# Li-Yuetao/ActiveSplat

Measured on AMD Instinct MI355X. Metric: render+backward frames/sec at 640x480, N Gaussians, higher is better.
Workload: dtype f32; 1 GPU; BASELINE configs[2]'s render (the north star's target configuration): 2000000 Gaussians, SH degree 3, 640x480, forward (colour+radii+depth+opacity) + backward (all input gradients), frames strictly one after the other; gaussians=2000000, sh_degree=3, width=640, height=480, tile_instances_D=4842856, streams=1, parallelism=single GPU

## Files before the change

activesplat_amd/_lib.py:

```python
from __future__ import annotations

import ctypes as C
import os

_HERE = os.path.dirname(os.path.abspath(__file__))
LIB_PATH = os.path.join(_HERE, "libgsplat_hip.so")

_lib = None
_emulated = False


class GsCamera(C.Structure):
    _fields_ = [("image_width", C.c_int32), ("image_height", C.c_int32), ("sh_degree", C.c_int32),
                ("sh_coeffs", C.c_int32), ("tanfovx", C.c_float), ("tanfovy", C.c_float),
                ("scale_modifier", C.c_float), ("num_views", C.c_int32), ("bg", C.c_void_p),
                ("viewmatrix", C.c_void_p), ("projmatrix", C.c_void_p), ("campos", C.c_void_p)]


class GsGeomLayout(C.Structure):
    _fields_ = [(n, C.c_uint64) for n in ("total_bytes", "geom", "rect", "tiles_touched", "offsets", "block_sums", "clamped",
                                          "tile_total", "tile_base", "sh_jac", "depth_bits")]


class GsImageLayout(C.Structure):
    _fields_ = [(n, C.c_uint64) for n in ("total_bytes", "ranges", "final_T", "n_contrib", "split_state")]


class GsAdamTensor(C.Structure):
    _fields_ = [("n", C.c_int64), ("param", C.c_void_p), ("grad", C.c_void_p), ("exp_avg", C.c_void_p), ("exp_avg_sq", C.c_void_p),
                ("lr", C.c_double), ("beta1", C.c_double), ("beta2", C.c_double), ("eps", C.c_double), ("step", C.c_int32),
                ("reserved", C.c_int32)]


class GsRowTensor(C.Structure):
    _fields_ = [("param", C.c_void_p), ("exp_avg", C.c_void_p), ("exp_avg_sq", C.c_void_p), ("grad", C.c_void_p),
                ("lr", C.c_double), ("beta1", C.c_double), ("beta2", C.c_double), ("eps", C.c_double), ("width", C.c_int32),
                ("step", C.c_int32)]


class GsBinLayout(C.Structure):
    _fields_ = [(n, C.c_uint64) for n in ("total_bytes", "path", "pairs", "keys_unsorted", "vals_unsorted", "keys_sorted",
                                          "sort_temp", "segments", "seg_T", "pairs_alt")]


class GsDbscanLayout(C.Structure):
    _fields_ = [(n, C.c_uint64) for n in ("total_bytes", "mask_bits", "core_bits", "root_bits", "word_prefix", "parent", "root", "row_range")]


class GsEvalLayout(C.Structure):
    _fields_ = [("total_bytes", C.c_uint64), ("ms_ssim_defined", C.c_int32), ("levels", C.c_int32), ("level_width", C.c_int32 * 5),
                ("level_height", C.c_int32 * 5)]


class GsHullLayout(C.Structure):
    _fields_ = [(n, C.c_uint64) for n in ("total_bytes", "cluster_status")]


class GsMeshLayout(C.Structure):
    _fields_ = [(n, C.c_uint64) for n in ("total_bytes", "total", "records", "rects", "tile_count", "tile_offset", "list")]


SORT_AUTO, SORT_TILE_LDS, SORT_RADIX = 0, 1, 2


ABI_VERSION = 22

vp, i32, u32, i64, u64, f32, f64, cint = C.c_void_p, C.c_int32, C.c_uint32, C.c_int64, C.c_uint64, C.c_float, C.c_double, C.c_int

BINDINGS = {
    "gs_atlas_layout": (cint, [i32, i32, i32, C.POINTER(i32), C.POINTER(i32), C.POINTER(i32)]),
    "gs_geom_layout": (cint, [i32, i32, i32, C.POINTER(GsGeomLayout)]),
    "gs_image_layout": (cint, [i32, i32, C.POINTER(GsImageLayout)]),
    "gs_bin_layout": (cint, [i64, u32, i32, i32, C.POINTER(GsBinLayout)]),
    "gs_set_sort_path": (cint, [i32]),
    "gs_set_forward_segments": (cint, [i32]),
    "gs_set_half_quadrants": (cint, [i32]),
    "gs_set_backward_chain": (cint, [i32, i32]),
    "gs_set_backward_chain_tickets": (cint, [i32]),
    "gs_set_backward_chain_polls": (cint, [i32]),
    "gs_set_forward_priority": (cint, [i32, f32]),
    "gs_async_status_word": (cint, [C.POINTER(C.POINTER(u32))]),
    "gs_async_status_clear": (cint, []),
    "gs_recorded_cut": (cint, [u32, C.POINTER(u32), C.POINTER(i32)]),
    "gs_set_backward_segments": (cint, [i32]),
    "gs_backward_scratch_bytes": (u64, [i32]),
    "gs_last_error": (C.c_char_p, []),
    "gs_version": (C.c_char_p, []),
    "gs_abi_version": (i32, []),
    "gs_profile_enable": (cint, [i32]),
    "gs_profile_stage_count": (i32, []),
    "gs_profile_stage_name": (C.c_char_p, [i32]),
    "gs_profile_collect": (cint, [vp, vp, i32]),
    "gs_preprocess_forward": (cint, [C.POINTER(GsCamera), i32] + [vp] * 12 + [i32, vp]),
    "gs_render_forward": (cint, [C.POINTER(GsCamera), i32, i64, u32] + [vp] * 10),
    "gs_render_backward": (cint, [C.POINTER(GsCamera), i32, i64] + [vp] * 21 + [i32, i32, vp]),
    "gs_preprocess_forward_raw": (cint, [C.POINTER(GsCamera), i32] + [vp] * 7 + [i32] + [vp] * 7 + [i32, vp]),
    "gs_render_backward_raw": (cint, [C.POINTER(GsCamera), i32, i64] + [vp] * 7 + [i32, i32] + [vp] * 14 + [i32, i32, vp]),
    "gs_pose_grad_scratch_bytes": (u64, [i32]),
    "gs_render_backward_raw_pose": (cint, [C.POINTER(GsCamera), i32, i64] + [vp] * 7 + [i32, i32] + [vp] * 14 + [i32, i32, i32, vp, vp, vp]),
    "gs_adam_step": (cint, [i64] + [vp] * 4 + [f64] * 4 + [i32, vp]),
    "gs_adam_step_multi": (cint, [i32, C.POINTER(GsAdamTensor), vp]),
    "gs_render_backward_raw_adam": (cint, [C.POINTER(GsCamera), i32, i64] + [vp] * 7 + [i32] + [vp] * 8 + [i32, i32, C.POINTER(GsAdamTensor), vp]),
    "gs_pack_columns": (cint, [i32, C.POINTER(GsRowTensor), i64, i64, vp, vp]),
    "gs_adam_rows": (cint, [i32, C.POINTER(GsRowTensor), i64, i64, i64, vp, vp, vp]),
    "gs_unpack_columns": (cint, [i32, C.POINTER(GsRowTensor), i64, vp, vp]),
    "gs_activate_forward": (cint, [i32, i32] + [vp] * 10),
    "gs_activate_backward": (cint, [i32, i32] + [vp] * 13),
    "gs_activate_backward_accumulate": (cint, [i32, i32] + [vp] * 13),
    "gs_activate_backward_pose": (cint, [i32, i32] + [vp] * 13 + [i32, i32, vp, vp, vp]),
    "gs_mapping_loss_scratch_bytes": (u64, [i32, i32]),
    "gs_mapping_loss": (cint, [i32, i32] + [vp] * 5 + [f32, f32] + [vp] * 4 + [i64, vp]),
    "gs_depth_error_median_scratch_bytes": (u64, [i32, i32]),
    "gs_depth_error_median": (cint, [i32, i32] + [vp] * 5),
    "gs_depth_error_median_grid": (cint, [i32, i32] + [vp] * 4 + [i32, vp]),
    "gs_depth_error_median_workgroups": (i32, [i32, i32]),
    "gs_mapping_loss_outlier": (cint, [i32, i32] + [vp] * 5 + [f32, f32] + [vp] * 4 + [i64, vp, vp]),
    "gs_tracking_loss_scratch_bytes": (u64, [i32, i32]),
    "gs_tracking_loss": (cint, [i32, i32] + [vp] * 6 + [i32, f32, f32, f32] + [vp] * 5),
    "gs_tracking_loss_outlier": (cint, [i32, i32] + [vp] * 6 + [i32, f32, f32, f32] + [vp] * 6),
    "gs_preprocess_forward_raw_dev": (cint, [C.POINTER(GsCamera), i32] + [vp] * 8 + [i64, i64, i32] + [vp] * 7 + [i32, vp]),
    "gs_preprocess_forward_topdown": (cint, [C.POINTER(GsCamera), i32] + [vp] * 5 + [i32, f32, f32] + [vp] * 6),
    "gs_render_forward_topdown": (cint, [C.POINTER(GsCamera), i32, i64, u32] + [vp] * 9),
    "gs_render_backward_raw_pose_dev": (cint, [C.POINTER(GsCamera), i32, i64] + [vp] * 8 + [i64, i64, i32] + [vp] * 8 + [i32, i32, vp, vp, vp]),
    "gs_tracking_state_bytes": (u64, []),
    "gs_tracking_begin": (cint, [vp, vp, i64, i64, vp, vp]),
    "gs_tracking_step": (cint, [i32, vp, i32, i32, vp, f32, f32, vp, vp, i64, i64, f64, f64, i32, vp, vp, vp]),
    "gs_compact_scratch_bytes": (u64, [i64]),
    "gs_compact_index": (cint, [i64] + [vp] * 5),
    "gs_gather_rows": (cint, [i64, i32] + [vp] * 4),
    "gs_gather_rows_zero_tail": (cint, [i64, i64, i32] + [vp] * 4),
    "gs_densify_classify": (cint, [i32, i32] + [vp] * 5 + [f32, f32, i32, i32] + [vp] * 5),
    "gs_densify_children": (cint, [i32, i32, i32, vp, vp, u64, vp, vp, vp]),
    "gs_compact3_scratch_bytes": (u64, [i64]),
    "gs_compact_index3": (cint, [i64, vp, vp, vp, i32] + [vp] * 4),
    "gs_visibility_stats": (cint, [i32] + [vp] * 4),
    "gs_accumulate_grad2d": (cint, [i32] + [vp] * 5),
    "gs_grid_dbscan_layout": (cint, [i32] * 4 + [C.POINTER(GsDbscanLayout)]),
    "gs_grid_dbscan": (cint, [i32, i32, i32, vp, i64, i64, f32] + [i32] * 4 + [vp] * 7),
    "gs_cluster_hulls_layout": (cint, [i32] * 5 + [C.POINTER(GsHullLayout)]),
    "gs_cluster_hulls": (cint, [i32, i32, i32, vp, vp, i64, i64, vp, vp, i32, C.POINTER(u32), i32, i32, f32, f64, f64, i32] + [vp] * 8),
    "gs_high_loss_grid": (cint, [i32, i32, vp, vp, vp, f32, f32, i32, i32, vp, vp, vp]),
    "gs_grow_scratch_bytes": (u64, [i32, i32]),
    "gs_grow_gaussians": (cint, [i32, i32] + [vp] * 6 + [f32, i32] + [vp] * 8),
    "gs_keyframe_overlap": (cint, [i32, vp, i32, vp, vp, i32, i32, i32, vp, vp]),
    "gs_frame_ingest": (cint, [i32, i32, vp, vp, vp, i32, C.POINTER(i32)] + [vp] * 5),
    "gs_mesh_render_layout": (cint, [i32, i32, i32, u32, C.POINTER(GsMeshLayout)]),
    "gs_mesh_render": (cint, [i32, vp, i32, vp, vp, C.POINTER(f32), C.POINTER(f32), f32, i32, i32, vp, u32, vp, vp, vp, vp, vp]),
    "gs_depth_cloud": (cint, [i32, i32, vp, C.POINTER(f32), C.POINTER(f32), vp, vp, vp]),
    "gs_cloud_nearest_scratch_bytes": (u64, [i64, i64]),
    "gs_cloud_nearest": (cint, [i64, vp, vp, i64, vp, vp, i32, vp, vp, vp]),
    "gs_completion_row_scratch_bytes": (u64, []),
    "gs_completion_row": (cint, [i64, vp, i64, vp, vp, f64, vp, vp, vp]),
    "gs_eval_frame_layout": (cint, [i32, i32, i32, C.POINTER(GsEvalLayout)]),
    "gs_eval_frame": (cint, [i32, i32] + [vp] * 5 + [f32, i32, vp, vp, vp]),
}

SYMBOLS = tuple(BINDINGS)


def _bind(lib):
    try:
        lib.gs_abi_version.restype = i32
        have = int(lib.gs_abi_version())
# ... 92 lines not shown
```

activesplat_amd/csrc/api.hip:

```cpp
#include <stdio.h>
#include <string.h>

#include <mutex>

#include "gs_common.h"

namespace {

thread_local char g_err[512] = "";

int fail(int code, const char* fmt, const char* a = "")
{
    snprintf(g_err, sizeof(g_err), fmt, a);
    return code;
}

int launched(const char* who, const char* what, hipError_t e)
{
    if (e == hipSuccess) return GS_OK;
    snprintf(g_err, sizeof(g_err), "%s: %s%s%s", who, what, *what ? " " : "", hipGetErrorString(e));
    return GS_ELAUNCH;
}

bool adam_aligned16(const void* p, const void* g, const void* m, const void* v)
// ... 94 lines not shown
    g.geom = (float4*)(b + L.geom); g.rect = (uint2*)(b + L.rect); g.tiles = (uint32_t*)(b + L.tiles_touched);
    g.offsets = (uint32_t*)(b + L.offsets); g.block_sums = (uint32_t*)(b + L.block_sums);
    g.clamped = (uint32_t*)(b + L.clamped);
    g.tile_total = (uint32_t*)(b + L.tile_total); g.tile_base = (uint32_t*)(b + L.tile_base);
    g.sh_jac = (float2*)(b + L.sh_jac);
    g.depth_bits = (uint32_t*)(b + L.depth_bits);
    g.vis_max = nullptr; g.vis_seen = nullptr;
    return g;
}

}

extern "C" {

const char* gs_last_error(void) { return g_err; }
const char* gs_version(void) { return "activesplat_amd gsplat_hip 0.4 (gfx950)"; }
int32_t gs_abi_version(void) { return GS_ABI_VERSION; }

int gs_profile_enable(int32_t on)
{
    g_prof.on = on != 0;
    g_prof.n = 0;
    return GS_OK;
}

int32_t gs_profile_stage_count(void) { return ST_COUNT; }

const char* gs_profile_stage_name(int32_t stage) { return stage >= 0 && stage < ST_COUNT ? kStageNames[stage] : ""; }

int gs_profile_collect(float* ms_sum, int32_t* calls, int32_t n_stages)
{
    if (!ms_sum || !calls || n_stages < ST_COUNT) return fail(GS_EINVAL, "gs_profile_collect: bad argument");
    for (int i = 0; i < n_stages; i++) { ms_sum[i] = 0.f; calls[i] = 0; }
    for (int i = 0; i < g_prof.n; i++) {
        if (hipEventSynchronize(g_prof.ev[i][1]) != hipSuccess) return fail(GS_ELAUNCH, "gs_profile_collect: event sync failed");
        float ms = 0.f;
        if (hipEventElapsedTime(&ms, g_prof.ev[i][0], g_prof.ev[i][1]) != hipSuccess) return fail(GS_ELAUNCH, "gs_profile_collect: elapsed failed");
        ms_sum[g_prof.stage[i]] += ms; calls[g_prof.stage[i]]++;
    }
    g_prof.n = 0;
    return GS_OK;
}

int gs_set_sort_path(int32_t path)
{
    if (path < GS_SORT_AUTO || path > GS_SORT_RADIX) return fail(GS_EINVAL, "gs_set_sort_path: bad path");
    g_sort_path = path;
    return GS_OK;
}

int gs_set_half_quadrants(int32_t max_tiles)
{
    gs::g_half_quadrant_tiles = max_tiles < 0 ? 0 : max_tiles;
    return GS_OK;
}

int gs_set_backward_chain(int32_t pieces, int32_t min_tiles)
{
    if (pieces < 1 || pieces > gs::kChainPieces) return fail(GS_EINVAL, "gs_set_backward_chain: pieces out of range");
    gs::g_chain_pieces = pieces;
    gs::g_chain_min_tiles = min_tiles < 0 ? gs::kChainMinTiles : min_tiles;
    return GS_OK;
}

int gs_set_backward_chain_tickets(int32_t on)
{
    gs::g_chain_tickets = on != 0;
    return GS_OK;
}

int gs_set_backward_chain_polls(int32_t polls)
{
    gs::g_chain_polls = polls == -1 ? gs::kChainPollsDefault : polls;
    return GS_OK;
}

int gs_set_forward_priority(int32_t mode, float param)
{
    if (mode > gs::kFwdPrioChunk) return fail(GS_EINVAL, "gs_set_forward_priority: mode out of range");
    if (mode == gs::kFwdPrioT && param >= 1.0f) return fail(GS_EINVAL, "gs_set_forward_priority: a transmittance threshold lies below 1");
    if (mode < 0) { mode = gs::kFwdPrioDefault; param = gs::kFwdPrioDefaultParam; }
    gs::g_fwd_prio_param = param > 0.0f ? param : 0.0f;
    gs::g_fwd_prio = mode;
    return GS_OK;
}

int gs_async_status_word(uint32_t** host_word)
{
    static uint32_t* word = nullptr;
    static std::mutex mu;
    std::lock_guard<std::mutex> lock(mu);
    if (!word) {
        void* h = nullptr;
        if (hipHostMalloc(&h, 64, hipHostMallocMapped | hipHostMallocPortable) != hipSuccess) {
            (void)hipGetLastError();
            return fail(GS_ELAUNCH, "gs_async_status_word: hipHostMalloc failed");
        }
        memset(h, 0, 64);
        void* d = nullptr;
        if (hipHostGetDevicePointer(&d, h, 0) != hipSuccess) { (void)hipGetLastError(); return fail(GS_ELAUNCH, "gs_async_status_word: no device view of the host word"); }
        void* f = nullptr;
        if (hipMalloc(&f, 64) == hipSuccess && hipMemset(f, 0, 64) == hipSuccess && hipGetDevice(&gs::g_chain_fail_device) == hipSuccess) gs::g_chain_fail_dev = (uint32_t*)f;
        else (void)hipGetLastError();
        word = (uint32_t*)h;
        gs::g_async_status_dev = (uint32_t*)d;
    }
    if (host_word) *host_word = word;
    return GS_OK;
}

int gs_async_status_clear(void)
{
    if (hipDeviceSynchronize() != hipSuccess) { (void)hipGetLastError(); return fail(GS_ELAUNCH, "gs_async_status_clear: device synchronisation failed"); }
    if (gs::g_chain_fail_dev && hipMemset(gs::g_chain_fail_dev, 0, 4) != hipSuccess) { (void)hipGetLastError(); return fail(GS_ELAUNCH, "gs_async_status_clear: hipMemset failed"); }
    return GS_OK;
}

int gs_recorded_cut(uint32_t target, uint32_t* nearest, int32_t* level)
{
    const uint32_t pos = gs::cut_nearest(target);
    if (nearest) *nearest = pos;
    if (level) *level = pos ? gs::cut_level(pos) : -1;
    return GS_OK;
}

int gs_set_backward_segments(int32_t segments)
{
    if (segments < 1 || segments > gs::kFewSegmentsMax) return fail(GS_EINVAL, "gs_set_backward_segments: 1, 2 or 3");
    gs::g_few_segments = segments;
    return GS_OK;
}

int gs_set_forward_segments(int32_t on)
{
    g_segments_enabled = on != 0;
    return GS_OK;
}

int gs_atlas_layout(int32_t P, int32_t view_width, int32_t num_views, int32_t* virtual_P, int32_t* atlas_width, int32_t* view_stride)
{
    if (P < 0 || view_width <= 0 || num_views < 1 || num_views > 64) return fail(GS_EINVAL, "gs_atlas_layout: bad argument");
    const int32_t stride = atlas_view_stride(view_width, num_views);
    if (virtual_P) *virtual_P = virtual_rows(P, num_views);
    if (atlas_width) *atlas_width = num_views * stride;
    if (view_stride) *view_stride = stride;
    return GS_OK;
}

int gs_geom_layout(int32_t P, int32_t width, int32_t height, GsGeomLayout* out)
{
    if (!out || P < 0 || width <= 0 || height <= 0) return fail(GS_EINVAL, "gs_geom_layout: bad argument");
    const uint64_t n = (uint64_t)(P > 0 ? P : 1);
    const uint64_t nb = (n + gs::kBlock - 1) / gs::kBlock;
    const uint64_t tiles = tiles_of(width, height);
    const uint64_t rows = (n + 1023) / 1024;
    uint64_t o = 0;
    out->geom = o; o = align_up(o + n * GS_GEOM_FLOATS * 4);
    out->rect = o; o = align_up(o + n * 8);
    out->tiles_touched = o; o = align_up(o + n * 4);
    out->offsets = o; o = align_up(o + n * 4);
    out->block_sums = o; o = align_up(o + (nb + 1) * 4);
    out->clamped = o; o = align_up(o + n * 4);
    out->tile_total = o; o = align_up(o + tiles * 4);
    out->tile_base = o; o = align_up(o + (tiles <= (uint64_t)gs::kMaxLdsTiles ? rows * tiles * 4 : 4));
    out->sh_jac = o; o = align_up(o + n * gs::kShJacFloats * 4);
    out->depth_bits = o; o = align_up(o + n * 4);
// ... 169 lines not shown
    ForwardCall c{};
    c.in.means3D = means3D; c.in.shs = shs; c.in.colors = colors_precomp; c.in.opac = logit_opacities; c.in.scales = log_scales; c.in.rots = unnorm_rotations;
    c.P = P; c.pose.source = gs::POSE_HOST; c.pose.pose7 = h_pose7; c.isotropic = isotropic; c.max_2D_radius = max_2D_radius; c.seen = seen;
    c.radii = radii; c.geom_state = geom_state; c.image_state = image_state; c.d_counts = d_counts; c.h_counts = h_counts; c.want_backward = want_backward;
    return preprocess_forward_impl(cam, c, stream);
}

int gs_preprocess_forward_raw_dev(const GsCamera* cam, int32_t P, const float* means3D, const float* shs, const float* colors_precomp,
                                  const float* logit_opacities, const float* log_scales, const float* unnorm_rotations,
                                  const float* cam_unnorm_rots, const float* cam_trans, int64_t num_frames, int64_t time_idx, int32_t isotropic,
                                  float* max_2D_radius, uint8_t* seen, int32_t* radii, void* geom_state, void* image_state, uint32_t* d_counts,
                                  uint32_t* h_counts, int32_t want_backward, gs_stream_t stream)
{
    ForwardCall c{};
    c.pose.source = gs::POSE_DEVICE;
    if (!dev_pose(cam_unnorm_rots, cam_trans, num_frames, time_idx, c.pose.dev))
        return fail(GS_EINVAL, "gs_preprocess_forward_raw_dev: null pose columns or time index outside [0, num_frames)");
    if (P > 0 && (!log_scales || !unnorm_rotations)) return fail(GS_EINVAL, "gs_preprocess_forward_raw_dev: null scale / rotation parameters");
    c.in.means3D = means3D; c.in.shs = shs; c.in.colors = colors_precomp; c.in.opac = logit_opacities; c.in.scales = log_scales; c.in.rots = unnorm_rotations;
    c.P = P; c.isotropic = isotropic; c.max_2D_radius = max_2D_radius; c.seen = seen;
    c.radii = radii; c.geom_state = geom_state; c.image_state = image_state; c.d_counts = d_counts; c.h_counts = h_counts; c.want_backward = want_backward;
    return preprocess_forward_impl(cam, c, stream);
}

static int bin_tile_lists(const char* who, const gs::Cam& k, int32_t P, int64_t D, uint32_t max_tile_instances, gs::GeomPtrs gp, uint2* ranges,
                          const GsBinLayout& BL, char* bb, uint32_t* point_list, hipStream_t st)
{
    hipError_t e;
    if (BL.path == GS_SORT_TILE_LDS) {
        if (D > 0) {
            ScopedStage ps(ST_TILE_SCATTER_SORT, st);
            e = gs::launch_tile_scatter_sort(k, P, gp, gp.tile_base, ranges, max_tile_instances,
                                             (unsigned long long*)(bb + BL.pairs), (unsigned long long*)(bb + BL.pairs_alt), point_list, (uint32_t)D, st);
            if (int rc = launched(who, "tile scatter/sort", e)) return rc;
        }
    } else {
        e = hipMemsetAsync(ranges, 0, (size_t)k.gx * k.gy * 8, st);
        if (int rc = launched(who, "memset", e)) return rc;
        if (k.gx * k.gy <= gs::kMaxLdsTiles) {
            e = gs::launch_scan_block_sums(P, gp, gp.block_sums + (P + gs::kBlock - 1) / gs::kBlock, st);
            if (int rc = launched(who, "scan", e)) return rc;
        }
        if (D == 0) {
            e = gs::launch_emit(k, P, gp, nullptr, nullptr, st);
            if (int rc = launched(who, "emit", e)) return rc;
        } else {
            uint64_t* ku = (uint64_t*)(bb + BL.keys_unsorted); uint32_t* vu = (uint32_t*)(bb + BL.vals_unsorted);
            uint64_t* ks = (uint64_t*)(bb + BL.keys_sorted);
            { ScopedStage ps(ST_EMIT, st); e = gs::launch_emit(k, P, gp, ku, vu, st); }
            if (int rc = launched(who, "emit", e)) return rc;
            const int end_bit = 32 + tile_bits(k.gx * k.gy);
            {
                ScopedStage ps(ST_SORT, st);
                e = gs::sort_pairs(bb + BL.sort_temp, (size_t)(BL.total_bytes - BL.sort_temp), ku, ks, vu, point_list, D, end_bit, st);
            }
            if (int rc = launched(who, "sort", e)) return rc;
            { ScopedStage ps(ST_RANGES, st); e = gs::launch_ranges(D, ks, ranges, st); }
            if (int rc = launched(who, "ranges", e)) return rc;
        }
    }
    return GS_OK;
}

int gs_render_forward(const GsCamera* cam, int32_t P, int64_t D, uint32_t max_tile_instances, void* geom_state,
                      void* bin_state, uint32_t* point_list, void* image_state, float* out_color, float* out_depth,
                      float* out_opacity, float* out_depth_sq, void* backward_scratch, gs_stream_t stream)
{
    gs::Cam k;
    if (!make_cam(cam, k)) return fail(GS_EINVAL, "gs_render_forward: invalid camera settings");
    if (P < 0 || D < 0 || !geom_state || !image_state || !out_color || !out_depth || !out_opacity)
        return fail(GS_EINVAL, "gs_render_forward: null pointer");
    if (D > 0 && (!bin_state || !point_list)) return fail(GS_EINVAL, "gs_render_forward: null binning workspace");
    if (D >= (int64_t)1 << 32) return fail(GS_ECAPACITY, "gs_render_forward: more than 2^32 tile instances");
    hipStream_t st = (hipStream_t)stream;
    const int32_t Pin = P;
    P = virtual_count(k, Pin);
    gs::GeomPtrs gp = carve_geom(geom_state, P, k);
    GsImageLayout IL; gs_image_layout(k.W, k.H, &IL);
    char* ib = (char*)image_state;
    uint2* ranges = (uint2*)(ib + IL.ranges);
    GsBinLayout BL; gs_bin_layout(D, max_tile_instances, k.W, k.H, &BL);
    char* bb = (char*)bin_state;
    if (int rc = bin_tile_lists("gs_render_forward", k, P, D, max_tile_instances, gp, ranges, BL, bb, point_list, st)) return rc;
    ScopedStage ps(ST_BLEND_FWD, st);
    return launched("gs_render_forward", "blend", gs::launch_blend_forward(k, ranges, point_list, gp.geom, out_color, out_depth, out_opacity,
                    (float*)(ib + IL.final_T), (uint32_t*)(ib + IL.n_contrib), out_depth_sq, BL.path == GS_SORT_TILE_LDS ? (uint32_t)D : 0xffffffffu,
                    (int)BL.segments, BL.segments > 1 ? (float*)(bb + BL.seg_T) : nullptr, (float*)(ib + IL.split_state), (uint32_t)P,
                    (float*)backward_scratch, st));
}

int gs_preprocess_forward_topdown(const GsCamera* cam, int32_t P, const float* means3D, const float* colors_precomp, const float* logit_opacities,
                                  const float* log_scales, const float* unnorm_rotations, int32_t isotropic, float band_upper, float band_lower,
                                  int32_t* radii, void* geom_state, void* image_state, uint32_t* d_counts, uint32_t* h_counts, gs_stream_t stream)
{
    if (cam && cam->num_views > 1) return fail(GS_EINVAL, "gs_preprocess_forward_topdown: one view only");
    if (P > 0 && (!colors_precomp || !log_scales || !unnorm_rotations))
        return fail(GS_EINVAL, "gs_preprocess_forward_topdown: null colour / scale / rotation parameters");
    if (band_upper != band_upper || band_lower != band_lower) return fail(GS_EINVAL, "gs_preprocess_forward_topdown: NaN height band");
    ForwardCall c{};
    c.in.means3D = means3D; c.in.colors = colors_precomp; c.in.opac = logit_opacities; c.in.scales = log_scales; c.in.rots = unnorm_rotations;
    c.P = P; c.pose.source = gs::POSE_BAND; c.pose.band_upper = band_upper; c.pose.band_lower = band_lower; c.isotropic = isotropic;
    c.radii = radii; c.geom_state = geom_state; c.image_state = image_state; c.d_counts = d_counts; c.h_counts = h_counts;
    return preprocess_forward_impl(cam, c, stream);
}

int gs_render_forward_topdown(const GsCamera* cam, int32_t P, int64_t D, uint32_t max_tile_instances, void* geom_state, void* bin_state,
                              uint32_t* point_list, void* image_state, float* free_opacity, uint8_t* free_map_binary, uint8_t* visible_rgb,
                              uint8_t* visible_map_binary, gs_stream_t stream)
{
    gs::Cam k;
    if (!make_cam(cam, k)) return fail(GS_EINVAL, "gs_render_forward_topdown: invalid camera settings");
    if (k.V != 1) return fail(GS_EINVAL, "gs_render_forward_topdown: one view only");
    if (P < 0 || D < 0 || !geom_state || !image_state || !free_opacity || !free_map_binary || !visible_rgb || !visible_map_binary)
        return fail(GS_EINVAL, "gs_render_forward_topdown: null pointer");
    if (((uintptr_t)free_map_binary | (uintptr_t)visible_rgb | (uintptr_t)visible_map_binary | (uintptr_t)free_opacity) & 3)
        return fail(GS_EINVAL, "gs_render_forward_topdown: output maps must be 4-byte aligned");
    if (D > 0 && (!bin_state || !point_list)) return fail(GS_EINVAL, "gs_render_forward_topdown: null binning workspace");
    if (D >= (int64_t)1 << 32) return fail(GS_ECAPACITY, "gs_render_forward_topdown: more than 2^32 tile instances");
    hipStream_t st = (hipStream_t)stream;
    virtual_count(k, P);
    gs::GeomPtrs gp = carve_geom(geom_state, P, k);
    GsImageLayout IL; gs_image_layout(k.W, k.H, &IL);
    uint2* ranges = (uint2*)((char*)image_state + IL.ranges);
    GsBinLayout BL; gs_bin_layout(D, max_tile_instances, k.W, k.H, &BL);
    if (int rc = bin_tile_lists("gs_render_forward_topdown", k, P, D, max_tile_instances, gp, ranges, BL, (char*)bin_state, point_list, st)) return rc;
    ScopedStage ps(ST_BLEND_FWD, st);
    return launched("gs_render_forward_topdown", "blend", gs::launch_blend_topdown(k, ranges, point_list, gp.geom, free_opacity, free_map_binary, visible_rgb,
                    visible_map_binary, BL.path == GS_SORT_TILE_LDS ? (uint32_t)D : 0xffffffffu, (uint32_t)P, st));
}

struct BackwardCall {
    int32_t P;
    int64_t D;
    gs::GaussianBackward g;
    gs::PoseRequest pose;
    int32_t isotropic, accumulate;
    const void* geom_state; const uint32_t* point_list; const void* image_state;
    const float* dL_dcolor; const float* dL_ddepth;
    void* scratch; int32_t scratch_zeroed, have_sh_jacobian;
    const GsAdamTensor* adam5;
};

static int render_backward_impl(const GsCamera* cam, const BackwardCall& c, gs_stream_t stream)
{
    gs::GaussianBackward g = c.g;
    const gs::GaussianInputs& in = g.in;
    const gs::GaussianGrads& out = g.out;
    const gs::PoseRequest& pose = c.pose;
    const int32_t P = c.P;
    const bool pose_only = pose.grad == gs::POSE_GRAD_ONLY;
    gs::Cam k;
    if (!make_cam(cam, k)) return fail(GS_EINVAL, "gs_render_backward: invalid camera settings");
    set_input_activation(k, pose, c.isotropic, pose_only ? 0 : c.accumulate);
    if (k.act && k.V != 1) return fail(GS_EINVAL, "gs_render_backward_raw: one view only");
    if (k.act && (!in.opac || in.cov3D || (in.shs && k.sh_coeffs != 16)))
        return fail(GS_EINVAL, "gs_render_backward_raw: scale / rotation parameters with colours or 16-coefficient SH rows only");
    if (k.V > 1) return fail(GS_EINVAL, "gs_render_backward: multi-view atlas renders are forward-only");
    if (P < 0 || c.D < 0 || !c.geom_state || !c.image_state || !c.dL_dcolor || !c.scratch)
        return fail(GS_EINVAL, "gs_render_backward: null pointer");
    if (pose.grad && (!k.act || c.adam5 || (!pose.dL_dpose7 && pose.source != gs::POSE_DEVICE) || !pose.pose_scratch))
        return fail(GS_EINVAL, "gs_render_backward_raw_pose: raw-parameter mode with a pose-gradient output and its scratch only");
    if (pose.source == gs::POSE_DEVICE && !pose_only) return fail(GS_EINVAL, "gs_render_backward_raw_pose_dev: the pose-only backward only");
    if (P == 0) {
        if (pose.grad && pose.dL_dpose7)
            return launched("gs_render_backward_raw_pose", "memset", hipMemsetAsync(pose.dL_dpose7, 0, 7 * sizeof(float), (hipStream_t)stream));
        return GS_OK;
    }
    gs::FusedAdam fa{};
    if (c.adam5) {
        if (!k.act || c.accumulate) return fail(GS_EINVAL, "gs_render_backward_raw_adam: raw-parameter mode without accumulation only");
        if (!in.means3D || !g.radii || !out.dmeans2D || !in.scales || !in.rots || (in.shs == nullptr) == (in.colors == nullptr))
// ... 750 lines not shown
```

activesplat_amd/csrc/blend.hip:

```cpp
#include "gs_common.h"
#include <atomic>

namespace gs {

constexpr int kFwdStreams = 4;

constexpr float kAlphaMin = 1.0f / 255.0f;
constexpr float kTmin = 0.0001f;
constexpr float kLog2e = 1.4426950408889634f;
constexpr uint32_t kNoId = 0xffffffffu;

struct TileCtx {
    int tile, tx, ty, px, py, quad, seg;
    float qx0, qy0, pxf, pyf;
    bool inside;
};

template <int NW>
__device__ __forceinline__ bool tile_ctx_at(const Cam& cam, unsigned block, int wave, int lane, TileCtx& c, int segments = 0)
{
    const int G = (segments > 1 ? 4 * segments : 4) / NW;
    const int ntiles = cam.gx * cam.gy, per = (ntiles + 7) >> 3;
    const int idx = (int)(block >> 3);
    c.tile = (int)(block & 7) * per + idx / G;
    if (idx / G >= per || c.tile >= ntiles) return false;
    int quad = (idx % G) * NW + wave;
    c.seg = segments > 1 ? quad >> 2 : 0;
    if (segments > 1) quad &= 3;
    c.tx = c.tile % cam.gx; c.ty = c.tile / cam.gx; c.quad = quad;
    const int qx = c.tx * kTile + (quad & 1) * kQuad, qy = c.ty * kTile + (quad >> 1) * kQuad;
    c.px = qx + (lane & 7); c.py = qy + (lane >> 3);
    c.qx0 = (float)qx; c.qy0 = (float)qy; c.pxf = (float)c.px; c.pyf = (float)c.py;
    c.inside = c.px < cam.W && c.py < cam.H;
    return true;
}

template <int NW>
__device__ __forceinline__ bool tile_ctx_nw(const Cam& cam, int wave, int lane, TileCtx& c, int segments = 0)
{
    return tile_ctx_at<NW>(cam, blockIdx.x, wave, lane, c, segments);
}


struct StreamPixel { int sid, l, px, py; float pxf, pyf; bool inside; };
__device__ __forceinline__ StreamPixel stream_pixel(const Cam& cam, float qx0, float qy0, int lane)
{
    StreamPixel s;
    s.sid = lane >> 4; s.l = lane & 15;
    s.px = (int)qx0 + (s.sid & 1) * 4 + (s.l & 3); s.py = (int)qy0 + (s.sid >> 1) * 4 + (s.l >> 2);
    s.inside = s.px < cam.W && s.py < cam.H;
    s.pxf = (float)s.px; s.pyf = (float)s.py;
    return s;
}

struct StagedConic { float4 s0; float c; };
__device__ __forceinline__ StagedConic staged_conic(const float4& q0, const float4& q1)
{
    return {make_float4(q0.x, q0.y, -0.5f * kLog2e * q0.z, -kLog2e * q0.w), -0.5f * kLog2e * q1.x};
}
__device__ __forceinline__ void stage_record(float4* s0, float4* s1, float4* s2, int lane, const float4& q0,
                                             const float4& q1, const float4& q2, uint32_t id)
{
    const StagedConic k = staged_conic(q0, q1);
    s0[lane] = k.s0;
    s1[lane] = make_float4(k.c, q1.y, q1.z, q1.w);
    s2[lane] = make_float4(q2.x, q2.y, __uint_as_float(id), 0.0f);
}

struct SplatAlpha { float alpha, p, G; bool hit; };
__device__ __forceinline__ SplatAlpha splat_alpha(const float4& a0, float c, float op, float pxf, float pyf)
{
    SplatAlpha a;
    const float dx = a0.x - pxf, dy = a0.y - pyf;
    float bdy, cyy;
    {
#pragma clang fp contract(off)
        bdy = a0.w * dy; cyy = (c * dy) * dy;
    }
    a.p = (a0.z * dx + bdy) * dx + cyy;
    a.G = __builtin_amdgcn_exp2f(a.p);
    a.alpha = fminf(0.99f, op * a.G);
    a.hit = a.p <= 0.0f && a.alpha >= kAlphaMin;
    return a;
}

struct Composite { float T, w; bool done, ok; };
__device__ __forceinline__ Composite composite_step(float T, bool done, float alpha, bool hit)
{
    const float test_T = T * (1.0f - alpha);
    const bool vis = !done && hit;
    const bool ok = vis && test_T >= kTmin;
    return {ok ? test_T : T, ok ? alpha * T : 0.0f, done || (vis != ok), ok};
}

__device__ __forceinline__ void write_sentinel(float4* s0, float4* s1, float4* s2, int lane)
{
    if (lane == 0) {
        s0[kWave] = make_float4(0.f, 0.f, 0.f, 0.f);
        s1[kWave] = make_float4(0.f, 0.f, 0.f, 0.f);
        s2[kWave] = make_float4(0.f, 0.f, __uint_as_float(0u), 0.f);
    }
    __builtin_amdgcn_wave_barrier();
}

__device__ __forceinline__ unsigned scan_blocks(const float4& q0, const float4& q2, bool valid, float qx0, float qy0, bool g0, bool g1, bool g2, bool g3,
                                                unsigned long long& m_any, unsigned long long* masks = nullptr)
{
    const float ex = q2.z, ey = q2.w;
    const float xl = q0.x - ex, xh = q0.x + ex, yl = q0.y - ey, yh = q0.y + ey;
    const unsigned long long vis = __ballot(valid) & __ballot(ex >= 0.0f);
    const unsigned long long cx0 = __ballot(xh >= qx0) & __ballot(xl <= qx0 + 3.0f), cx1 = __ballot(xh >= qx0 + 4.0f) & __ballot(xl <= qx0 + 4.0f + 3.0f);
    const unsigned long long cy0 = vis & __ballot(yh >= qy0) & __ballot(yl <= qy0 + 3.0f), cy1 = vis & __ballot(yh >= qy0 + 4.0f) & __ballot(yl <= qy0 + 4.0f + 3.0f);
    const unsigned long long b0 = g0 ? cx0 & cy0 : 0ull, b1 = g1 ? cx1 & cy0 : 0ull, b2 = g2 ? cx0 & cy1 : 0ull, b3 = g3 ? cx1 & cy1 : 0ull;
    m_any = (b0 | b1) | (b2 | b3);
    if (masks) { masks[0] = b0; masks[1] = b1; masks[2] = b2; masks[3] = b3; }
    return (__builtin_amdgcn_inverse_ballot_w64(b0) ? 1u : 0u) | (__builtin_amdgcn_inverse_ballot_w64(b1) ? 2u : 0u) |
           (__builtin_amdgcn_inverse_ballot_w64(b2) ? 4u : 0u) | (__builtin_amdgcn_inverse_ballot_w64(b3) ? 8u : 0u);
}
__device__ __forceinline__ void scan_going_blocks(const float4& q0, const float4& q2, bool valid, float qx0, float qy0, unsigned long long going,
                                                  unsigned long long& m_any, unsigned long long* masks)
{
    scan_blocks(q0, q2, valid, qx0, qy0, (going & 0xffffull) != 0ull, (going & 0xffff0000ull) != 0ull, (going & 0xffff00000000ull) != 0ull,
                (going >> 48) != 0ull, m_any, masks);
}

__device__ __forceinline__ int build_stream_lists(uint8_t* lists, const unsigned long long* mb, int lane, int* ranks = nullptr)
{
    reinterpret_cast<uint32_t*>(lists)[lane] = 0x40404040u;
    __builtin_amdgcn_wave_barrier();
    int ntrips = 0;
#pragma unroll
    for (int s = 0; s < 4; s++) {
        const unsigned long long m = mb[s];
        const int rank = (int)__builtin_amdgcn_mbcnt_hi((uint32_t)(m >> 32), __builtin_amdgcn_mbcnt_lo((uint32_t)m, 0u));
        const bool in = __builtin_amdgcn_inverse_ballot_w64(m);
        if (in) lists[s * kWave + rank] = (uint8_t)lane;
        if (ranks) ranks[s] = in ? rank : 0xff;
        ntrips = max(ntrips, (int)__popcll(m));
    }
    return ntrips;
}

struct GradFill {
    size_t at, end;
};
__device__ __forceinline__ GradFill grad_fill_start(const float4* zero_fill, uint32_t P, int tid)
{
    GradFill f = {0, 0};
    if (zero_fill) {
        const size_t total = (size_t)P * (kGradStride / 4), per = (total + gridDim.x - 1) / gridDim.x;
        f.at = (size_t)blockIdx.x * per + tid; f.end = min(total, (size_t)blockIdx.x * per + per);
    }
    return f;
}
__device__ __forceinline__ GradFill grad_fill_step(float4* zero_fill, GradFill f, int threads)
{
    constexpr int kPerStep = 2;
#pragma unroll
    for (int k = 0; k < kPerStep; k++)
        if (f.at < f.end) { zero_fill[f.at] = make_float4(0.f, 0.f, 0.f, 0.f); f.at += threads; }
    return f;
}
__device__ __forceinline__ void grad_fill_rest(float4* zero_fill, GradFill f, int threads)
{
    for (; f.at < f.end; f.at += threads) zero_fill[f.at] = make_float4(0.f, 0.f, 0.f, 0.f);
}

template <bool DEPTH_SQ>
__device__ __forceinline__ void store_pixel_outputs(const Cam& cam, int px, int py, float T, uint32_t last, float C0, float C1, float C2, float Dp, float Dq,
                                                    float* out_color, float* out_depth, float* out_opacity, float* final_T, uint32_t* n_contrib,
                                                    float* out_depth_sq)
{
    const size_t pix = (size_t)py * cam.W + px, HW = (size_t)cam.H * cam.W;
    final_T[pix] = T;
    n_contrib[pix] = last;
    out_color[pix] = C0 + T * cam.bg[0];
    out_color[HW + pix] = C1 + T * cam.bg[1];
    out_color[2 * HW + pix] = C2 + T * cam.bg[2];
    out_depth[pix] = Dp;
    out_opacity[pix] = 1.0f - T;
    if (DEPTH_SQ) out_depth_sq[pix] = Dq;
}
__device__ __forceinline__ void set_wave_priority(int level)
{
    level = __builtin_amdgcn_readfirstlane(level);
    if (level >= 3) __builtin_amdgcn_s_setprio(3);
    else if (level == 2) __builtin_amdgcn_s_setprio(2);
    else if (level == 1) __builtin_amdgcn_s_setprio(1);
    else __builtin_amdgcn_s_setprio(0);
}
constexpr int kRoundSlack = 4;

template <bool DEPTH_SQ, int NS, int SEG, int NW>
__global__ __launch_bounds__(NW * kWave) void blend_forward_streams_kernel(
    Cam cam, const uint2* __restrict__ ranges, const uint32_t* __restrict__ point_list,
    const float4* __restrict__ geom, float* __restrict__ out_color, float* __restrict__ out_depth,
    float* __restrict__ out_opacity, float* __restrict__ final_T, uint32_t* __restrict__ n_contrib,
    float* __restrict__ out_depth_sq, uint32_t cap, float* __restrict__ seg_T, float* __restrict__ split_state, uint32_t P,
    float4* __restrict__ zero_fill)
{
    static_assert(NS == 4 && kWave / NS == 16, "the scan tests the four 4x4 blocks of a quadrant");
    __shared__ float4 s_rec[NW][3][kWave + 1];
    __shared__ __attribute__((aligned(16))) uint8_t s_list[NW][4 * kWave + 16];
    const int tid = threadIdx.x, lane = tid & 63, wave = tid >> 6;
    GradFill fill = grad_fill_start(SEG == 0 ? zero_fill : nullptr, P, tid);
    TileCtx c;
    if (SEG == 0 && cam.chain > 1 && split_state && blockIdx.x == 0 && tid < 8)
        reinterpret_cast<uint32_t*>(split_state)[(size_t)cam.gx * cam.gy * 4 * (kChainStateFloats + kChainPieces - 1) + (size_t)tid * kChainTicketStride] = 0u;
    if (!tile_ctx_nw<NW>(cam, wave, lane, c)) { if (SEG == 0) grad_fill_rest(zero_fill, fill, NW * kWave); return; }
    if (SEG == 0 && cam.chain > 1 && split_state && lane < kChainPieces - 1)
        reinterpret_cast<uint32_t*>(split_state)[(size_t)cam.gx * cam.gy * 4 * kChainStateFloats + (size_t)(c.tile * 4 + c.quad) * (kChainPieces - 1) + lane] = 0u;
    const StreamPixel sp = stream_pixel(cam, c.qx0, c.qy0, lane);
    const int px = sp.px, py = sp.py;
    const bool inside = sp.inside;
    const float pxf = sp.pxf, pyf = sp.pyf;
    float4* s0 = s_rec[wave][0]; float4* s1 = s_rec[wave][1]; float4* s2 = s_rec[wave][2];
    write_sentinel(s0, s1, s2, lane);
    uint8_t* my_list = s_list[wave] + sp.sid * kWave;
    uint2 range = ranges[c.tile];
    range.x = min(range.x, cap); range.y = min(range.y, cap);
    const uint32_t n_all = range.y - range.x;
    const uint32_t* list = point_list + range.x;
    uint32_t first = 0, n = n_all;
    float T = 1.0f;
    bool next_stopped = true;
    float* my_seg_T = nullptr;
    uint32_t* seg_flag = nullptr;
    if (SEG != 0) {
        const uint32_t S = gridDim.y, seg = blockIdx.y;
        const uint32_t L = (((n_all + S - 1) / S + kWave - 1) / kWave) * kWave;
        first = min(n_all, seg * L);
        n = min(n_all, first + L);
        float* tile_T = seg_T + ((size_t)c.tile * S) * kBlock + c.quad * kWave + lane;
        my_seg_T = tile_T + (size_t)seg * kBlock;
        if (SEG == 1) {
            seg_flag = reinterpret_cast<uint32_t*>(seg_T + (size_t)cam.gx * cam.gy * S * kBlock) + c.tile * 4 + c.quad;
            const uint32_t f = __hip_atomic_load(seg_flag, __ATOMIC_RELAXED, __HIP_MEMORY_SCOPE_AGENT);
            if (f & ((1u << seg) - 1u)) { my_seg_T[0] = 1.0f; return; }
        }
        if (SEG == 2) {
            for (uint32_t q = 0; q < seg; q++) T *= tile_T[(size_t)q * kBlock];
            next_stopped = seg + 1 == S ? true : (T * my_seg_T[0] < kTmin);
        }
    }
    float C0 = 0.f, C1 = 0.f, C2 = 0.f, Dp = 0.f, Dq = 0.f;
    uint32_t last = 0;
    const bool stopped_at_entry = SEG == 2 && T < kTmin;
    bool done = !inside || stopped_at_entry;

    if (SEG == 1 || !__all(done)) {
        uint32_t id_next = first + (uint32_t)lane < n ? list[first + lane] : kNoId;
        uint32_t id_next2 = first + (uint32_t)lane + 64u < n ? list[first + lane + 64] : kNoId;
        if (id_next >= P) id_next = kNoId;
        if (id_next2 >= P) id_next2 = kNoId;
        float4 r0 = make_float4(0.f, 0.f, 0.f, 0.f), r1 = r0, r2 = make_float4(0.f, 0.f, -1.f, -1.f);
        if (first < n) {
            const float4* gr = geom + (size_t)(id_next != kNoId ? id_next : 0u) * 3;
            r0 = gr[0]; r1 = gr[1]; r2 = gr[2];
        }
        for (uint32_t base = first; base < n; base += kWave) {
            if (SEG == 0) fill = grad_fill_step(zero_fill, fill, NW * kWave);
            if (SEG == 0 && cam.fwd_prio != kFwdPrioOff) {
                const float chunks = (float)((base - first) >> 6);
                const float p = cam.fwd_prio_param;
                int level;
                if (cam.fwd_prio == kFwdPrioChunk) {
                    level = (chunks >= p ? 1 : 0) + (chunks >= 2.0f * p ? 1 : 0) + (chunks >= 3.0f * p ? 1 : 0);
                } else {
                    float t1 = p, t2 = p * p, t3 = p * p * p;
                    if (cam.fwd_prio == kFwdPrioDecay) {
                        constexpr float kLog2Tmin = -13.287712f;
                        t1 = __builtin_amdgcn_exp2f(kLog2Tmin * chunks * __builtin_amdgcn_rcpf(chunks + p));
                        t2 = __builtin_amdgcn_exp2f(kLog2Tmin * chunks * __builtin_amdgcn_rcpf(chunks + 2.0f * p));
                        t3 = __builtin_amdgcn_exp2f(kLog2Tmin * chunks * __builtin_amdgcn_rcpf(chunks + 4.0f * p));
                    }
                    level = (__ballot(!done && T > t1) != 0ull ? 1 : 0) + (__ballot(!done && T > t2) != 0ull ? 1 : 0) +
                            (__ballot(!done && T > t3) != 0ull ? 1 : 0);
                    const uint32_t left = (n - base) >> 6;
                    level = min(level, (left > kFwdPrioListChunks ? 1 : 0) + (left > 2u * kFwdPrioListChunks ? 1 : 0) + (left > 3u * kFwdPrioListChunks ? 1 : 0));
                }
                set_wave_priority(level);
            }
            const float4 q0 = r0, q1 = r1, q2 = r2;
            const uint32_t id_cur = id_next;
            id_next = id_next2;
            id_next2 = base + 128u + (uint32_t)lane < n ? list[base + 128u + lane] : kNoId;
            if (id_next2 >= P) id_next2 = kNoId;
            {
                const float4* gr = geom + (size_t)(id_next != kNoId ? id_next : 0u) * 3;
                r0 = gr[0]; r1 = gr[1]; r2 = gr[2];
            }

            const unsigned long long going = SEG == 1 ? ~0ull : ~__ballot(done);
            unsigned long long m_any, mb[4];
            scan_going_blocks(q0, q2, id_cur != kNoId, c.qx0, c.qy0, going, m_any, mb);
            if (m_any == 0ull) continue;
            stage_record(s0, s1, s2, lane, q0, q1, q2, id_cur);
            const int ntrips = build_stream_lists(s_list[wave], mb, lane);
            __builtin_amdgcn_wave_barrier();
            uint32_t jj2_next = *reinterpret_cast<const uint16_t*>(my_list);
            int lj = -1;
            for (int t = 0; t < ntrips; t += 2) {
                const uint32_t jj2 = jj2_next;
                jj2_next = *reinterpret_cast<const uint16_t*>(my_list + t + 2);
                const int jj[2] = {(int)(jj2 & 0xffu), (int)(jj2 >> 8)};
                float4 a0[2], a1[2], a2[2];
#pragma unroll
                for (int u = 0; u < 2; u++) { a0[u] = s0[jj[u]]; a1[u] = s1[jj[u]]; a2[u] = s2[jj[u]]; }
#pragma unroll
                for (int u = 0; u < 2; u++) {
                    const SplatAlpha a = splat_alpha(a0[u], a1[u].x, a1[u].y, pxf, pyf);
                    if (SEG == 1) {
                        T = a.hit ? T * (1.0f - a.alpha) : T;
                        continue;
                    }
                    const Composite k = composite_step(T, done, a.alpha, a.hit);
                    T = k.T; done = k.done;
                    C0 += a1[u].z * k.w; C1 += a1[u].w * k.w; C2 += a2[u].x * k.w; Dp += a2[u].y * k.w;
                    if (DEPTH_SQ) Dq += a2[u].y * a2[u].y * k.w;
                    lj = k.ok ? jj[u] : lj;
                }
            }
            last = lj >= 0 ? base + (uint32_t)lj + 1u : last;
            __builtin_amdgcn_wave_barrier();
            if (SEG != 1 && __all(done)) break;
            if (SEG == 1 && __all(!inside || T < kTmin)) break;
        }
        if (SEG == 0 && cam.fwd_prio != kFwdPrioOff) __builtin_amdgcn_s_setprio(0);
    }
    if (SEG == 0) grad_fill_rest(zero_fill, fill, NW * kWave);
    if (SEG == 1) {
        my_seg_T[0] = T;
        if (__all(!inside || T < kTmin) && lane == 0) atomicOr(seg_flag, 1u << blockIdx.y);
        return;
    }
    if (SEG == 2) {
        if (inside && !stopped_at_entry) {
            const size_t pix = (size_t)py * cam.W + px, HW = (size_t)cam.H * cam.W;
            const float tb = next_stopped ? T : 0.0f;
            atomicAdd(out_color + pix, C0 + tb * cam.bg[0]);
            atomicAdd(out_color + HW + pix, C1 + tb * cam.bg[1]);
            atomicAdd(out_color + 2 * HW + pix, C2 + tb * cam.bg[2]);
            atomicAdd(out_depth + pix, Dp);
            if (DEPTH_SQ) atomicAdd(out_depth_sq + pix, Dq);
            if (last) atomicMax(n_contrib + pix, last);
            if (next_stopped) { final_T[pix] = T; out_opacity[pix] = 1.0f - T; }
        }
        return;
    }
    if (inside) store_pixel_outputs<DEPTH_SQ>(cam, px, py, T, last, C0, C1, C2, Dp, Dq, out_color, out_depth, out_opacity, final_T, n_contrib, out_depth_sq);
}

__host__ __device__ __forceinline__ uint32_t rgb_to_grey_u8(uint32_t r, uint32_t g, uint32_t b)
{
    return (4899u * r + 9617u * g + 1868u * b + 8192u) >> 14;
}
__device__ __forceinline__ uint32_t unit_to_u8(float c)
{
    return (uint32_t)(fminf(fmaxf(c, 0.0f), 1.0f) * 255.0f);
}

__global__ __launch_bounds__(kBlock) void blend_topdown_kernel(
    Cam cam, const uint2* __restrict__ ranges, const uint32_t* __restrict__ point_list, const float4* __restrict__ geom,
    float* __restrict__ free_opacity, uint8_t* __restrict__ free_binary, uint8_t* __restrict__ visible_rgb, uint8_t* __restrict__ visible_binary,
    uint32_t cap, uint32_t P)
{
    constexpr int NW = 4;
    static_assert(kFwdStreams == 4, "the scan tests the four 4x4 blocks of a quadrant");
    __shared__ float4 s_rec[NW][3][kWave + 1];
    __shared__ __attribute__((aligned(16))) uint8_t s_list[NW][4 * kWave + 16];
    const int tid = threadIdx.x, lane = tid & 63, wave = tid >> 6;
    TileCtx c;
    if (!tile_ctx_nw<NW>(cam, wave, lane, c)) return;
    const StreamPixel sp = stream_pixel(cam, c.qx0, c.qy0, lane);
    const int px = sp.px, py = sp.py, l = sp.l;
    const bool inside = sp.inside;
    const float pxf = sp.pxf, pyf = sp.pyf;
    float4* s0 = s_rec[wave][0]; float4* s1 = s_rec[wave][1]; float4* s2 = s_rec[wave][2];
    write_sentinel(s0, s1, s2, lane);
    uint8_t* my_list = s_list[wave] + sp.sid * kWave;
    uint2 range = ranges[c.tile];
    range.x = min(range.x, cap); range.y = min(range.y, cap);
    const uint32_t n = range.y - range.x;
    const uint32_t* list = point_list + range.x;
    float T = 1.0f, Tb = 1.0f, C0 = 0.f, C1 = 0.f, C2 = 0.f;
    bool done = !inside, done_b = !inside;

    if (!__all(done)) {
        uint32_t id_next = (uint32_t)lane < n ? list[lane] : kNoId;
        uint32_t id_next2 = (uint32_t)lane + 64u < n ? list[lane + 64] : kNoId;
        if (id_next >= P) id_next = kNoId;
        if (id_next2 >= P) id_next2 = kNoId;
        float4 r0 = make_float4(0.f, 0.f, 0.f, 0.f), r1 = r0, r2 = make_float4(0.f, 0.f, -1.f, -1.f);
        if (0u < n) {
            const float4* gr = geom + (size_t)(id_next != kNoId ? id_next : 0u) * 3;
            r0 = gr[0]; r1 = gr[1]; r2 = gr[2];
        }
        for (uint32_t base = 0; base < n; base += kWave) {
            const float4 q0 = r0, q1 = r1, q2 = r2;
            const uint32_t id_cur = id_next;
            id_next = id_next2;
            id_next2 = base + 128u + (uint32_t)lane < n ? list[base + 128u + lane] : kNoId;
            if (id_next2 >= P) id_next2 = kNoId;
            {
                const float4* gr = geom + (size_t)(id_next != kNoId ? id_next : 0u) * 3;
                r0 = gr[0]; r1 = gr[1]; r2 = gr[2];
            }
            const unsigned long long going = ~__ballot(done && done_b);
            unsigned long long m_any, mb[4];
            scan_going_blocks(q0, q2, id_cur != kNoId, c.qx0, c.qy0, going, m_any, mb);
            if (m_any == 0ull) continue;
// ... 492 lines not shown
                sm[4] = opb * fmaf(u3, ddy[3], fmaf(u2, ddy[2], fmaf(u1, ddy[1], u0 * ddy[0])));
                sm[5] = (gr[0] + gr[1]) + (gr[2] + gr[3]);
                sm[6] = ww[0] * e0[0]; sm[7] = ww[0] * e1[0]; sm[8] = ww[0] * e2[0]; sm[9] = 0.0f;
#pragma unroll
                for (int i = 1; i < 16; i++) {
                    sm[6] = fmaf(ww[i], e0[i], sm[6]); sm[7] = fmaf(ww[i], e1[i], sm[7]); sm[8] = fmaf(ww[i], e2[i], sm[8]);
                }
                if (DEPTH_GRAD) {
                    const float4* z4 = reinterpret_cast<const float4*>(s_ez[wave] + rb * 16);
#pragma unroll
                    for (int v = 0; v < 4; v++) {
                        const float4 z = z4[v];
                        sm[9] = fmaf(ww[4 * v + 3], z.w, fmaf(ww[4 * v + 2], z.z, fmaf(ww[4 * v + 1], z.y, fmaf(ww[4 * v], z.x, sm[9]))));
                    }
                }
                __builtin_amdgcn_wave_barrier();
                float4* ps = reinterpret_cast<float4*>(pair_lds + lane * kPairStride);
                ps[0] = make_float4(sm[0], sm[1], sm[2], sm[3]);
                ps[1] = make_float4(sm[4], 0.f, sm[5], sm[6]);
                ps[2] = make_float4(sm[7], sm[8], sm[9], 0.f);
            }
            __builtin_amdgcn_wave_barrier();
            {
                const int pr[4] = {p0 - t0, p1 - t0, p2 - t0, p3 - t0};
#pragma unroll
                for (int r = 0; r < 4; r++) {
                    if ((unsigned)pr[r] < (unsigned)kBT) {
                        const float4* q = reinterpret_cast<const float4*>(pair_lds + (pr[r] * 4 + r) * kPairStride);
                        const float4 qa = q[0], qb = q[1], qc = q[2];
                        racc[0] += qa.x; racc[1] += qa.y; racc[2] += qa.z; racc[3] += qa.w; racc[4] += qb.x;
                        racc[5] += qb.z; racc[6] += qb.w; racc[7] += qc.x; racc[8] += qc.y; racc[9] += qc.z;
                    }
                }
            }
            __builtin_amdgcn_wave_barrier();
        }
        __builtin_amdgcn_wave_barrier();
        {
            float* fls = s_m[wave][0];
            if (lane < cnt) {
                float4* f4 = reinterpret_cast<float4*>(fls + lane * kPairStride);
                f4[0] = make_float4(racc[0], racc[1], racc[2], racc[3]);
                f4[1] = make_float4(racc[4], 0.f, racc[5], racc[6]);
                f4[2] = make_float4(racc[7], racc[8], racc[9], 0.f);
            }
            __builtin_amdgcn_wave_barrier();
            const int krec = min(fl_rec, 5);
            for (int g = 0; g < cnt; g += 24) {
                float val[4];
                uint32_t id[4];
#pragma unroll
                for (int u = 0; u < 4; u++) {
                    const int slot = g + 6 * u + krec, sl = min(slot, kWave);
                    const float v = fls[sl * kPairStride + fl_off];
                    id[u] = __float_as_uint(s2[sl].w);
                    val[u] = (lane < 60 && slot < cnt) ? v : 0.0f;
                }
                asm volatile("" ::: "memory");
#pragma unroll
                for (int u = 0; u < 4; u++)
                    if (val[u] != 0.0f) atomicAdd(grad2d + (size_t)id[u] * kGradStride + fl_comp, val[u]);
            }
        }
        __builtin_amdgcn_wave_barrier();
        cnt = 0;
    }
    if (pieces > 1 && piece < pieces - 1) {
        float* out = chain_st + piece * 2 * kWave;
        __hip_atomic_store(out + lane, T, __ATOMIC_RELAXED, __HIP_MEMORY_SCOPE_AGENT);
        __hip_atomic_store(out + kWave + lane, S, __ATOMIC_RELAXED, __HIP_MEMORY_SCOPE_AGENT);
        GS_WAIT_VMEM();
        __builtin_amdgcn_wave_barrier();
        if (lane == 0) __hip_atomic_store(chain_fl + piece, cam.chain_epoch, __ATOMIC_RELAXED, __HIP_MEMORY_SCOPE_AGENT);
    }
}

std::atomic<int> g_half_quadrant_tiles{256};
std::atomic<int> g_chain_pieces{kChainPieces};
std::atomic<int> g_chain_min_tiles{kChainMinTiles};
std::atomic<int> g_chain_tickets{0};
std::atomic<int> g_chain_polls{kChainPollsDefault};
std::atomic<int> g_fwd_prio{kFwdPrioDefault};
std::atomic<float> g_fwd_prio_param{kFwdPrioDefaultParam};
uint32_t* g_async_status_dev = nullptr;
uint32_t* g_chain_fail_dev = nullptr;
int g_chain_fail_device = -1;
std::atomic<int> g_few_segments{kFewSegmentsMax};

static hipError_t clear_handover_flags(const Cam& cam, float* split_state, hipStream_t st)
{
    return hipMemsetAsync(split_state + (size_t)cam.gx * cam.gy * 4 * kChainStateFloats, 0, chain_flag_words((size_t)cam.gx * cam.gy) * sizeof(uint32_t), st);
}
static hipError_t mark_nothing_recorded(const Cam& cam, float* split_state, hipStream_t st)
{
    return hipMemsetAsync(split_state + (kCutLevels * 5 + 4) * ((size_t)cam.W * cam.H), 0, sizeof(uint32_t), st);
}

hipError_t launch_blend_forward(const Cam& cam_in, const uint2* ranges, const uint32_t* point_list, const float4* geom,
                                float* out_color, float* out_depth, float* out_opacity, float* final_T,
                                uint32_t* n_contrib, float* out_depth_sq, uint32_t cap, int segments, float* seg_T, float* split_state, uint32_t P,
                                float* zero_fill, hipStream_t st)
{
    Cam cam = cam_in;
    const int k_half = g_half_quadrant_tiles.load(std::memory_order_relaxed), k_fseg = g_few_segments.load(std::memory_order_relaxed);
    cam.half = (segments <= 1 || !seg_T) && cam.gx * cam.gy <= k_half;
    cam.split = (cam.V == 1 && split_state && cam.gx * cam.gy <= min(k_half, kFewTiles)) && k_fseg > 1 ? k_fseg : 0;
    cam.chain = (cam.V == 1 && split_state && cam.gx * cam.gy > kFewTiles) ? kChainPieces : 0;
    cam.fwd_prio = g_fwd_prio.load(std::memory_order_relaxed);
    cam.fwd_prio_param = g_fwd_prio_param.load(std::memory_order_relaxed);
    if (!(cam.fwd_prio_param > 0.0f)) cam.fwd_prio_param = fwd_prio_default_param(cam.fwd_prio);
    const int nb = ((cam.gx * cam.gy + 7) >> 3) << 3;
#define GS_FWD(DSQ, SEG, GRID)                                                                                                     \
    hipLaunchKernelGGL((blend_forward_streams_kernel<DSQ, kFwdStreams, SEG, 4>), GRID, dim3(kBlock), 0, st, cam, ranges, point_list, geom, \
                       out_color, out_depth, out_opacity, final_T, n_contrib, out_depth_sq, cap, seg_T, split_state, P, (float4*)zero_fill)
    const size_t HW = (size_t)cam.W * cam.H;
    if (segments > 1 && seg_T) {
        hipError_t e = zero_fill ? hipMemsetAsync(zero_fill, 0, (size_t)P * kGradStride * sizeof(float), st) : hipSuccess;
        if (e == hipSuccess)
            e = hipMemsetAsync(seg_T + (size_t)cam.gx * cam.gy * segments * kBlock, 0, (size_t)cam.gx * cam.gy * 4 * sizeof(uint32_t), st);
        if (e == hipSuccess) e = hipMemsetAsync(out_color, 0, 3 * HW * sizeof(float), st);
        if (e == hipSuccess) e = hipMemsetAsync(out_depth, 0, HW * sizeof(float), st);
        if (e == hipSuccess && out_depth_sq) e = hipMemsetAsync(out_depth_sq, 0, HW * sizeof(float), st);
        if (e == hipSuccess) e = hipMemsetAsync(n_contrib, 0, HW * sizeof(uint32_t), st);
        if (e == hipSuccess && split_state && cam.gx * cam.gy <= kFewTiles) e = mark_nothing_recorded(cam, split_state, st);
        if (e == hipSuccess && cam.chain > 1) e = clear_handover_flags(cam, split_state, st);
        if (e != hipSuccess) return e;
        const dim3 grid(nb, segments);
        if (out_depth_sq) { GS_FWD(true, 1, grid); GS_FWD(true, 2, grid); }
        else { GS_FWD(false, 1, grid); GS_FWD(false, 2, grid); }
    } else if (cam.half || cam.split) {
        if (cam.chain > 1) {
            hipError_t e = clear_handover_flags(cam, split_state, st);
            if (e != hipSuccess) return e;
        }
        const dim3 grid(((cam.gx * cam.gy + 7) >> 3) << 3), block(kPcWaves * kWave);
        if (out_depth_sq)
            hipLaunchKernelGGL((blend_forward_pc_kernel<true>), grid, block, 0, st, cam, ranges, point_list, geom, out_color, out_depth, out_opacity,
                               final_T, n_contrib, out_depth_sq, cap, split_state, P, (float4*)zero_fill);
        else
            hipLaunchKernelGGL((blend_forward_pc_kernel<false>), grid, block, 0, st, cam, ranges, point_list, geom, out_color, out_depth, out_opacity,
                               final_T, n_contrib, out_depth_sq, cap, split_state, P, (float4*)zero_fill);
    } else {
        if (split_state && cam.gx * cam.gy <= kFewTiles) {
            hipError_t e = mark_nothing_recorded(cam, split_state, st);
            if (e != hipSuccess) return e;
        }
        if (out_depth_sq) GS_FWD(true, 0, dim3(nb)); else GS_FWD(false, 0, dim3(nb));
    }
#undef GS_FWD
    return hipGetLastError();
}

hipError_t launch_blend_topdown(const Cam& cam_in, const uint2* ranges, const uint32_t* point_list, const float4* geom, float* free_opacity,
                                uint8_t* free_binary, uint8_t* visible_rgb, uint8_t* visible_binary, uint32_t cap, uint32_t P, hipStream_t st)
{
    Cam cam = cam_in;
    cam.half = 0; cam.split = 0; cam.chain = 0;
    if (cam.V != 1) return hipErrorInvalidValue;
    const int nb = ((cam.gx * cam.gy + 7) >> 3) << 3;
    hipLaunchKernelGGL(blend_topdown_kernel, dim3(nb), dim3(kBlock), 0, st, cam, ranges, point_list, geom, free_opacity, free_binary, visible_rgb,
                       visible_binary, cap, P);
    return hipGetLastError();
}

hipError_t launch_blend_backward(const Cam& cam_in, const uint2* ranges, const uint32_t* point_list, const float4* geom, const float* split_state,
                                 const float* final_T, const uint32_t* n_contrib, const float* dL_dcolor,
                                 const float* dL_ddepth, float* grad2d, hipStream_t st)
{
    Cam cam = cam_in;
    cam.half = 0;
    const int k_half = g_half_quadrant_tiles.load(std::memory_order_relaxed), k_fseg = g_few_segments.load(std::memory_order_relaxed);
    const int k_pieces = g_chain_pieces.load(std::memory_order_relaxed), k_min = g_chain_min_tiles.load(std::memory_order_relaxed);
    cam.split = (split_state != nullptr && cam.gx * cam.gy <= min(k_half, kFewTiles) && k_fseg > 1) ? k_fseg : 0;
    cam.chain = (cam.V == 1 && split_state && cam.gx * cam.gy > max(k_min, kFewTiles) && k_pieces > 1) ? k_pieces : 0;
    static std::atomic<unsigned> epoch{0};
    do { cam.chain_epoch = ++epoch; } while (cam.chain_epoch == 0u);
    cam.chain_ticket = g_chain_tickets.load(std::memory_order_relaxed); cam.chain_polls = g_chain_polls.load(std::memory_order_relaxed);
    cam.async_status = g_async_status_dev;
    cam.chain_fail = chain_fail_word();
    const int per = ((cam.gx * cam.gy + 7) >> 3) * (cam.split ? cam.split : cam.chain > 1 ? cam.chain : 1);
#define GS_BWD(DG, FEW)                                                                                                          \
    hipLaunchKernelGGL((blend_backward_kernel<DG, 1, FEW>), dim3(per * 8 * 4), dim3(kWave), 0, st, cam, ranges, point_list, geom, final_T, \
                       n_contrib, dL_dcolor, dL_ddepth, grad2d, split_state)
    if (cam.split) { if (dL_ddepth) GS_BWD(true, true); else GS_BWD(false, true); }
    else { if (dL_ddepth) GS_BWD(true, false); else GS_BWD(false, false); }
#undef GS_BWD
    return hipGetLastError();
}

}
```

activesplat_amd/csrc/gs_common.h:

```cpp
#pragma once
#include <hip/hip_runtime.h>
#include <stdint.h>
#include <math.h>

#include <atomic>
#include <type_traits>

#include "../../include/gsplat_hip.h"

namespace gs {

constexpr int kTile = GS_TILE;
constexpr int kBlock = 256;
constexpr int kWave = 64;
constexpr int kQuad = 8;
#ifndef GS_BIN_CHUNK
#define GS_BIN_CHUNK 2048
#endif
constexpr int kBinChunk = GS_BIN_CHUNK;
constexpr int kMaxLdsTiles = 8192;
constexpr int kSortChunk = 2048;
constexpr int kSortCapMax = 16384;

struct Cam {
// ... 70 lines not shown
    const float u[4] = {q[0] * inv, q[1] * inv, q[2] * inv, q[3] * inv};
    if (iso) { for (int k = 0; k < 4; k++) out[k] = u[k]; return; }
    float m[4];
    qmul(cam_q, u, m);
    const float invm = 1.0f / fmaxf(sqrtf(m[0] * m[0] + m[1] * m[1] + m[2] * m[2] + m[3] * m[3]), 1e-12f);
    for (int k = 0; k < 4; k++) out[k] = m[k] * invm;
}
__device__ __forceinline__ void activate_rotation_bwd(const float* cam_q, int iso, const float* q, const float* g, float* dq)
{
    const float nq = fmaxf(sqrtf(q[0] * q[0] + q[1] * q[1] + q[2] * q[2] + q[3] * q[3]), 1e-12f);
    const float u[4] = {q[0] / nq, q[1] / nq, q[2] / nq, q[3] / nq};
    float du[4];
    if (iso) {
        for (int k = 0; k < 4; k++) du[k] = g[k];
    } else {
        float m[4];
        qmul(cam_q, u, m);
        const float nm = fmaxf(sqrtf(m[0] * m[0] + m[1] * m[1] + m[2] * m[2] + m[3] * m[3]), 1e-12f);
        const float r[4] = {m[0] / nm, m[1] / nm, m[2] / nm, m[3] / nm};
        const float dot = r[0] * g[0] + r[1] * g[1] + r[2] * g[2] + r[3] * g[3];
        float dm[4];
        for (int k = 0; k < 4; k++) dm[k] = (g[k] - r[k] * dot) / nm;
        qmul_bwd_rhs(cam_q, dm, du);
    }
    const float dotu = u[0] * du[0] + u[1] * du[1] + u[2] * du[2] + u[3] * du[3];
    for (int k = 0; k < 4; k++) dq[k] = (du[k] - u[k] * dotu) / nq;
}

__device__ __forceinline__ void qmul_bwd_lhs(const float* b, const float* dm, float* da)
{
    da[0] = b[0] * dm[0] + b[1] * dm[1] + b[2] * dm[2] + b[3] * dm[3];
    da[1] = -b[1] * dm[0] + b[0] * dm[1] - b[3] * dm[2] + b[2] * dm[3];
    da[2] = -b[2] * dm[0] + b[3] * dm[1] + b[0] * dm[2] - b[1] * dm[3];
    da[3] = -b[3] * dm[0] - b[2] * dm[1] + b[1] * dm[2] + b[0] * dm[3];
}
constexpr int kPoseAcc = 16;
__device__ __forceinline__ void pose_grad_accumulate(const float* cam_q, int iso, const float* w, const float* dmean, const float* q,
                                                     const float* g, float (&acc)[kPoseAcc])
{
    for (int a = 0; a < 3; a++) {
        acc[a] += dmean[a];
        for (int b = 0; b < 3; b++) acc[3 + 3 * a + b] += dmean[a] * w[b];
    }
    if (iso) return;
    const float nq = fmaxf(sqrtf(q[0] * q[0] + q[1] * q[1] + q[2] * q[2] + q[3] * q[3]), 1e-12f);
    const float u[4] = {q[0] / nq, q[1] / nq, q[2] / nq, q[3] / nq};
    float m[4];
    qmul(cam_q, u, m);
    const float nm = fmaxf(sqrtf(m[0] * m[0] + m[1] * m[1] + m[2] * m[2] + m[3] * m[3]), 1e-12f);
    const float r[4] = {m[0] / nm, m[1] / nm, m[2] / nm, m[3] / nm};
    const float dot = r[0] * g[0] + r[1] * g[1] + r[2] * g[2] + r[3] * g[3];
    float dm[4], da[4];
    for (int k = 0; k < 4; k++) dm[k] = (g[k] - r[k] * dot) / nm;
    qmul_bwd_lhs(u, dm, da);
    for (int k = 0; k < 4; k++) acc[12 + k] += da[k];
}

struct AdamCoef { float one_m_b1, b2, one_m_b2, step_size, inv_bc2s, eps; };
struct FusedAdam {
    float* p[5];
    float* m[5];
    float* v[5];
    AdamCoef c[5];
    const uint32_t* fail;
};

struct GeomPtrs {
    float4* geom;
    uint2* rect;
    uint32_t* tiles;
    uint32_t* offsets;
    uint32_t* block_sums;
    uint32_t* clamped;
    uint32_t* tile_total;
    uint32_t* tile_base;
    uint32_t* depth_bits;
    float2* sh_jac;
    float* vis_max;
    uint8_t* vis_seen;
};

#ifndef GS_WAIT_VMEM
#define GS_WAIT_VMEM() asm volatile("s_waitcnt vmcnt(0)" ::: "memory")
#endif

__device__ __forceinline__ float wave_sum(float v)
{
#pragma unroll
    for (int m = 32; m >= 1; m >>= 1) v += __shfl_xor(v, m);
    return v;
}
__device__ __forceinline__ uint32_t wave_sum_u32(uint32_t v)
{
#pragma unroll
    for (int m = 32; m >= 1; m >>= 1) v += __shfl_xor(v, m);
    return v;
}
__device__ __forceinline__ uint32_t wave_inclusive_scan(uint32_t v, int lane)
{
#pragma unroll
    for (int d = 1; d < 64; d <<= 1) {
        uint32_t o = __shfl_up(v, d);
        if (lane >= d) v += o;
    }
    return v;
}
__device__ __forceinline__ void pose_grad_block_row(float (&acc)[kPoseAcc], float* __restrict__ row)
{
    __shared__ float s_red[kBlock / kWave][kPoseAcc];
    const int lane = threadIdx.x & (kWave - 1), wave = threadIdx.x / kWave;
    for (int k = 0; k < kPoseAcc; k++) {
        const float v = wave_sum(acc[k]);
        if (lane == 0) s_red[wave][k] = v;
    }
    __syncthreads();
    if (threadIdx.x < kPoseAcc) {
        float s = 0.f;
        for (int w = 0; w < kBlock / kWave; w++) s += s_red[w][threadIdx.x];
        row[threadIdx.x] = s;
    }
}
template <class PoseT>
__device__ __forceinline__ void pose_grad_finish_block(int64_t nrows, const PoseT& pose, const float* __restrict__ rows, float* __restrict__ out)
{
    constexpr int kSlices = kBlock / kPoseAcc;
    __shared__ double s[kSlices][kPoseAcc];
    const int c = threadIdx.x % kPoseAcc, sl = threadIdx.x / kPoseAcc;
    double acc = 0.0;
    for (int64_t r = sl; r < nrows; r += kSlices) acc += (double)rows[r * kPoseAcc + c];
    s[sl][c] = acc;
    __syncthreads();
    if (threadIdx.x != 0) return;
    double t[kPoseAcc];
    for (int k = 0; k < kPoseAcc; k++) {
        double v = 0.0;
        for (int j = 0; j < kSlices; j++) v += s[j][k];
        t[k] = v;
    }
    const double* dR = t + 3;
    const double q0 = pose.q[0], q1 = pose.q[1], q2 = pose.q[2], q3 = pose.q[3];
    const double nq = sqrt(q0 * q0 + q1 * q1 + q2 * q2 + q3 * q3);
    const double r = q0 / nq, x = q1 / nq, y = q2 / nq, z = q3 / nq;
    const double d0 = 2.0 * (-z * dR[1] + y * dR[2] + z * dR[3] - x * dR[5] - y * dR[6] + x * dR[7]);
    const double d1 = 2.0 * (y * dR[1] + z * dR[2] + y * dR[3] - 2.0 * x * dR[4] - r * dR[5] + z * dR[6] + r * dR[7] - 2.0 * x * dR[8]);
    const double d2 = 2.0 * (-2.0 * y * dR[0] + x * dR[1] + r * dR[2] + x * dR[3] + z * dR[5] - r * dR[6] + z * dR[7] - 2.0 * y * dR[8]);
    const double d3 = 2.0 * (-2.0 * z * dR[0] - r * dR[1] + x * dR[2] + r * dR[3] - 2.0 * z * dR[4] + y * dR[5] + x * dR[6] + y * dR[7]);
    const double dot = r * d0 + x * d1 + y * d2 + z * d3;
    out[0] = (float)((d0 - r * dot) / nq + t[12]); out[1] = (float)((d1 - x * dot) / nq + t[13]);
    out[2] = (float)((d2 - y * dot) / nq + t[14]); out[3] = (float)((d3 - z * dot) / nq + t[15]);
    out[4] = (float)t[0]; out[5] = (float)t[1]; out[6] = (float)t[2];
}

__device__ __forceinline__ double strided_record_sum(const double* __restrict__ part, int64_t records, int stride)
{
    double a = 0.0;
    for (int64_t r = threadIdx.x; r < records; r += kBlock) a += part[r * stride];
    return a;
}

template <int K>
__device__ __forceinline__ void block_tree_sum(double (&a)[K], double (&s_tree)[K][kBlock])
{
    const int tid = threadIdx.x;
#pragma unroll
    for (int k = 0; k < K; ++k) s_tree[k][tid] = a[k];
    __syncthreads();
// ... 289 lines not shown
            GS_SHJ4(1, 0.f, c21 * z, c21 * y);
            GS_SHJ4(2, c22 * (-2.f * x), c22 * (-2.f * y), c22 * (4.f * z));
            GS_SHJ4(3, c23 * z, 0.f, c23 * x);
        }
    }
    {
        GS_SHLOAD(2);
        GS_SHC(0, 8);
        if (want_j) GS_SHJ4(0, c24 * (2.f * x), c24 * (-2.f * y), 0.f);
        if (deg >= 3) {
            GS_SHC(1, 9); GS_SHC(2, 10); GS_SHC(3, 11);
            if (want_j) {
                GS_SHJ4(1, c30 * (6.f * x * y), c30 * (3.f * xx - 3.f * yy), 0.f);
                GS_SHJ4(2, c31 * y * z, c31 * x * z, c31 * x * y);
                GS_SHJ4(3, c32 * (-2.f * x * y), c32 * (4.f * zz - xx - 3.f * yy), c32 * (8.f * y * z));
            }
        }
    }
    if (deg < 3) return;
    {
        GS_SHLOAD(3);
        GS_SHC(0, 12); GS_SHC(1, 13); GS_SHC(2, 14); GS_SHC(3, 15);
        if (want_j) {
            GS_SHJ4(0, c33 * (-6.f * x * z), c33 * (-6.f * y * z), c33 * (6.f * zz - 3.f * xx - 3.f * yy));
            GS_SHJ4(1, c34 * (4.f * zz - 3.f * xx - yy), c34 * (-2.f * x * y), c34 * (8.f * x * z));
            GS_SHJ4(2, c35 * (2.f * x * z), c35 * (-2.f * y * z), c35 * (xx - yy));
            GS_SHJ4(3, c36 * (3.f * xx - 3.f * yy), c36 * (-6.f * x * y), 0.f);
        }
    }
}
#undef GS_SHC
#undef GS_SHJ4
#undef GS_SHLOAD

constexpr int kShJacFloats = 10;
__device__ __forceinline__ void store_sh_jac(float2* base, size_t i, const float (&J)[9], uint32_t clamp_bits)
{
    float2* o = base + i * (kShJacFloats / 2);
    o[0] = make_float2(J[0], J[1]); o[1] = make_float2(J[2], J[3]); o[2] = make_float2(J[4], J[5]); o[3] = make_float2(J[6], J[7]);
    o[4] = make_float2(J[8], __uint_as_float(clamp_bits));
}
__device__ __forceinline__ void load_sh_jac(const float2* base, size_t i, float (&J)[9], uint32_t& clamp_bits)
{
    const float2* o = base + i * (kShJacFloats / 2);
    const float2 a = o[0], b = o[1], c = o[2], d = o[3], e = o[4];
    J[0] = a.x; J[1] = a.y; J[2] = b.x; J[3] = b.y; J[4] = c.x; J[5] = c.y; J[6] = d.x; J[7] = d.y; J[8] = e.x;
    clamp_bits = __float_as_uint(e.y);
}

struct GaussianInputs {
    const float* means3D;
    const float* shs;
    const float* colors;
    const float* opac;
    const float* scales;
    const float* rots;
    const float* cov3D;
};
struct GaussianGrads { float *dmeans2D, *dmeans3D, *dopac, *dcolors, *dshs, *dscales, *drots, *dcov3D; };
struct DevPose { const float* q; const float* t; int64_t stride; };
enum PoseSource { POSE_NONE = 0, POSE_HOST, POSE_DEVICE, POSE_BAND };
enum PoseGrad { POSE_GRAD_NONE = 0, POSE_GRAD_WITH_PARAMS = 1, POSE_GRAD_ONLY = 2 };
struct PoseRequest {
    PoseSource source;
    const float* pose7;
    DevPose dev;
    float band_upper, band_lower;
    PoseGrad grad;
    float* dL_dpose7;
    void* pose_scratch;
};
struct GaussianBackward {
    GaussianInputs in;
    GaussianGrads out;
    const int32_t* radii;
    const uint32_t* clamped;
    const float2* sh_jac;
    const float* grad2d;
    const FusedAdam* adam;
};

template <class CamT>
hipError_t launch_preprocess_forward(const CamT& cam, int P, const GaussianInputs& in, int32_t* radii, GeomPtrs gp, hipStream_t st);
hipError_t launch_scan_block_sums(int P, GeomPtrs gp, uint32_t* d_total, hipStream_t st);
template <class CamT>
hipError_t launch_preprocess_backward(const CamT& cam, int P, const GaussianBackward& g, const PoseRequest& pose, hipStream_t st);
hipError_t launch_tile_count(const Cam& cam, int P, GeomPtrs gp, uint32_t* tile_total, uint32_t* tile_base,
                             uint2* ranges, uint32_t* d_counts, uint32_t* host_counts, hipStream_t st);
hipError_t launch_tile_scatter_sort(const Cam& cam, int P, GeomPtrs gp, uint32_t* tile_base, const uint2* ranges,
                                    uint32_t max_tile_instances, unsigned long long* pairs, unsigned long long* pairs_alt,
                                    uint32_t* point_list, uint32_t cap, hipStream_t st);
extern std::atomic<int> g_half_quadrant_tiles;
extern std::atomic<int> g_chain_pieces;
extern std::atomic<int> g_chain_min_tiles;
extern std::atomic<int> g_chain_tickets;
extern std::atomic<int> g_chain_polls;
enum { kFwdPrioOff = 0, kFwdPrioT = 1, kFwdPrioDecay = 2, kFwdPrioChunk = 3 };
constexpr int kFwdPrioDefault = kFwdPrioT;
constexpr float kFwdPrioDefaultParam = 0.0f;
constexpr uint32_t kFwdPrioListChunks = 3;
extern std::atomic<int> g_fwd_prio;
extern std::atomic<float> g_fwd_prio_param;
inline float fwd_prio_default_param(int mode)
{
    return mode == kFwdPrioT ? 0.1f : mode == kFwdPrioDecay ? 3.0f : 6.0f;
}
extern uint32_t* g_async_status_dev;
extern uint32_t* g_chain_fail_dev;
extern int g_chain_fail_device;
inline uint32_t* chain_fail_word()
{
    if (!g_chain_fail_dev) return nullptr;
    int dev = -1;
    if (hipGetDevice(&dev) != hipSuccess) { (void)hipGetLastError(); return nullptr; }
    return dev == g_chain_fail_device ? g_chain_fail_dev : nullptr;
}
extern std::atomic<int> g_few_segments;
constexpr int kFewTiles = 256;
constexpr int kChainPieces = 3;
constexpr int kChainMinTiles = 768;
constexpr int kChainStateFloats = (kChainPieces - 1) * 2 * kWave;
constexpr int kChainTicketStride = 32;
constexpr int kChainTicketWords = 8 * kChainTicketStride;
inline size_t chain_flag_words(size_t tiles) { return tiles * 4 * (kChainPieces - 1) + kChainTicketWords; }
inline size_t chain_state_words(size_t tiles) { return tiles * 4 * kChainStateFloats + chain_flag_words(tiles); }
constexpr int kChainPollsDefault = 1 << 21;
constexpr int kCutStep = 256;
constexpr int kCutLinear = 4096;
constexpr int kCutLast = 131072;
constexpr int kCutLevels = kCutLinear / kCutStep + 5;
constexpr int kFewSegmentsMax = 3;
__host__ __device__ inline int cut_level(uint32_t pos)
{
    if (pos >= (uint32_t)kCutStep && pos <= (uint32_t)kCutLinear) return pos % kCutStep == 0 ? (int)(pos / kCutStep) - 1 : -1;
    if (pos > (uint32_t)kCutLinear && pos <= (uint32_t)kCutLast && (pos & (pos - 1u)) == 0u) {
        int l = kCutLinear / kCutStep - 1;
        for (uint32_t q = kCutLinear; q < pos; q <<= 1) ++l;
        return l;
    }
    return -1;
}
__host__ __device__ inline uint32_t cut_nearest(uint32_t target)
{
    if (target < (uint32_t)kCutStep / 2) return 0u;
    if (target <= (uint32_t)kCutLinear + kCutStep / 2) {
        uint32_t k = (target + kCutStep / 2) / kCutStep;
        if (k < 1u) k = 1u;
        if (k > (uint32_t)(kCutLinear / kCutStep)) k = kCutLinear / kCutStep;
        return k * kCutStep;
    }
    uint32_t pos = kCutLinear;
    while (pos < (uint32_t)kCutLast && (unsigned long long)target * 46341ull >= ((unsigned long long)pos << 16)) pos <<= 1;
    return pos;
}
hipError_t launch_emit(const Cam& cam, int P, GeomPtrs gp, uint64_t* keys, uint32_t* vals, hipStream_t st);
hipError_t launch_ranges(int64_t D, const uint64_t* keys_sorted, uint2* ranges, hipStream_t st);
hipError_t launch_blend_forward(const Cam& cam, const uint2* ranges, const uint32_t* point_list, const float4* geom,
                                float* out_color, float* out_depth, float* out_opacity, float* final_T,
                                uint32_t* n_contrib, float* out_depth_sq, uint32_t cap, int segments, float* seg_T, float* split_state, uint32_t P, float* zero_fill,
                                hipStream_t st);
hipError_t launch_blend_topdown(const Cam& cam, const uint2* ranges, const uint32_t* point_list, const float4* geom, float* free_opacity,
                                uint8_t* free_binary, uint8_t* visible_rgb, uint8_t* visible_binary, uint32_t cap, uint32_t P, hipStream_t st);
hipError_t launch_blend_backward(const Cam& cam, const uint2* ranges, const uint32_t* point_list, const float4* geom, const float* split_state,
                                 const float* final_T, const uint32_t* n_contrib, const float* dL_dcolor,
                                 const float* dL_ddepth, float* grad2d, hipStream_t st);
hipError_t launch_adam_multi(int count, const GsAdamTensor* tensors, hipStream_t st);
hipError_t launch_rows(int mode, int count, const GsRowTensor* t, int64_t row0, int64_t n_valid, int64_t n_rows, const float* in, float* out,
                       hipStream_t st);
hipError_t launch_adam(int64_t n, float* p, const float* g, float* m, float* v, double lr, double b1, double b2,
                       double eps, int step, hipStream_t st);

hipError_t launch_activate_forward(int P, int iso, const float* pose7, const float* means3D, const float* rots, const float* logit_op,
                                   const float* log_scales, float* o_means, float* o_rots, float* o_op, float* o_scales, hipStream_t st);
hipError_t launch_activate_backward(int P, int iso, const float* pose7, const float* rots, const float* o_op, const float* o_scales,
                                    const float* g_means, const float* g_rots, const float* g_op, const float* g_scales, float* d_means,
                                    float* d_rots, float* d_logit, float* d_logs, int accumulate, hipStream_t st);
hipError_t launch_activate_backward_pose(int P, int iso, const float* pose7, const float* means3D, const float* rots, const float* o_op,
                                         const float* o_scales, const float* g_means, const float* g_rots, const float* g_op,
                                         const float* g_scales, float* d_means, float* d_rots, float* d_logit, float* d_logs, int accumulate,
                                         int pose_mode, float* pose_rows, hipStream_t st);
inline int64_t pose_rows_count(int64_t P) { return (P + kBlock - 1) / kBlock; }
hipError_t launch_pose_grad_finish(int64_t nrows, const float* pose7, const float* pose_rows, float* dpose7, hipStream_t st);
hipError_t launch_pose_grad_finish_dev(int64_t nrows, const float* dev_q, int64_t stride, const float* pose_rows, float* dpose7, hipStream_t st);
constexpr int kTrackState = 32;
struct TrackAdam { float one_m_b1, b2, one_m_b2, bc2_sqrt, eps, neg_step_size[2]; };
hipError_t launch_tracking_begin(const float* rots_col, const float* trans_col, int64_t stride, float* state, hipStream_t st);
hipError_t launch_tracking_step(int64_t pose_nrows, const float* pose_rows, int64_t loss_nrows, const float* loss_rows, float w_im, float w_depth,
                                float* rots_col, float* trans_col, int64_t stride, const TrackAdam& c, float* state, float* history_row,
                                hipStream_t st);
inline int64_t tracking_loss_rows(int64_t npix) { return (npix + kBlock - 1) / kBlock; }
hipError_t launch_tracking_loss(int W, int H, const float* im, const float* gt, const float* depth, const float* depth_sq, const float* gt_depth,
                                const float* sil, int use_sil, float sil_thres, float w_im, float w_depth, float* dL_dim, float* dL_ddepth,
                                float* rows, float* losses, hipStream_t st, const float* d_median = nullptr);
constexpr int kLossAccSlots = 256;
hipError_t launch_mapping_loss(int W, int H, const float* im, const float* gt, const float* depth, const float* depth_sq,
                               const float* gt_depth, float w_im, float w_depth, float* losses, float* dL_dim,
                               float* dL_ddepth, float* scratch, int64_t persistent_call, hipStream_t st, const float* d_median = nullptr);
__device__ __forceinline__ float depth_error(float g, float d)
{
#pragma clang fp contract(off)
    return fabsf(g - d) * (g > 0.0f ? 1.0f : 0.0f);
}
constexpr int kMedianBins = 2048;
constexpr int kMedianScratchWords = 3 * kMedianBins + 16;
constexpr int kMedianChunk = 2048;
constexpr int kMedianAutoGrid = 64;
constexpr int kMedianMaxGrid = 1024;
int depth_median_grid(int64_t n);
hipError_t launch_depth_error_median(int64_t n, const float* depth, const float* gt_depth, uint32_t* scratch, float* d_median, int grid,
                                     hipStream_t st);
hipError_t launch_visibility_stats(int P, const int32_t* radii, uint8_t* seen, float* max_radius, hipStream_t st);
hipError_t launch_accumulate_grad2d(int P, const float* grad, const uint8_t* seen, float* accum, float* denom, hipStream_t st);
struct DbscanArgs {
    const float* values; int64_t row_stride, image_stride;
    int H, W, Ww, npix;
    float threshold; int complement, eps, min_samples, max_clusters;
    int half_width[9];
    uint64_t *mask_bits, *core_bits, *root_bits;
    uint32_t* word_prefix;
    uint32_t* parent;
    int32_t* root;
    uint32_t* row_range;
    int32_t *labels, *n_clusters, *table; float *sum_value, *total;
};
hipError_t launch_grid_dbscan(const DbscanArgs& a, int B, hipStream_t st);
struct HullArgs {
    const int32_t* labels;
    const float* depth; int64_t row_stride, image_stride;
    const int32_t* n_clusters; const float* sum_value;
    int H, W, Ww, max_clusters, max_points;
    int kh, kw; uint32_t footprint[15];
    float skip_depth; double scale;
    int32_t* cluster_status;
    double* volume; int32_t* n_points; int32_t* contour_xy;
    double *sum_volume, *sum_invisibility; int32_t* status;
};
hipError_t launch_cluster_hulls(const HullArgs& a, int B, hipStream_t st);
struct HighLossArgs {
    const float *depth, *opacity, *gt;
    int W, H, gw, gh;
    float depth_thres, opacity_thres;
    uint8_t* mask_full;
    float* grid;
// ... 64 lines not shown
```

activesplat_amd/csrc/preprocess.hip:

```cpp
#include "gs_common.h"
#include <type_traits>

#pragma clang fp contract(off)

namespace gs {

__device__ __forceinline__ int clamp_tile(float v, int hi)
{
    v = fminf(fmaxf(v, -1048576.0f), 1048576.0f);
    int i = (int)v;
    return min(hi, max(0, i));
}

__device__ __forceinline__ void sh_basis(int deg, float x, float y, float z, float* b)
{
    b[0] = 0.28209479177387814f;
    if (deg > 0) {
        b[1] = -0.4886025119029199f * y; b[2] = 0.4886025119029199f * z; b[3] = -0.4886025119029199f * x;
        if (deg > 1) {
            const float xx = x * x, yy = y * y, zz = z * z, xy = x * y, yz = y * z, xz = x * z;
            b[4] = 1.0925484305920792f * xy;
            b[5] = -1.0925484305920792f * yz;
            b[6] = 0.31539156525252005f * (2.0f * zz - xx - yy);
            b[7] = -1.0925484305920792f * xz;
            b[8] = 0.5462742152960396f * (xx - yy);
            if (deg > 2) {
                b[9] = -0.5900435899266435f * y * (3.0f * xx - yy);
                b[10] = 2.890611442640554f * xy * z;
                b[11] = -0.4570457994644658f * y * (4.0f * zz - xx - yy);
                b[12] = 0.3731763325901154f * z * (2.0f * zz - 3.0f * xx - 3.0f * yy);
                b[13] = -0.4570457994644658f * x * (4.0f * zz - xx - yy);
                b[14] = 1.445305721320277f * z * (xx - yy);
                b[15] = -0.5900435899266435f * x * (xx - 3.0f * yy);
            }
        }
    }
}

template <bool HAS_SH>
__device__ __forceinline__ uint32_t project_gaussian(const Cam& cam, int P, int view, int i, int io, int tid, const float* s_mean,
                                                     const float* s_scale, const float* s_rot, const float* s_cov, const float* s_col,
                                                     bool has_cov, float o, const float (&sh_rgb)[3], uint32_t sh_clamp,
                                                     int32_t* __restrict__ radii, const GeomPtrs& gp, int* radius_out = nullptr, bool band = false)
{
    uint32_t ntiles = 0;
    if (radius_out) *radius_out = 0;
    if (i < P) {
        const float* m = cam.view + 16 * view;
        const float* q = cam.proj + 16 * view;
        const float px = s_mean[tid * 3], py = s_mean[tid * 3 + 1], pz = s_mean[tid * 3 + 2];
        const float tx = ((m[0] * px + m[4] * py) + m[8] * pz) + m[12];
        const float ty = ((m[1] * px + m[5] * py) + m[9] * pz) + m[13];
        const float tz = ((m[2] * px + m[6] * py) + m[10] * pz) + m[14];
        int radius = 0;
        float4 g0 = make_float4(0.f, 0.f, 0.f, 0.f), g1 = g0, g2 = g0;
        uint2 rc = make_uint2(0u, 0u);
        uint32_t clampbits = 0;
        if (tz > 0.2f) {
            const float hx = ((q[0] * px + q[4] * py) + q[8] * pz) + q[12];
            const float hy = ((q[1] * px + q[5] * py) + q[9] * pz) + q[13];
            const float hw = ((q[3] * px + q[7] * py) + q[11] * pz) + q[15];
            const float pw = 1.0f / (hw + 1e-7f);
            const float ndcx = hx * pw, ndcy = hy * pw;
            const float limx = 1.3f * cam.tanfovx, limy = 1.3f * cam.tanfovy;
            const float txtz = tx / tz, tytz = ty / tz;
            const float cx_ = fminf(limx, fmaxf(-limx, txtz)) * tz;
            const float cy_ = fminf(limy, fmaxf(-limy, tytz)) * tz;
            const float J00 = cam.fx / tz, J02 = -(cam.fx * cx_) / (tz * tz);
            const float J11 = cam.fy / tz, J12 = -(cam.fy * cy_) / (tz * tz);
            const float T00 = J00 * m[0] + J02 * m[2], T01 = J00 * m[4] + J02 * m[6], T02 = J00 * m[8] + J02 * m[10];
            const float T10 = J11 * m[1] + J12 * m[2], T11 = J11 * m[5] + J12 * m[6], T12 = J11 * m[9] + J12 * m[10];
            float k00, k01, k11, det;
            if (has_cov) {
                const float c0 = s_cov[tid * 6], c1 = s_cov[tid * 6 + 1], c2 = s_cov[tid * 6 + 2];
                const float c3 = s_cov[tid * 6 + 3], c4 = s_cov[tid * 6 + 4], c5 = s_cov[tid * 6 + 5];
                const float v00 = (c0 * T00 + c1 * T01) + c2 * T02;
                const float v01 = (c1 * T00 + c3 * T01) + c4 * T02;
                const float v02 = (c2 * T00 + c4 * T01) + c5 * T02;
                const float v10 = (c0 * T10 + c1 * T11) + c2 * T12;
                const float v11 = (c1 * T10 + c3 * T11) + c4 * T12;
                const float v12 = (c2 * T10 + c4 * T11) + c5 * T12;
                k00 = ((T00 * v00 + T01 * v01) + T02 * v02) + 0.3f;
                k01 = (T10 * v00 + T11 * v01) + T12 * v02;
                k11 = ((T10 * v10 + T11 * v11) + T12 * v12) + 0.3f;
                det = k00 * k11 - k01 * k01;
            } else {
                const float sx = cam.mod * s_scale[tid * 3], sy = cam.mod * s_scale[tid * 3 + 1], sz = cam.mod * s_scale[tid * 3 + 2];
                const float4 rq = reinterpret_cast<const float4*>(s_rot)[tid];
                const float r = rq.x, x = rq.y, y = rq.z, z = rq.w;
                const float R00 = 1.0f - 2.0f * (y * y + z * z), R01 = 2.0f * (x * y - r * z), R02 = 2.0f * (x * z + r * y);
                const float R10 = 2.0f * (x * y + r * z), R11 = 1.0f - 2.0f * (x * x + z * z), R12 = 2.0f * (y * z - r * x);
                const float R20 = 2.0f * (x * z - r * y), R21 = 2.0f * (y * z + r * x), R22 = 1.0f - 2.0f * (x * x + y * y);
                const float M00 = R00 * sx, M01 = R01 * sy, M02 = R02 * sz;
                const float M10 = R10 * sx, M11 = R11 * sy, M12 = R12 * sz;
                const float M20 = R20 * sx, M21 = R21 * sy, M22 = R22 * sz;
                const float a10 = (T00 * M00 + T01 * M10) + T02 * M20, a11 = (T00 * M01 + T01 * M11) + T02 * M21, a12 = (T00 * M02 + T01 * M12) + T02 * M22;
                const float a20 = (T10 * M00 + T11 * M10) + T12 * M20, a21 = (T10 * M01 + T11 * M11) + T12 * M21, a22 = (T10 * M02 + T11 * M12) + T12 * M22;
                const float n1 = (a10 * a10 + a11 * a11) + a12 * a12, n2 = (a20 * a20 + a21 * a21) + a22 * a22;
                const float xc = a11 * a22 - a12 * a21, yc = a12 * a20 - a10 * a22, zc = a10 * a21 - a11 * a20;
                k00 = n1 + 0.3f;
                k01 = (a10 * a20 + a11 * a21) + a12 * a22;
                k11 = n2 + 0.3f;
                det = (((xc * xc + yc * yc) + zc * zc) + 0.3f * (n1 + n2)) + 0.09f;
            }
            if (det > 0.0f) {
                const float det_inv = 1.0f / det;
                const float mid = 0.5f * (k00 + k11);
                const float sq = sqrtf(fmaxf(0.1f, mid * mid - det));
                const float lam = fmaxf(mid + sq, mid - sq);
                float rf = ceilf(3.0f * sqrtf(lam));
                rf = fminf(rf, 16777216.0f);
                const float pxv = ((ndcx + 1.0f) * (float)cam.Wv - 1.0f) * 0.5f;
                const float pyy = ((ndcy + 1.0f) * (float)cam.H - 1.0f) * 0.5f;
                const int xs = view * cam.gxv;
                const int x0 = clamp_tile((pxv - rf) / 16.0f, cam.gxv) + xs, x1 = clamp_tile(((pxv + rf) + 15.0f) / 16.0f, cam.gxv) + xs;
                const float pxx = cam.V > 1 ? pxv + (float)(xs * kTile) : pxv;
                const int y0 = clamp_tile((pyy - rf) / 16.0f, cam.gy), y1 = clamp_tile(((pyy + rf) + 15.0f) / 16.0f, cam.gy);
                const int area = (x1 - x0) * (y1 - y0);
                float cr, cg, cb;
                if (HAS_SH) { cr = sh_rgb[0]; cg = sh_rgb[1]; cb = sh_rgb[2]; }
                else { cr = s_col[tid * 3]; cg = s_col[tid * 3 + 1]; cb = s_col[tid * 3 + 2]; }
                const float con_a = k11 * det_inv, con_b = -k01 * det_inv, con_c = k00 * det_inv;
                const bool finite = __builtin_isfinite(pxx) && __builtin_isfinite(pyy) && __builtin_isfinite(con_a) && __builtin_isfinite(con_b) &&
                                    __builtin_isfinite(con_c) && __builtin_isfinite(o) && __builtin_isfinite(cr) && __builtin_isfinite(cg) &&
                                    __builtin_isfinite(cb) && __builtin_isfinite(tz);
                if (area > 0 && finite) {
                    radius = (int)rf;
                    ntiles = (uint32_t)area;
                    rc = make_uint2((uint32_t)x0 | ((uint32_t)x1 << 16), (uint32_t)y0 | ((uint32_t)y1 << 16));
                    if (HAS_SH) clampbits = sh_clamp;
                    float ex = -1.0f, ey = -1.0f;
                    const float o255 = o * 255.0f;
                    if (o255 > 1.0f) {
                        const float tau2 = 2.0f * (__logf(o255) + 0.02f);
                        ex = sqrtf(tau2 * k00) + 0.01f;
                        ey = sqrtf(tau2 * k11) + 0.01f;
                    }
                    g0 = make_float4(pxx, pyy, con_a, con_b);
                    g1 = make_float4(con_c, band ? -o : o, cr, cg);
                    g2 = make_float4(cb, tz, ex, ey);
                }
            }
        }
        radii[io] = radius;
        if (radius_out) *radius_out = radius;
        if (ntiles) {
            gp.geom[(size_t)io * 3] = g0; gp.geom[(size_t)io * 3 + 1] = g1; gp.geom[(size_t)io * 3 + 2] = g2;
            gp.rect[io] = rc;
            gp.depth_bits[io] = __float_as_uint(g2.y);
        }
        gp.tiles[io] = ntiles;
        if (HAS_SH && !gp.sh_jac) gp.clamped[io] = clampbits;
    } else if (cam.V > 1) {
        radii[io] = 0;
        gp.geom[(size_t)io * 3] = gp.geom[(size_t)io * 3 + 1] = gp.geom[(size_t)io * 3 + 2] = make_float4(0.f, 0.f, 0.f, 0.f);
        gp.rect[io] = make_uint2(0u, 0u);
        gp.tiles[io] = 0u;
        gp.depth_bits[io] = 0u;
        if (HAS_SH) gp.clamped[io] = 0u;
    }
    return ntiles;
}

__device__ __forceinline__ float activate_staged_rows(const Cam& cam, int tid, bool row, float* s_mean, float* s_scale, float* s_rot, float logit)
{
    const float ls0 = s_scale[cam.act_iso ? tid : tid * 3];
    if (cam.act_iso) __syncthreads();
    if (row) {
        float R[3][3];
        quat_to_rot(cam.act_q, R);
        const float px = s_mean[tid * 3], py = s_mean[tid * 3 + 1], pz = s_mean[tid * 3 + 2];
        s_mean[tid * 3] = R[0][0] * px + R[0][1] * py + R[0][2] * pz + cam.act_t[0];
        s_mean[tid * 3 + 1] = R[1][0] * px + R[1][1] * py + R[1][2] * pz + cam.act_t[1];
        s_mean[tid * 3 + 2] = R[2][0] * px + R[2][1] * py + R[2][2] * pz + cam.act_t[2];
        if (cam.act_iso) {
            const float e = __expf(ls0);
            s_scale[tid * 3] = e; s_scale[tid * 3 + 1] = e; s_scale[tid * 3 + 2] = e;
        } else {
            s_scale[tid * 3] = __expf(ls0); s_scale[tid * 3 + 1] = __expf(s_scale[tid * 3 + 1]); s_scale[tid * 3 + 2] = __expf(s_scale[tid * 3 + 2]);
        }
        const float4 q4 = reinterpret_cast<const float4*>(s_rot)[tid];
        const float q[4] = {q4.x, q4.y, q4.z, q4.w};
        float out[4];
        activate_rotation(cam.act_q, cam.act_iso, q, out);
        reinterpret_cast<float4*>(s_rot)[tid] = make_float4(out[0], out[1], out[2], out[3]);
    }
    return 1.0f / (1.0f + __expf(-logit));
}

template <int SH, bool ACT = false, class CamT = Cam>
__global__ __launch_bounds__(kBlock) void preprocess_forward_kernel(
    typename CamArg<CamT>::type cam, int P, const float* __restrict__ means3D, const float* __restrict__ shs,
    const float* __restrict__ colors, const float* __restrict__ opac, const float* __restrict__ scales,
    const float* __restrict__ rots, const float* __restrict__ cov3Dp, int32_t* __restrict__ radii, GeomPtrs gp)
{
    load_device_pose(cam);
    constexpr bool HAS_SH = SH != 0;
    constexpr bool SLAB = SH == 1;
    constexpr int kGeoFloats = kBlock * 7, kColFloats = SLAB ? 0 : kBlock * 3;
    constexpr int kSlabFloats = SLAB ? (kBlock / kWave) * kShHalf * kShPad : 0;
    constexpr int kPoolFloats = (kGeoFloats + kColFloats) > kSlabFloats ? (kGeoFloats + kColFloats) : kSlabFloats;
    __shared__ __attribute__((aligned(16))) float s_mean[kBlock * 3];
    __shared__ __attribute__((aligned(16))) float s_pool[kPoolFloats];
    __shared__ uint32_t s_wsum[kBlock / kWave];
    float* const s_scale = s_pool;
    float* const s_rot = s_pool + kBlock * 3;
    float* const s_cov = s_pool;
    float* const s_col = s_pool + kGeoFloats;
    float* const s_sh = s_pool;

    const int tid = threadIdx.x;
    const int vbase = blockIdx.x * kBlock;
    const int view = cam.V > 1 ? (int)blockIdx.x / cam.nbv : 0;
    const int base = (cam.V > 1 ? (int)blockIdx.x - view * cam.nbv : (int)blockIdx.x) * kBlock;
    const int nrows = max(0, min(kBlock, P - base));
    if (vbase + tid < cam.gx * cam.gy) gp.tile_total[vbase + tid] = 0u;
    const int i = base + tid, io = vbase + tid;
    float o_in = i < P ? opac[i] : 0.0f;
    stage_rows<3>(s_mean, means3D, base, nrows, tid);
    if (!SLAB) {
        if (cov3Dp) stage_rows<6>(s_cov, cov3Dp, base, nrows, tid);
        else {
            if (ACT && cam.act_iso) stage_rows<1>(s_scale, scales, base, nrows, tid); else stage_rows<3>(s_scale, scales, base, nrows, tid);
            stage_rows<4>(s_rot, rots, base, nrows, tid);
        }
        if (SH == 0) stage_rows<3>(s_col, colors, base, nrows, tid);
    }
    __syncthreads();
    constexpr bool BAND = std::is_same<CamT, CamBand>::value;
    bool in_band = false;
    if constexpr (BAND) {
        const float up = -s_mean[tid * 3 + 1];
// ... 206 lines not shown
```

activesplat_amd/csrc/tilebin.hip:

```cpp
#include "gs_common.h"


namespace gs {

template <class F>
__device__ __forceinline__ void expand_wave(const uint32_t* incl_w, const uint32_t* s_x0w, const uint32_t* s_y0,
                                            int wave, int lane, uint32_t total, int gx, F f)
{
    for (uint32_t t0 = 0; t0 < total; t0 += kWave) {
        const uint32_t t = t0 + lane;
        if (t < total) {
            int lo = 0, hi = 63;
#pragma unroll
            for (int s = 0; s < 6; s++) {
                const int mid = (lo + hi) >> 1;
                if (incl_w[mid] > t) hi = mid; else lo = mid + 1;
            }
            const int j = wave * kWave + lo;
            const uint32_t k = t - (lo ? incl_w[lo - 1] : 0u);
            const uint32_t xw = s_x0w[j];
            const uint32_t w = xw >> 16, x0 = xw & 0xffffu;
            const uint32_t tile = (s_y0[j] + k / w) * (uint32_t)gx + x0 + k % w;
            f(tile, j);
        }
    }
}

template <bool SCATTER, int THREADS>
__global__ __launch_bounds__(THREADS) void tile_bin_kernel(Cam cam, int P, GeomPtrs gp, int tiles, int chunk,
                                                          uint32_t* __restrict__ tile_total,
                                                          uint32_t* __restrict__ tile_base,
                                                          const uint2* __restrict__ ranges,
                                                          unsigned long long* __restrict__ pairs, uint32_t cap, int nchunks)
{
    __shared__ uint32_t s_hist[kMaxLdsTiles];
    __shared__ uint32_t s_incl[THREADS];
    __shared__ uint32_t s_x0w[THREADS];
    __shared__ uint32_t s_y0[THREADS];
    __shared__ uint32_t s_depth[THREADS];

    const int tid = threadIdx.x, lane = tid & 63, wave = tid >> 6;
  const int cper = (nchunks + 7) >> 3;
  for (int b = blockIdx.x; b < 8 * cper; b += gridDim.x) {
    const int cid = SCATTER ? (b & 7) * cper + (b >> 3) : b;
    if (cid >= nchunks) continue;
    uint32_t* my_base = tile_base + (size_t)cid * tiles;
    __syncthreads();
    for (int t = tid; t < tiles; t += THREADS) s_hist[t] = SCATTER ? ranges[t].x + my_base[t] : 0u;
    __syncthreads();
    const int cbase = cid * chunk;
    for (int r = 0; r < chunk / THREADS; r++) {
        const int i = cbase + r * THREADS + tid;
        if (cbase + r * THREADS >= P) break;
        uint32_t n = 0, x0 = 0, w = 1, y0 = 0, dbits = 0;
        if (i < P) {
            n = gp.tiles[i];
            if (n) {
                const uint2 rc = gp.rect[i];
                x0 = rc.x & 0xffffu; w = (rc.x >> 16) - x0; y0 = rc.y & 0xffffu;
                if (SCATTER) dbits = gp.depth_bits[i];
            }
        }
        const int gbase = cbase + r * THREADS;
        auto place = [&](uint32_t tile, uint32_t depth_bits, uint32_t id) {
            if (SCATTER) {
                const uint32_t slot = atomicAdd(&s_hist[tile], 1u);
                if (slot < cap) pairs[slot] = ((unsigned long long)depth_bits << 32) | id;
            } else {
                atomicAdd(&s_hist[tile], 1u);
            }
        };
        if (!__any(n > 16u)) {
            uint32_t kx = 0, ky = 0;
            for (uint32_t k = 0; __any(k < n); k++) {
                if (k < n) {
                    place((y0 + ky) * (uint32_t)cam.gx + x0 + kx, dbits, (uint32_t)i);
                    if (++kx == w) { kx = 0; ++ky; }
                }
            }
            continue;
        }
        if (n) {
            s_x0w[tid] = x0 | (w << 16);
            s_y0[tid] = y0;
            if (SCATTER) s_depth[tid] = dbits;
        }
        const uint32_t incl = wave_inclusive_scan(n, lane);
        s_incl[tid] = incl;
        const uint32_t total = __shfl(incl, 63);
        __builtin_amdgcn_wave_barrier();
        expand_wave(s_incl + wave * kWave, s_x0w, s_y0, wave, lane, total, cam.gx, [&](uint32_t tile, int j) {
            place(tile, SCATTER ? s_depth[j] : 0u, (uint32_t)(gbase + j));
        });
        __builtin_amdgcn_wave_barrier();
    }
    if (!SCATTER) {
        __syncthreads();
        for (int t = tid; t < tiles; t += THREADS) my_base[t] = s_hist[t];
    }
  }
}

template <int TW>
__global__ __launch_bounds__(1024) void tile_colscan_kernel(uint32_t* __restrict__ base, int chunks, int tiles, uint32_t* __restrict__ tile_total)
{
    constexpr int SEG = 1024 / TW;
    __shared__ uint32_t s_sum[SEG][TW + 1];
    const int l = threadIdx.x % TW, sgm = threadIdx.x / TW;
    const int ngroups = (tiles + TW - 1) / TW, gper = (ngroups + 7) >> 3;
    const int grp = (int)(blockIdx.x & 7) * gper + (int)(blockIdx.x >> 3);
    const int t = ((int)(blockIdx.x >> 3) < gper && grp < ngroups) ? grp * TW + l : tiles;
    const int L = (chunks + SEG - 1) / SEG, r0 = min(chunks, sgm * L), r1 = min(chunks, r0 + L);
    uint32_t sum = 0;
    if (t < tiles) {
#pragma unroll 8
        for (int r = r0; r < r1; r++) sum += base[(size_t)r * tiles + t];
    }
    s_sum[sgm][l] = sum;
    __syncthreads();
    uint32_t run = 0;
    for (int q = 0; q < sgm; q++) run += s_sum[q][l];
    if (t < tiles) {
#pragma unroll 8
        for (int r = r0; r < r1; r++) {
            const size_t idx = (size_t)r * tiles + t;
            const uint32_t v = base[idx];
            base[idx] = run;
            run += v;
        }
        if (sgm == SEG - 1) tile_total[t] = run;
    }
}

constexpr int kScanPerThreadMax = 8;
__global__ __launch_bounds__(1024) void tile_scan_kernel(const uint32_t* __restrict__ tile_total, int tiles,
                                                         uint2* __restrict__ ranges, uint32_t* __restrict__ counts,
                                                         uint32_t* __restrict__ host_counts)
{
    __shared__ uint32_t s_w[16];
    __shared__ uint32_t s_m[16];
    const int tid = threadIdx.x, lane = tid & 63, wave = tid >> 6;
    const int per = (tiles + 1023) >> 10, t0 = tid * per;
    uint32_t v[kScanPerThreadMax];
    uint32_t sum = 0, vmax = 0;
#pragma unroll
    for (int k = 0; k < kScanPerThreadMax; k++) {
        v[k] = (k < per && t0 + k < tiles) ? tile_total[t0 + k] : 0u;
        sum += v[k];
        vmax = max(vmax, v[k]);
    }
    const uint32_t inc = wave_inclusive_scan(sum, lane);
#pragma unroll
    for (int m = 32; m >= 1; m >>= 1) vmax = max(vmax, (uint32_t)__shfl_xor(vmax, m));
    if (lane == 63) { s_w[wave] = inc; s_m[wave] = vmax; }
    __syncthreads();
    uint32_t start = inc - sum, total = 0, mx = 0;
    for (int w = 0; w < 16; w++) {
        if (w < wave) start += s_w[w];
        total += s_w[w];
        mx = max(mx, s_m[w]);
    }
#pragma unroll
    for (int k = 0; k < kScanPerThreadMax; k++) {
        if (k < per && t0 + k < tiles) ranges[t0 + k] = make_uint2(start, start + v[k]);
        start += v[k];
    }
    if (tid == 0) {
        counts[0] = total; counts[1] = mx;
        if (host_counts) { host_counts[0] = total; host_counts[1] = mx; }
    }
}

#ifndef GS_MIN_F64
#define GS_MIN_F64(a, b) ({ double r_; asm("v_min_f64 %0, %1, %2" : "=v"(r_) : "v"(a), "v"(b)); r_; })
#define GS_MAX_F64(a, b) ({ double r_; asm("v_max_f64 %0, %1, %2" : "=v"(r_) : "v"(a), "v"(b)); r_; })
// ... 26 lines not shown
    const unsigned long long b = __builtin_bit_cast(unsigned long long, v);
    const uint32_t lo = lane_xor_u32<M>((uint32_t)b), hi = lane_xor_u32<M>((uint32_t)(b >> 32));
    return __builtin_bit_cast(double, ((unsigned long long)hi << 32) | lo);
}

template <int E, int THREADS>
__device__ __forceinline__ void bitonic_sort_block(double (&v)[E], double* buf, int tid)
{
    const uint32_t base = (uint32_t)tid * E;
    uint32_t neg = 0u;
#define GS_DOMAIN(want_neg)                                                      \
    {                                                                            \
        const uint32_t w_ = (want_neg) ? 0x80000000u : 0u, m_ = w_ ^ neg;        \
        _Pragma("unroll") for (int i = 0; i < E; i++) v[i] = f64_flip(v[i], m_); \
        neg = w_;                                                                \
    }
#define GS_SORT2(a, b)                                      \
    {                                                       \
        const double mn_ = GS_MIN_F64(a, b), mx_ = GS_MAX_F64(a, b); \
        a = mn_; b = mx_;                                   \
    }
#pragma unroll
    for (int kk = 2; kk <= E; kk <<= 1) {
        if (kk == E) GS_DOMAIN((base & (uint32_t)E) != 0u)
#pragma unroll
        for (int j = kk >> 1; j > 0; j >>= 1) {
#pragma unroll
            for (int i = 0; i < E; i++) {
                if ((i & j) != 0) continue;
                if (kk == E || (i & kk) == 0) GS_SORT2(v[i], v[i | j])
                else GS_SORT2(v[i | j], v[i])
            }
        }
    }
    for (uint32_t kk = 2 * E; kk <= (uint32_t)E * THREADS; kk <<= 1) {
        const bool up = (base & kk) == 0;
        for (uint32_t j = kk >> 1; j >= (uint32_t)E; j >>= 1) {
            const int m = (int)(j / E);
            const bool lower = (tid & m) == 0;
            GS_DOMAIN(lower != up)
            double p[E];
            switch (m) {
#define GS_CASE(M) case M: _Pragma("unroll") for (int i = 0; i < E; i++) p[i] = lane_xor_f64<M>(v[i]); break;
                GS_CASE(1) GS_CASE(2) GS_CASE(4) GS_CASE(8)
#undef GS_CASE
                case 16: case 32:
                    __builtin_amdgcn_wave_barrier();
#pragma unroll
                    for (int i = 0; i < E; i++) buf[i * THREADS + tid] = v[i];
                    __builtin_amdgcn_wave_barrier();
#pragma unroll
                    for (int i = 0; i < E; i++) p[i] = buf[i * THREADS + (tid ^ m)];
                    __builtin_amdgcn_wave_barrier();
                    break;
                default:
                    __syncthreads();
#pragma unroll
                    for (int i = 0; i < E; i++) buf[i * THREADS + tid] = v[i];
                    __syncthreads();
#pragma unroll
                    for (int i = 0; i < E; i++) p[i] = buf[i * THREADS + (tid ^ m)];
                    __syncthreads();
            }
#pragma unroll
            for (int i = 0; i < E; i++) v[i] = GS_MIN_F64(v[i], f64_flip(p[i], 0x80000000u));
        }
        GS_DOMAIN(!up)
#pragma unroll
        for (int j = E >> 1; j > 0; j >>= 1) {
#pragma unroll
            for (int i = 0; i < E; i++) {
                if ((i & j) == 0) GS_SORT2(v[i], v[i | j])
            }
        }
    }
    GS_DOMAIN(false)
#undef GS_DOMAIN
#undef GS_SORT2
}

template <int E, int THREADS>
__device__ __forceinline__ void tile_sort_impl(const uint2 range, uint32_t n, const unsigned long long* pairs,
                                               unsigned long long* pairs_out, uint32_t* __restrict__ point_list,
                                               unsigned long long* buf, int tid)
{
    double k[E];
    const uint32_t base = (uint32_t)tid * E;
#pragma unroll
    for (int i = 0; i < E; i++) {
        const uint32_t e = (uint32_t)i * THREADS + tid;
        k[i] = key_to_f64(e < n ? pairs[range.x + e] : kPadKey);
    }
    bitonic_sort_block<E, THREADS>(k, reinterpret_cast<double*>(buf), tid);
    __syncthreads();
#pragma unroll
    for (int i = 0; i < E; i++) buf[base + i] = f64_to_key(k[i]);
    __syncthreads();
#pragma unroll
    for (int i = 0; i < E; i++) {
        const uint32_t e = (uint32_t)i * THREADS + tid;
        if (e < n) {
            const unsigned long long v = buf[e];
            pairs_out[range.x + e] = v;
            point_list[range.x + e] = (uint32_t)v;
        }
    }
}

template <int CAP, int THREADS>
__global__ __launch_bounds__(THREADS) void tile_sort_kernel(const uint2* __restrict__ ranges,
                                                             const unsigned long long* pairs, unsigned long long* pairs_out,
                                                             uint32_t* __restrict__ point_list, uint32_t cap, uint32_t skip_le)
{
    __shared__ unsigned long long s_a[CAP];
    const int tid = threadIdx.x;
    uint2 range = ranges[blockIdx.x];
    range.x = min(range.x, cap); range.y = min(range.y, cap);
    const uint32_t start = blockIdx.y * (uint32_t)CAP;
    if (range.y - range.x <= start || range.y - range.x <= skip_le) return;
    range.x += start;
    const uint32_t n = min(range.y - range.x, (uint32_t)CAP);
    constexpr int EMAX = CAP / THREADS;
    if (n <= (uint32_t)THREADS * (EMAX / 4)) tile_sort_impl<EMAX / 4, THREADS>(range, n, pairs, pairs_out, point_list, s_a, tid);
    else if (n <= (uint32_t)THREADS * (EMAX / 2)) tile_sort_impl<EMAX / 2, THREADS>(range, n, pairs, pairs_out, point_list, s_a, tid);
    else tile_sort_impl<EMAX, THREADS>(range, n, pairs, pairs_out, point_list, s_a, tid);
}

constexpr int kBucketCap = 5632;
constexpr int kBuckets = 2048;
constexpr int kBucketThreads = 512;
constexpr int kBucketRankMax = 64;
constexpr int kBucketThreadsBig = 1024;
constexpr int kBucketCapBig = 11 * kBucketThreadsBig;
constexpr int kBucketsBig = 4096;

template <int E, int T, int NB, int CAP>
__device__ __forceinline__ void bucket_sort_impl(const uint2 range, uint32_t n, const unsigned long long* __restrict__ pairs,
                                                 uint32_t* __restrict__ point_list, unsigned long long* s_keys, uint32_t* s_cnt, uint16_t* s_off,
                                                 float* s_redf, uint32_t* s_redu, int tid)
{
    const int lane = tid & 63, wave = tid >> 6;
    unsigned long long k[E];
    float zmin = 3.0e38f, zmax = 0.0f;
#pragma unroll
    for (int i = 0; i < E; i++) {
        const uint32_t e = (uint32_t)i * T + tid;
        k[i] = e < n ? pairs[range.x + e] : kPadKey;
        if (e < n) {
            const float z = __uint_as_float((uint32_t)(k[i] >> 32));
            zmin = fminf(zmin, z); zmax = fmaxf(zmax, z);
        }
    }
    const int nbins = n <= (uint32_t)NB / 2 ? NB / 4 : (n <= (uint32_t)(NB + NB / 4) ? NB / 2 : NB);
    for (int b = tid; b < nbins / 2; b += T) s_cnt[b] = 0u;
#pragma unroll
    for (int m = 32; m >= 1; m >>= 1) { zmin = fminf(zmin, __shfl_xor(zmin, m)); zmax = fmaxf(zmax, __shfl_xor(zmax, m)); }
    if (lane == 0) { s_redf[wave] = zmin; s_redf[T / kWave + wave] = zmax; }
    __syncthreads();
    float zlo = s_redf[0], zhi = s_redf[T / kWave];
#pragma unroll
    for (int w = 1; w < T / kWave; w++) { zlo = fminf(zlo, s_redf[w]); zhi = fmaxf(zhi, s_redf[T / kWave + w]); }
    const float span = zhi - zlo;
    const float scale = span > 0.0f ? (float)nbins / span : 0.0f;
    const uint32_t last_bin = (uint32_t)nbins - 1u;
#define GS_BIN(key) min(last_bin, (uint32_t)((__uint_as_float((uint32_t)((key) >> 32)) - zlo) * scale))
    uint32_t arr[(E + 1) / 2];
#pragma unroll
    for (int i = 0; i < E; i++) {
        const uint32_t e = (uint32_t)i * T + tid;
        if ((i & 1) == 0) arr[i >> 1] = 0u;
        if (e < n) {
            const uint32_t b = GS_BIN(k[i]);
            const uint32_t sh = (b & 1u) * 16u;
            arr[i >> 1] |= ((atomicAdd(&s_cnt[b >> 1], 1u << sh) >> sh) & 0xffffu) << (16 * (i & 1));
        }
    }
    __syncthreads();
    constexpr int PB = NB / T;
    static_assert(PB % 2 == 0, "a thread scans whole counter words");
    uint32_t c[PB], sum = 0, cmax = 0;
#pragma unroll
    for (int j = 0; j < PB; j++) { c[j] = tid * PB < nbins ? (s_cnt[(tid * PB + j) >> 1] >> (16 * (j & 1))) & 0xffffu : 0u; sum += c[j]; cmax = max(cmax, c[j]); }
    const uint32_t incl = wave_inclusive_scan(sum, lane);
#pragma unroll
    for (int m = 32; m >= 1; m >>= 1) cmax = max(cmax, (uint32_t)__shfl_xor(cmax, m));
    if (lane == 63) s_redu[wave] = incl;
    if (lane == 0) s_redu[T / kWave + wave] = cmax;
    __syncthreads();
    uint32_t run = incl - sum, fullest = 0;
#pragma unroll
    for (int w = 0; w < T / kWave; w++) { if (w < wave) run += s_redu[w]; fullest = max(fullest, s_redu[T / kWave + w]); }
    if (tid * PB < nbins) {
#pragma unroll
        for (int j = 0; j < PB; j++) { s_off[tid * PB + j] = (uint16_t)run; run += c[j]; }
        if (tid * PB + PB == nbins) s_off[nbins] = (uint16_t)run;
    }
    __syncthreads();
    if (fullest <= (uint32_t)kBucketRankMax) {
#pragma unroll
        for (int i = 0; i < E; i++) {
            const uint32_t e = (uint32_t)i * T + tid;
            if (e < n) s_keys[s_off[GS_BIN(k[i])] + ((arr[i >> 1] >> (16 * (i & 1))) & 0xffffu)] = k[i];
        }
        __syncthreads();
#pragma unroll
        for (int i = 0; i < E; i++) {
            const uint32_t p = (uint32_t)i * T + tid;
            if (p < n) {
                const unsigned long long key = s_keys[p];
                const uint32_t b = GS_BIN(key);
                const uint32_t lo = s_off[b], hi = s_off[b + 1];
                uint32_t rank = lo;
                for (uint32_t j = lo; j < hi; j++) rank += s_keys[j] < key ? 1u : 0u;
                point_list[range.x + rank] = (uint32_t)key;
            }
        }
        return;
    }
#undef GS_BIN
    constexpr int EA = E > 8 ? 8 : E;
    double va[EA];
#pragma unroll
    for (int i = 0; i < EA; i++) va[i] = key_to_f64(k[i]);
    bitonic_sort_block<EA, T>(va, reinterpret_cast<double*>(s_keys), tid);
    const uint32_t nA = min(n, (uint32_t)(EA * T));
    if (E <= 8) {
        __syncthreads();
#pragma unroll
        for (int i = 0; i < EA; i++) s_keys[(uint32_t)tid * EA + i] = f64_to_key(va[i]);
        __syncthreads();
        for (uint32_t e = tid; e < n; e += T) {
            const unsigned long long v = s_keys[e];
            point_list[range.x + e] = (uint32_t)v;
        }
        return;
    }
    constexpr int EB = 4;
    static_assert(CAP <= (8 + EB) * T && E <= 8 + EB, "run B holds the keys beyond run A");
    double vb[EB];
#pragma unroll
    for (int i = 0; i < EB; i++) vb[i] = key_to_f64((EA + i) < E ? k[(EA + i) < E ? (EA + i) : 0] : kPadKey);
    __syncthreads();
    bitonic_sort_block<EB, T>(vb, reinterpret_cast<double*>(s_keys), tid);
    __syncthreads();
#pragma unroll
    for (int i = 0; i < EA; i++) s_keys[(uint32_t)tid * EA + i] = f64_to_key(va[i]);
#pragma unroll
    for (int i = 0; i < EB; i++) if ((uint32_t)(EA * T + tid * EB + i) < (uint32_t)CAP) s_keys[EA * T + (uint32_t)tid * EB + i] = f64_to_key(vb[i]);
    __syncthreads();
    const uint32_t nB = n - nA;
    for (uint32_t e = tid; e < n; e += T) {
        const bool in_a = e < nA;
        const unsigned long long key = in_a ? s_keys[e] : s_keys[EA * T + (e - nA)];
        const uint32_t base = in_a ? (uint32_t)(EA * T) : 0u, len = in_a ? nB : nA;
        uint32_t lo = 0, hi = len;
        while (lo < hi) {
            const uint32_t mid = (lo + hi) >> 1;
            if (s_keys[base + mid] < key) lo = mid + 1; else hi = mid;
        }
        const uint32_t rank = (in_a ? e : e - nA) + lo;
        point_list[range.x + rank] = (uint32_t)key;
    }
}

template <bool BIG>
__global__ __launch_bounds__(BIG ? kBucketThreadsBig : kBucketThreads, BIG ? 4 : 6) void tile_bucket_sort_kernel(
    const uint2* __restrict__ ranges, const unsigned long long* __restrict__ pairs, uint32_t* __restrict__ point_list, uint32_t cap)
{
    constexpr int T = BIG ? kBucketThreadsBig : kBucketThreads, NB = BIG ? kBucketsBig : kBuckets, CAP = BIG ? kBucketCapBig : kBucketCap;
    __shared__ unsigned long long s_keys[CAP];
    __shared__ uint32_t s_cnt[NB / 2];
    __shared__ uint16_t s_off[NB + 2];
    __shared__ float s_redf[2 * T / kWave];
    __shared__ uint32_t s_redu[2 * T / kWave];
    const int tid = threadIdx.x;
    uint2 range = ranges[blockIdx.x];
    range.x = min(range.x, cap); range.y = min(range.y, cap);
    const uint32_t n = range.y - range.x;
    if (n == 0 || n > (uint32_t)CAP || (BIG && n <= (uint32_t)kBucketCap)) return;
    if (BIG) { bucket_sort_impl<11, T, NB, CAP>(range, n, pairs, point_list, s_keys, s_cnt, s_off, s_redf, s_redu, tid); return; }
    if (n <= 2u * T) bucket_sort_impl<2, T, NB, CAP>(range, n, pairs, point_list, s_keys, s_cnt, s_off, s_redf, s_redu, tid);
    else if (n <= 4u * T) bucket_sort_impl<4, T, NB, CAP>(range, n, pairs, point_list, s_keys, s_cnt, s_off, s_redf, s_redu, tid);
    else if (n <= 8u * T) bucket_sort_impl<8, T, NB, CAP>(range, n, pairs, point_list, s_keys, s_cnt, s_off, s_redf, s_redu, tid);
    else bucket_sort_impl<11, T, NB, CAP>(range, n, pairs, point_list, s_keys, s_cnt, s_off, s_redf, s_redu, tid);
}

template <int CAP, int CHUNK, int THREADS>
__global__ __launch_bounds__(THREADS) void tile_merge_kernel(const uint2* __restrict__ ranges,
                                                              unsigned long long* __restrict__ pairs,
                                                              uint32_t* __restrict__ point_list, uint32_t cap, uint32_t skip_le)
{
    __shared__ unsigned long long s_k[CAP];
    const int tid = threadIdx.x;
    uint2 range = ranges[blockIdx.x];
    range.x = min(range.x, cap); range.y = min(range.y, cap);
    const uint32_t n = range.y - range.x;
    if (n <= (uint32_t)CHUNK || n > (uint32_t)CAP || n <= skip_le) return;
    for (uint32_t i = tid; i < n; i += THREADS) s_k[i] = pairs[range.x + i];
    __syncthreads();
    const uint32_t nruns = (n + CHUNK - 1) / CHUNK;
    for (uint32_t i = tid; i < n; i += THREADS) {
        const unsigned long long key = s_k[i];
        const uint32_t own = i / CHUNK;
        uint32_t rank = i - own * CHUNK;
        for (uint32_t r = 0; r < nruns; r++) {
            if (r == own) continue;
            const uint32_t b0 = r * CHUNK, len = min((uint32_t)CHUNK, n - b0);
            uint32_t lo = 0, hi = len;
            while (lo < hi) {
                const uint32_t mid = (lo + hi) >> 1;
                if (s_k[b0 + mid] < key) lo = mid + 1; else hi = mid;
            }
            rank += lo;
        }
        pairs[range.x + rank] = key;
        point_list[range.x + rank] = (uint32_t)key;
    }
}

template <int OUT, int THREADS>
__global__ __launch_bounds__(THREADS) void tile_merge_pass_kernel(const uint2* __restrict__ ranges, const unsigned long long* __restrict__ src,
                                                                   unsigned long long* __restrict__ dst, uint32_t* __restrict__ point_list,
                                                                   uint32_t run, uint32_t cap)
{
    __shared__ unsigned long long s_in[OUT];
    __shared__ unsigned long long s_out[OUT];
    __shared__ uint32_t s_split[2];
    const int tid = threadIdx.x;
    uint2 range = ranges[blockIdx.x];
    range.x = min(range.x, cap); range.y = min(range.y, cap);
    const uint32_t n = range.y - range.x;
    const uint32_t o0 = blockIdx.y * (uint32_t)OUT;
    if (o0 >= n) return;
    const uint32_t o1 = min(n, o0 + (uint32_t)OUT);
    const uint32_t pair0 = o0 / (2u * run) * (2u * run);
    const uint32_t lenA = min(run, n - pair0), lenB = min(run, n - pair0 - lenA);
    const unsigned long long* A = src + range.x + pair0;
    const unsigned long long* B = A + lenA;
    if (tid < 2 * kWave) {
        const int lane = tid & (kWave - 1);
        const uint32_t d = (tid < kWave ? o0 : o1) - pair0;
        uint32_t lo = d > lenB ? d - lenB : 0u, hi = min(d, lenA);
        while (lo < hi) {
            const uint32_t span = hi - lo;
            const uint32_t q = lo + (uint32_t)(((uint64_t)span * (uint32_t)lane) >> 6);
            const int c = (int)__popcll(__ballot(A[q] < B[d - 1 - q]));
            const uint32_t q_prev = lo + (uint32_t)(((uint64_t)span * (uint32_t)max(c - 1, 0)) >> 6);
            const uint32_t q_c = lo + (uint32_t)(((uint64_t)span * (uint32_t)min(c, kWave - 1)) >> 6);
            if (c == 0) hi = lo;
            else if (c == kWave) lo = q_prev + 1;
            else { lo = q_prev + 1; hi = q_c; }
        }
        if (lane == 0) s_split[tid / kWave] = lo;
    }
    __syncthreads();
    const uint32_t d0 = o0 - pair0, d1 = o1 - pair0;
    const uint32_t a0 = s_split[0], a1 = s_split[1], b0 = d0 - a0, b1 = d1 - a1;
    const uint32_t na = a1 - a0, nb = b1 - b0, m = na + nb;
    for (uint32_t i = tid; i < m; i += THREADS) s_in[i] = i < na ? A[a0 + i] : B[b0 + (i - na)];
    __syncthreads();
    for (uint32_t i = tid; i < m; i += THREADS) {
        const unsigned long long key = s_in[i];
        const bool in_a = i < na;
        const uint32_t base = in_a ? na : 0u, len = in_a ? nb : na;
        uint32_t lo = 0, hi = len;
        while (lo < hi) {
            const uint32_t mid = (lo + hi) >> 1;
            if (s_in[base + mid] < key) lo = mid + 1; else hi = mid;
        }
        s_out[(in_a ? i : i - na) + lo] = key;
    }
    __syncthreads();
    for (uint32_t i = tid; i < m; i += THREADS) {
        const unsigned long long key = s_out[i];
        dst[range.x + o0 + i] = key;
        if (point_list) point_list[range.x + o0 + i] = (uint32_t)key;
    }
}

static void bin_config(int P, int& threads, int& chunk)
{
    (void)P;
    threads = 1024; chunk = kBinChunk;
}

template <bool SCATTER>
static void launch_bin(int threads, int nb, hipStream_t st, Cam cam, int P, GeomPtrs gp, int tiles, int chunk,
                       uint32_t* tile_total, uint32_t* tile_base, const uint2* ranges, unsigned long long* pairs, uint32_t cap)
{
    const int nchunks = nb;
    nb = 8 * ((nb + 7) / 8);
    hipLaunchKernelGGL((tile_bin_kernel<SCATTER, 1024>), dim3(nb), dim3(1024), 0, st, cam, P, gp, tiles, chunk, tile_total, tile_base, ranges, pairs, cap, nchunks);
}

hipError_t launch_tile_count(const Cam& cam, int P, GeomPtrs gp, uint32_t* tile_total, uint32_t* tile_base,
                             uint2* ranges, uint32_t* d_counts, uint32_t* host_counts, hipStream_t st)
{
    const int tiles = cam.gx * cam.gy;
    int threads, chunk; bin_config(P, threads, chunk);
    const int nb = (P + chunk - 1) / chunk;
    if (nb > 0) launch_bin<false>(threads, nb, st, cam, P, gp, tiles, chunk, tile_total, tile_base, nullptr, nullptr, 0u);
    hipLaunchKernelGGL(tile_colscan_kernel<16>, dim3(8 * (((tiles + 15) / 16 + 7) / 8)), dim3(1024), 0, st, tile_base, nb, tiles, tile_total);
    hipLaunchKernelGGL(tile_scan_kernel, dim3(1), dim3(1024), 0, st, tile_total, tiles, ranges, d_counts, host_counts);
    return hipGetLastError();
}

hipError_t launch_tile_scatter_sort(const Cam& cam, int P, GeomPtrs gp, uint32_t* tile_base, const uint2* ranges,
                                    uint32_t max_tile_instances, unsigned long long* pairs, unsigned long long* pairs_alt,
                                    uint32_t* point_list, uint32_t cap, hipStream_t st)
{
    const int tiles = cam.gx * cam.gy;
    int threads, chunk; bin_config(P, threads, chunk);
    const int nb = (P + chunk - 1) / chunk;
    if (nb > 0) launch_bin<true>(threads, nb, st, cam, P, gp, tiles, chunk, nullptr, tile_base, ranges, pairs, cap);
    constexpr int kBigChunk = 2 * kSortChunk;
    const bool big = max_tile_instances > (uint32_t)kBucketCap && max_tile_instances <= (uint32_t)kSortCapMax && tiles <= 512;
    const uint32_t skip_le = max_tile_instances <= (uint32_t)kSortCapMax ? (uint32_t)(big ? kBucketCapBig : kBucketCap) : 0u;
    if (skip_le) {
        hipLaunchKernelGGL(tile_bucket_sort_kernel<false>, dim3(tiles), dim3(kBucketThreads), 0, st, ranges, pairs, point_list, cap);
        if (max_tile_instances <= (uint32_t)kBucketCap) return hipGetLastError();
        if (big) {
            hipLaunchKernelGGL(tile_bucket_sort_kernel<true>, dim3(tiles), dim3(kBucketThreadsBig), 0, st, ranges, pairs, point_list, cap);
            if (max_tile_instances <= (uint32_t)kBucketCapBig) return hipGetLastError();
        }
    }
    if (max_tile_instances <= (uint32_t)kSortChunk) {
        hipLaunchKernelGGL((tile_sort_kernel<kSortChunk, 256>), dim3(tiles, 1), dim3(256), 0, st, ranges, pairs, pairs, point_list, cap, 0u);
        return hipGetLastError();
    }
    const unsigned chunks = (max_tile_instances + kBigChunk - 1) / kBigChunk;
    if (max_tile_instances <= (uint32_t)kSortCapMax) {
        hipLaunchKernelGGL((tile_sort_kernel<kBigChunk, 256>), dim3(tiles, chunks), dim3(256), 0, st, ranges, pairs, pairs, point_list, cap, skip_le);
        if (max_tile_instances > 8192)
            hipLaunchKernelGGL((tile_merge_kernel<kSortCapMax, kBigChunk, 1024>), dim3(tiles), dim3(1024), 0, st, ranges, pairs, point_list, cap, skip_le);
        else if (max_tile_instances > (uint32_t)kBigChunk)
            hipLaunchKernelGGL((tile_merge_kernel<8192, kBigChunk, 1024>), dim3(tiles), dim3(1024), 0, st, ranges, pairs, point_list, cap, skip_le);
        return hipGetLastError();
    }
    constexpr int kOut = kSortChunk;
    int passes = 0;
    for (uint64_t r = kBigChunk; r < max_tile_instances; r <<= 1) passes++;
    unsigned long long* cur = (passes & 1) ? pairs_alt : pairs;
    hipLaunchKernelGGL((tile_sort_kernel<kBigChunk, 256>), dim3(tiles, chunks), dim3(256), 0, st, ranges, pairs, cur, point_list, cap, 0u);
    const unsigned blocks = (max_tile_instances + kOut - 1) / kOut;
    uint64_t r = kBigChunk;
    for (int p = 0; p < passes; p++, r <<= 1) {
        unsigned long long* nxt = cur == pairs ? pairs_alt : pairs;
        hipLaunchKernelGGL((tile_merge_pass_kernel<kOut, 256>), dim3(tiles, blocks), dim3(256), 0, st, ranges, cur, nxt,
                           p == passes - 1 ? point_list : nullptr, (uint32_t)r, cap);
        cur = nxt;
    }
    return hipGetLastError();
}

}
```

include/gsplat_hip.h:

```cpp
#ifndef GSPLAT_HIP_H
#define GSPLAT_HIP_H

#include <stddef.h>
#include <stdint.h>

#ifdef __cplusplus
extern "C" {
#endif

#define GS_OK 0
#define GS_EINVAL 1
#define GS_ELAUNCH 2
#define GS_ECAPACITY 3

#define GS_TILE 16
#define GS_GEOM_FLOATS 12

typedef void* gs_stream_t;

typedef struct GsCamera {
    int32_t image_width;
    int32_t image_height;
    int32_t sh_degree;
    int32_t sh_coeffs;
    float tanfovx;
    float tanfovy;
    float scale_modifier;
    int32_t num_views;
    const float* bg;
    const float* viewmatrix;
    const float* projmatrix;
    const float* campos;
} GsCamera;

typedef struct GsGeomLayout {
    uint64_t total_bytes;
    uint64_t geom;
    uint64_t rect;
    uint64_t tiles_touched;
    uint64_t offsets;
    uint64_t block_sums;
    uint64_t clamped;
    uint64_t tile_total;
    uint64_t tile_base;
    uint64_t sh_jac;
    uint64_t depth_bits;
} GsGeomLayout;

typedef struct GsImageLayout {
    uint64_t total_bytes;
    uint64_t ranges;
    uint64_t final_T;
    uint64_t n_contrib;
    uint64_t split_state;
} GsImageLayout;

#define GS_SORT_AUTO 0
#define GS_SORT_TILE_LDS 1
#define GS_SORT_RADIX 2

typedef struct GsBinLayout {
    uint64_t total_bytes;
    uint64_t path;
    uint64_t pairs;
    uint64_t keys_unsorted;
    uint64_t vals_unsorted;
    uint64_t keys_sorted;
    uint64_t sort_temp;
    uint64_t segments;
    uint64_t seg_T;
    uint64_t pairs_alt;
} GsBinLayout;

int gs_atlas_layout(int32_t P, int32_t view_width, int32_t num_views, int32_t* virtual_P, int32_t* atlas_width, int32_t* view_stride);
int gs_geom_layout(int32_t P, int32_t width, int32_t height, GsGeomLayout* out);
int gs_image_layout(int32_t width, int32_t height, GsImageLayout* out);
int gs_bin_layout(int64_t D, uint32_t max_tile_instances, int32_t width, int32_t height, GsBinLayout* out);
int gs_set_sort_path(int32_t path);
int gs_set_forward_segments(int32_t on);
int gs_set_half_quadrants(int32_t max_tiles);
int gs_set_backward_chain(int32_t pieces, int32_t min_tiles);
int gs_set_backward_chain_tickets(int32_t on);
int gs_set_backward_chain_polls(int32_t polls);
int gs_set_forward_priority(int32_t mode, float param);
int gs_async_status_word(uint32_t** host_word);
int gs_async_status_clear(void);
int gs_recorded_cut(uint32_t target, uint32_t* nearest, int32_t* level);
int gs_set_backward_segments(int32_t segments);
uint64_t gs_backward_scratch_bytes(int32_t P);

const char* gs_last_error(void);
const char* gs_version(void);
#define GS_ABI_VERSION 22
int32_t gs_abi_version(void);

int gs_profile_enable(int32_t on);
int32_t gs_profile_stage_count(void);
const char* gs_profile_stage_name(int32_t stage);
int gs_profile_collect(float* ms_sum, int32_t* calls, int32_t n_stages);

int gs_preprocess_forward(const GsCamera* cam, int32_t P,
                          const float* means3D, const float* shs, const float* colors_precomp,
                          const float* opacities, const float* scales, const float* rotations,
                          const float* cov3D_precomp,
                          int32_t* radii, void* geom_state, void* image_state, uint32_t* d_counts,
                          uint32_t* h_counts, int32_t want_backward, gs_stream_t stream);

int gs_render_forward(const GsCamera* cam, int32_t P, int64_t D, uint32_t max_tile_instances,
                      void* geom_state, void* bin_state, uint32_t* point_list, void* image_state,
                      float* out_color, float* out_depth, float* out_opacity, float* out_depth_sq,
                      void* backward_scratch, gs_stream_t stream);

int gs_render_backward(const GsCamera* cam, int32_t P, int64_t D,
                       const float* means3D, const float* shs, const float* colors_precomp,
                       const float* scales, const float* rotations, const float* cov3D_precomp,
                       const int32_t* radii, const void* geom_state, const uint32_t* point_list,
                       const void* image_state, const float* dL_dcolor, const float* dL_ddepth,
                       float* dL_dmeans2D, float* dL_dmeans3D, float* dL_dopacities,
                       float* dL_dcolors_precomp, float* dL_dshs, float* dL_dscales,
                       float* dL_drotations, float* dL_dcov3D, void* scratch, int32_t scratch_zeroed,
                       int32_t have_sh_jacobian, gs_stream_t stream);

int gs_preprocess_forward_raw(const GsCamera* cam, int32_t P, const float* means3D, const float* shs, const float* colors_precomp,
                              const float* logit_opacities, const float* log_scales, const float* unnorm_rotations,
                              const float* h_pose7, int32_t isotropic, float* max_2D_radius, uint8_t* seen, int32_t* radii, void* geom_state,
                              void* image_state, uint32_t* d_counts, uint32_t* h_counts, int32_t want_backward, gs_stream_t stream);
int gs_render_backward_raw(const GsCamera* cam, int32_t P, int64_t D, const float* means3D, const float* shs, const float* colors_precomp,
                           const float* logit_opacities, const float* log_scales, const float* unnorm_rotations, const float* h_pose7,
                           int32_t isotropic, int32_t accumulate, const int32_t* radii, const void* geom_state, const uint32_t* point_list,
                           const void* image_state, const float* dL_dcolor, const float* dL_ddepth, float* dL_dmeans2D, float* dL_dmeans3D,
                           float* dL_dlogit_opacities, float* dL_dcolors_precomp, float* dL_dshs, float* dL_dlog_scales,
                           float* dL_dunnorm_rotations, void* scratch, int32_t scratch_zeroed, int32_t have_sh_jacobian, gs_stream_t stream);

uint64_t gs_pose_grad_scratch_bytes(int32_t P);
int gs_render_backward_raw_pose(const GsCamera* cam, int32_t P, int64_t D, const float* means3D, const float* shs, const float* colors_precomp,
                                const float* logit_opacities, const float* log_scales, const float* unnorm_rotations, const float* h_pose7,
                                int32_t isotropic, int32_t accumulate, const int32_t* radii, const void* geom_state, const uint32_t* point_list,
                                const void* image_state, const float* dL_dcolor, const float* dL_ddepth, float* dL_dmeans2D, float* dL_dmeans3D,
                                float* dL_dlogit_opacities, float* dL_dcolors_precomp, float* dL_dshs, float* dL_dlog_scales,
                                float* dL_dunnorm_rotations, void* scratch, int32_t scratch_zeroed, int32_t have_sh_jacobian, int32_t pose_only,
                                float* dL_dpose7, void* pose_scratch, gs_stream_t stream);

int gs_adam_step(int64_t n, float* param, const float* grad, float* exp_avg, float* exp_avg_sq,
                 double lr, double beta1, double beta2, double eps, int32_t step, gs_stream_t stream);

typedef struct GsAdamTensor {
    int64_t n;
    float* param;
    const float* grad;
    float* exp_avg;
    float* exp_avg_sq;
    double lr, beta1, beta2, eps;
    int32_t step;
    int32_t reserved;
} GsAdamTensor;
int gs_adam_step_multi(int32_t count, const GsAdamTensor* tensors, gs_stream_t stream);

int gs_render_backward_raw_adam(const GsCamera* cam, int32_t P, int64_t D, const float* means3D, const float* shs, const float* colors_precomp,
                                const float* logit_opacities, const float* log_scales, const float* unnorm_rotations, const float* h_pose7,
                                int32_t isotropic, const int32_t* radii, const void* geom_state, const uint32_t* point_list,
                                const void* image_state, const float* dL_dcolor, const float* dL_ddepth, float* dL_dmeans2D, void* scratch,
                                int32_t scratch_zeroed, int32_t have_sh_jacobian, const GsAdamTensor* adam5, gs_stream_t stream);

typedef struct GsRowTensor {
    float* param;
    float* exp_avg;
    float* exp_avg_sq;
    const float* grad;
    double lr, beta1, beta2, eps;
    int32_t width;
    int32_t step;
} GsRowTensor;
int gs_pack_columns(int32_t count, const GsRowTensor* tensors, int64_t n, int64_t n_padded, float* flat, gs_stream_t stream);
int gs_adam_rows(int32_t count, const GsRowTensor* tensors, int64_t row_lo, int64_t n_valid, int64_t n_rows, const float* grad_shard,
                 float* out_shard, gs_stream_t stream);
int gs_unpack_columns(int32_t count, const GsRowTensor* tensors, int64_t n, const float* flat, gs_stream_t stream);
// ... 172 lines not shown
```

Before: 1505 frames/s.

## Pack per-quadrant coverage masks into sort keys to skip non-overlapping splats in forward blend

Binning now packs per-quadrant cell coverage bits into the sort keys, with a key shift chosen from P, and the sort kernels extract ids through that shift. After sorting, the forward blend reads per-quadrant 64-bit mask words from the pairs buffer. It compacts only the list entries that touch its quadrant into a per-wave LDS ring, then walks that compacted stream with prefetching. This targets geom loads and scan work on splats that cannot affect a quadrant, at the cost of extra ring bookkeeping, wave barriers and more key-packing work in binning and sort. The feature is on by default and can be turned off with a new toggle.

```diff
diff --git a/activesplat_amd/_lib.py b/activesplat_amd/_lib.py
--- a/activesplat_amd/_lib.py
+++ b/activesplat_amd/_lib.py
@@ -63,7 +63,7 @@
 SORT_AUTO, SORT_TILE_LDS, SORT_RADIX = 0, 1, 2
 
 
-ABI_VERSION = 22
+ABI_VERSION = 23
 
 vp, i32, u32, i64, u64, f32, f64, cint = C.c_void_p, C.c_int32, C.c_uint32, C.c_int64, C.c_uint64, C.c_float, C.c_double, C.c_int
 
@@ -79,6 +79,7 @@
     "gs_set_backward_chain_tickets": (cint, [i32]),
     "gs_set_backward_chain_polls": (cint, [i32]),
     "gs_set_forward_priority": (cint, [i32, f32]),
+    "gs_set_quadrant_masks": (cint, [i32]),
     "gs_async_status_word": (cint, [C.POINTER(C.POINTER(u32))]),
     "gs_async_status_clear": (cint, []),
     "gs_recorded_cut": (cint, [u32, C.POINTER(u32), C.POINTER(i32)]),
diff --git a/activesplat_amd/csrc/api.hip b/activesplat_amd/csrc/api.hip
--- a/activesplat_amd/csrc/api.hip
+++ b/activesplat_amd/csrc/api.hip
@@ -200,6 +200,12 @@
     if (mode < 0) { mode = gs::kFwdPrioDefault; param = gs::kFwdPrioDefaultParam; }
     gs::g_fwd_prio_param = param > 0.0f ? param : 0.0f;
     gs::g_fwd_prio = mode;
+    return GS_OK;
+}
+
+int gs_set_quadrant_masks(int32_t on)
+{
+    gs::g_quad_masks = on != 0;
     return GS_OK;
 }
 
@@ -535,11 +541,13 @@
     GsBinLayout BL; gs_bin_layout(D, max_tile_instances, k.W, k.H, &BL);
     char* bb = (char*)bin_state;
     if (int rc = bin_tile_lists("gs_render_forward", k, P, D, max_tile_instances, gp, ranges, BL, bb, point_list, st)) return rc;
+    const unsigned long long* mask_words = (BL.path == GS_SORT_TILE_LDS && D > 0 && max_tile_instances <= (uint32_t)gs::kSortCapMax && gs::key_shift_for(P))
+                                               ? (const unsigned long long*)(bb + BL.pairs) : nullptr;
     ScopedStage ps(ST_BLEND_FWD, st);
     return launched("gs_render_forward", "blend", gs::launch_blend_forward(k, ranges, point_list, gp.geom, out_color, out_depth, out_opacity,
                     (float*)(ib + IL.final_T), (uint32_t*)(ib + IL.n_contrib), out_depth_sq, BL.path == GS_SORT_TILE_LDS ? (uint32_t)D : 0xffffffffu,
                     (int)BL.segments, BL.segments > 1 ? (float*)(bb + BL.seg_T) : nullptr, (float*)(ib + IL.split_state), (uint32_t)P,
-                    (float*)backward_scratch, st));
+                    (float*)backward_scratch, mask_words, st));
 }
 
 int gs_preprocess_forward_topdown(const GsCamera* cam, int32_t P, const float* means3D, const float* colors_precomp, const float* logit_opacities,
diff --git a/activesplat_amd/csrc/blend.hip b/activesplat_amd/csrc/blend.hip
--- a/activesplat_amd/csrc/blend.hip
+++ b/activesplat_amd/csrc/blend.hip
@@ -59,12 +59,12 @@
     return {make_float4(q0.x, q0.y, -0.5f * kLog2e * q0.z, -kLog2e * q0.w), -0.5f * kLog2e * q1.x};
 }
 __device__ __forceinline__ void stage_record(float4* s0, float4* s1, float4* s2, int lane, const float4& q0,
-                                             const float4& q1, const float4& q2, uint32_t id)
+                                             const float4& q1, const float4& q2, uint32_t id, uint32_t after = 0u)
 {
     const StagedConic k = staged_conic(q0, q1);
     s0[lane] = k.s0;
     s1[lane] = make_float4(k.c, q1.y, q1.z, q1.w);
-    s2[lane] = make_float4(q2.x, q2.y, __uint_as_float(id), 0.0f);
+    s2[lane] = make_float4(q2.x, q2.y, __uint_as_float(id), __uint_as_float(after));
 }
 
 struct SplatAlpha { float alpha, p, G; bool hit; };
@@ -189,6 +189,24 @@
     else if (level == 1) __builtin_amdgcn_s_setprio(1);
     else __builtin_amdgcn_s_setprio(0);
 }
+__device__ __forceinline__ int walk_priority_level(const Cam& cam, uint32_t at, uint32_t n, bool done, float T)
+{
+    const float chunks = (float)(at >> 6);
+    const float p = cam.fwd_prio_param;
+    if (cam.fwd_prio == kFwdPrioChunk)
+        return (chunks >= p ? 1 : 0) + (chunks >= 2.0f * p ? 1 : 0) + (chunks >= 3.0f * p ? 1 : 0);
+    float t1 = p, t2 = p * p, t3 = p * p * p;
+    if (cam.fwd_prio == kFwdPrioDecay) {
+        constexpr float kLog2Tmin = -13.287712f;
+        t1 = __builtin_amdgcn_exp2f(kLog2Tmin * chunks * __builtin_amdgcn_rcpf(chunks + p));
+        t2 = __builtin_amdgcn_exp2f(kLog2Tmin * chunks * __builtin_amdgcn_rcpf(chunks + 2.0f * p));
+        t3 = __builtin_amdgcn_exp2f(kLog2Tmin * chunks * __builtin_amdgcn_rcpf(chunks + 4.0f * p));
+    }
+    const int level = (__ballot(!done && T > t1) != 0ull ? 1 : 0) + (__ballot(!done && T > t2) != 0ull ? 1 : 0) + (__ballot(!done && T > t3) != 0ull ? 1 : 0);
+    const uint32_t left = (n - at) >> 6;
+    return min(level, (left > kFwdPrioListChunks ? 1 : 0) + (left > 2u * kFwdPrioListChunks ? 1 : 0) + (left > 3u * kFwdPrioListChunks ? 1 : 0));
+}
+constexpr int kFwdRing = 128;
 constexpr int kRoundSlack = 4;
 
 template <bool DEPTH_SQ, int NS, int SEG, int NW>
@@ -197,11 +215,12 @@
     const float4* __restrict__ geom, float* __restrict__ out_color, float* __restrict__ out_depth,
     float* __restrict__ out_opacity, float* __restrict__ final_T, uint32_t* __restrict__ n_contrib,
     float* __restrict__ out_depth_sq, uint32_t cap, float* __restrict__ seg_T, float* __restrict__ split_state, uint32_t P,
-    float4* __restrict__ zero_fill)
+    float4* __restrict__ zero_fill, const unsigned long long* __restrict__ mask_words)
 {
     static_assert(NS == 4 && kWave / NS == 16, "the scan tests the four 4x4 blocks of a quadrant");
     __shared__ float4 s_rec[NW][3][kWave + 1];
     __shared__ __attribute__((aligned(16))) uint8_t s_list[NW][4 * kWave + 16];
+    __shared__ uint32_t s_ring[SEG == 0 ? NW : 1][SEG == 0 ? kFwdRing : 1];
     const int tid = threadIdx.x, lane = tid & 63, wave = tid >> 6;
     GradFill fill = grad_fill_start(SEG == 0 ? zero_fill : nullptr, P, tid);
     TileCtx c;
@@ -248,7 +267,94 @@
     const bool stopped_at_entry = SEG == 2 && T < kTmin;
     bool done = !inside || stopped_at_entry;
 
-    if (SEG == 1 || !__all(done)) {
+    if (SEG == 0 && n != 0u && !__all(done)) {
+        uint32_t* ring = s_ring[wave];
+        const uint32_t nu = (uint32_t)__builtin_amdgcn_readfirstlane((int)n);
+        const bool use_words = mask_words != nullptr && list_has_mask_words(nu);
+        const unsigned long long* words = mask_words + (size_t)__builtin_amdgcn_readfirstlane((int)(range.x + (uint32_t)c.quad * ((nu + 63u) >> 6)));
+        uint32_t lbase = 0u, head = 0u, tail = 0u;
+        auto queue_chunks = [&]() {
+            while (tail - head < (uint32_t)kWave && lbase < nu) {
+                fill = grad_fill_step(zero_fill, fill, NW * kWave);
+                unsigned long long w = use_words ? words[lbase >> 6] : ~0ull;
+                w = ((unsigned long long)(uint32_t)__builtin_amdgcn_readfirstlane((int)(uint32_t)(w >> 32)) << 32) |
+                    (unsigned long long)(uint32_t)__builtin_amdgcn_readfirstlane((int)(uint32_t)w);
+                if (nu - lbase < (uint32_t)kWave) w &= (1ull << (nu - lbase)) - 1ull;
+                const uint32_t rank = __builtin_amdgcn_mbcnt_hi((uint32_t)(w >> 32), __builtin_amdgcn_mbcnt_lo((uint32_t)w, 0u));
+                if (__builtin_amdgcn_inverse_ballot_w64(w)) ring[(tail + rank) & (uint32_t)(kFwdRing - 1)] = lbase + (uint32_t)lane + 1u;
+                tail += (uint32_t)__popcll(w);
+                lbase += kWave;
+            }
+        };
+        auto pop_chunk = [&](uint32_t& after) -> uint32_t {
+            __builtin_amdgcn_wave_barrier();
+            const uint32_t cnt = min((uint32_t)kWave, tail - head);
+            after = 0u;
+            if ((uint32_t)lane < cnt) after = ring[(head + (uint32_t)lane) & (uint32_t)(kFwdRing - 1)];
+            head += cnt;
+            __builtin_amdgcn_wave_barrier();
+            return cnt;
+        };
+        auto load_id = [&](uint32_t after) -> uint32_t { return list[max(after, 1u) - 1u]; };
+        uint32_t after_next, after_next2;
+        queue_chunks();
+        uint32_t cnt_next = pop_chunk(after_next);
+        uint32_t idl_next = load_id(after_next);
+        queue_chunks();
+        uint32_t cnt_next2 = pop_chunk(after_next2);
+        uint32_t idl_next2 = load_id(after_next2);
+        uint32_t id_next = (after_next != 0u && idl_next < P) ? idl_next : kNoId;
+        float4 r0, r1, r2;
+        {
+            const float4* gr = geom + (size_t)(id_next != kNoId ? id_next : 0u) * 3;
+            r0 = gr[0]; r1 = gr[1]; r2 = gr[2];
+        }
+        while (cnt_next != 0u) {
+            if (cam.fwd_prio != kFwdPrioOff)
+                set_wave_priority(walk_priority_level(cam, (uint32_t)__builtin_amdgcn_readfirstlane((int)after_next) - 1u, nu, done, T));
+            const float4 q0 = r0, q1 = r1, q2 = r2;
+            const uint32_t id_cur = id_next, after_cur = after_next;
+            cnt_next = cnt_next2; after_next = after_next2;
+            id_next = (after_next != 0u && idl_next2 < P) ? idl_next2 : kNoId;
+            if (cnt_next != 0u) {
+                const float4* gr = geom + (size_t)(id_next != kNoId ? id_next : 0u) * 3;
+                r0 = gr[0]; r1 = gr[1]; r2 = gr[2];
+            }
+            queue_chunks();
+            cnt_next2 = pop_chunk(after_next2);
+            idl_next2 = load_id(after_next2);
+            const unsigned long long going = ~__ballot(done);
+            unsigned long long m_any, mb[4];
+            scan_going_blocks(q0, q2, id_cur != kNoId, c.qx0, c.qy0, going, m_any, mb);
+            if (m_any == 0ull) continue;
+            stage_record(s0, s1, s2, lane, q0, q1, q2, id_cur, after_cur);
+            const int ntrips = build_stream_lists(s_list[wave], mb, lane);
+            __builtin_amdgcn_wave_barrier();
+            uint32_t jj2_next = *reinterpret_cast<const uint16_t*>(my_list);
+            for (int t = 0; t < ntrips; t += 2) {
+                const uint32_t jj2 = jj2_next;
+                jj2_next = *reinterpret_cast<const uint16_t*>(my_list + t + 2);
+                const int jj[2] = {(int)(jj2 & 0xffu), (int)(jj2 >> 8)};
+                float4 a0[2], a1[2], a2[2];
+#pragma unroll
+                for (int u = 0; u < 2; u++) { a0[u] = s0[jj[u]]; a1[u] = s1[jj[u]]; a2[u] = s2[jj[u]]; }
+#pragma unroll
+                for (int u = 0; u < 2; u++) {
+                    const SplatAlpha a = splat_alpha(a0[u], a1[u].x, a1[u].y, pxf, pyf);
+                    const Composite k = composite_step(T, done, a.alpha, a.hit);
+                    T = k.T; done = k.done;
+                    C0 += a1[u].z * k.w; C1 += a1[u].w * k.w; C2 += a2[u].x * k.w; Dp += a2[u].y * k.w;
+                    if (DEPTH_SQ) Dq += a2[u].y * a2[u].y * k.w;
+                    last = k.ok ? __float_as_uint(a2[u].w) : last;
+                }
+                if (__all(done)) break;
+            }
+            __builtin_amdgcn_wave_barrier();
+            if (__all(done)) break;
+        }
+        if (cam.fwd_prio != kFwdPrioOff) __builtin_amdgcn_s_setprio(0);
+    }
+    if (SEG != 0 && (SEG == 1 || !__all(done))) {
         uint32_t id_next = first + (uint32_t)lane < n ? list[first + lane] : kNoId;
         uint32_t id_next2 = first + (uint32_t)lane + 64u < n ? list[first + lane + 64] : kNoId;
         if (id_next >= P) id_next = kNoId;
@@ -259,28 +365,6 @@
             r0 = gr[0]; r1 = gr[1]; r2 = gr[2];
         }
         for (uint32_t base = first; base < n; base += kWave) {
-            if (SEG == 0) fill = grad_fill_step(zero_fill, fill, NW * kWave);
-            if (SEG == 0 && cam.fwd_prio != kFwdPrioOff) {
-                const float chunks = (float)((base - first) >> 6);
-                const float p = cam.fwd_prio_param;
-                int level;
-                if (cam.fwd_prio == kFwdPrioChunk) {
-                    level = (chunks >= p ? 1 : 0) + (chunks >= 2.0f * p ? 1 : 0) + (chunks >= 3.0f * p ? 1 : 0);
-                } else {
-                    float t1 = p, t2 = p * p, t3 = p * p * p;
-                    if (cam.fwd_prio == kFwdPrioDecay) {
-                        constexpr float kLog2Tmin = -13.287712f;
-                        t1 = __builtin_amdgcn_exp2f(kLog2Tmin * chunks * __builtin_amdgcn_rcpf(chunks + p));
-                        t2 = __builtin_amdgcn_exp2f(kLog2Tmin * chunks * __builtin_amdgcn_rcpf(chunks + 2.0f * p));
-                        t3 = __builtin_amdgcn_exp2f(kLog2Tmin * chunks * __builtin_amdgcn_rcpf(chunks + 4.0f * p));
-                    }
-                    level = (__ballot(!done && T > t1) != 0ull ? 1 : 0) + (__ballot(!done && T > t2) != 0ull ? 1 : 0) +
-                            (__ballot(!done && T > t3) != 0ull ? 1 : 0);
-                    const uint32_t left = (n - base) >> 6;
-                    level = min(level, (left > kFwdPrioListChunks ? 1 : 0) + (left > 2u * kFwdPrioListChunks ? 1 : 0) + (left > 3u * kFwdPrioListChunks ? 1 : 0));
-                }
-                set_wave_priority(level);
-            }
             const float4 q0 = r0, q1 = r1, q2 = r2;
             const uint32_t id_cur = id_next;
             id_next = id_next2;
@@ -326,7 +410,6 @@
             if (SEG != 1 && __all(done)) break;
             if (SEG == 1 && __all(!inside || T < kTmin)) break;
         }
-        if (SEG == 0 && cam.fwd_prio != kFwdPrioOff) __builtin_amdgcn_s_setprio(0);
     }
     if (SEG == 0) grad_fill_rest(zero_fill, fill, NW * kWave);
     if (SEG == 1) {
@@ -985,6 +1068,7 @@
 std::atomic<int> g_chain_polls{kChainPollsDefault};
 std::atomic<int> g_fwd_prio{kFwdPrioDefault};
 std::atomic<float> g_fwd_prio_param{kFwdPrioDefaultParam};
+std::atomic<int> g_quad_masks{1};
 uint32_t* g_async_status_dev = nullptr;
 uint32_t* g_chain_fail_dev = nullptr;
 int g_chain_fail_device = -1;
@@ -1002,7 +1086,7 @@
 hipError_t launch_blend_forward(const Cam& cam_in, const uint2* ranges, const uint32_t* point_list, const float4* geom,
                                 float* out_color, float* out_depth, float* out_opacity, float* final_T,
                                 uint32_t* n_contrib, float* out_depth_sq, uint32_t cap, int segments, float* seg_T, float* split_state, uint32_t P,
-                                float* zero_fill, hipStream_t st)
+                                float* zero_fill, const unsigned long long* mask_words, hipStream_t st)
 {
     Cam cam = cam_in;
     const int k_half = g_half_quadrant_tiles.load(std::memory_order_relaxed), k_fseg = g_few_segments.load(std::memory_order_relaxed);
@@ -1012,10 +1096,11 @@
     cam.fwd_prio = g_fwd_prio.load(std::memory_order_relaxed);
     cam.fwd_prio_param = g_fwd_prio_param.load(std::memory_order_relaxed);
     if (!(cam.fwd_prio_param > 0.0f)) cam.fwd_prio_param = fwd_prio_default_param(cam.fwd_prio);
+    if (!g_quad_masks.load(std::memory_order_relaxed)) mask_words = nullptr;
     const int nb = ((cam.gx * cam.gy + 7) >> 3) << 3;
 #define GS_FWD(DSQ, SEG, GRID)                                                                                                     \
     hipLaunchKernelGGL((blend_forward_streams_kernel<DSQ, kFwdStreams, SEG, 4>), GRID, dim3(kBlock), 0, st, cam, ranges, point_list, geom, \
-                       out_color, out_depth, out_opacity, final_T, n_contrib, out_depth_sq, cap, seg_T, split_state, P, (float4*)zero_fill)
+                       out_color, out_depth, out_opacity, final_T, n_contrib, out_depth_sq, cap, seg_T, split_state, P, (float4*)zero_fill, mask_words)
     const size_t HW = (size_t)cam.W * cam.H;
     if (segments > 1 && seg_T) {
         hipError_t e = zero_fill ? hipMemsetAsync(zero_fill, 0, (size_t)P * kGradStride * sizeof(float), st) : hipSuccess;
diff --git a/activesplat_amd/csrc/gs_common.h b/activesplat_amd/csrc/gs_common.h
--- a/activesplat_amd/csrc/gs_common.h
+++ b/activesplat_amd/csrc/gs_common.h
@@ -176,6 +176,20 @@
 
 #ifndef GS_WAIT_VMEM
 #define GS_WAIT_VMEM() asm volatile("s_waitcnt vmcnt(0)" ::: "memory")
+#endif
+#ifndef GS_OPAQUE_UNIFORM_PTR
+#if defined(__HIP_DEVICE_COMPILE__)
+#define GS_OPAQUE_UNIFORM_PTR(p) asm volatile("" : "+s"(p))
+#else
+#define GS_OPAQUE_UNIFORM_PTR(p) ((void)0)
+#endif
+#endif
+#ifndef GS_SCHED_BARRIER
+#if defined(__HIP__) || defined(__HIPCC__)
+#define GS_SCHED_BARRIER() __builtin_amdgcn_sched_barrier(0)
+#else
+#define GS_SCHED_BARRIER() ((void)0)
+#endif
 #endif
 
 __device__ __forceinline__ float wave_sum(float v)
@@ -631,6 +645,40 @@
 
 template <class CamT>
 hipError_t launch_preprocess_forward(const CamT& cam, int P, const GaussianInputs& in, int32_t* radii, GeomPtrs gp, hipStream_t st);
+constexpr uint32_t kQuadCellsNone = 0x000000ffu;
+__host__ __device__ inline int quad_cell_of(float v)
+{
+    return (int)fminf(fmaxf(v, -1.0e9f), 1.0e9f) >> 2;
+}
+__host__ __device__ inline uint32_t quad_cells(float x, float y, float ex, float ey, uint32_t rect_x, uint32_t rect_y)
+{
+    if (!(ex >= 0.0f) || !(ey >= 0.0f)) return kQuadCellsNone;
+    const float xl = x - ex, xh = x + ex, yl = y - ey, yh = y + ey;
+    if (!(xl <= xh) || !(yl <= yh)) return kQuadCellsNone;
+    const int cx0 = 4 * (int)(rect_x & 0xffffu), cy0 = 4 * (int)(rect_y & 0xffffu);
+    const int xlo = quad_cell_of(ceilf(xl)) - cx0, xhi = quad_cell_of(floorf(xh)) - cx0;
+    const int ylo = quad_cell_of(ceilf(yl)) - cy0, yhi = quad_cell_of(floorf(yh)) - cy0;
+    if (xhi < 0 || yhi < 0 || xlo > xhi || ylo > yhi) return kQuadCellsNone;
+    const uint32_t a = (uint32_t)min(max(xlo, 0), 255), b = (uint32_t)min(xhi, 255), c = (uint32_t)min(max(ylo, 0), 255), d = (uint32_t)min(yhi, 255);
+    return a | (b << 8) | (c << 16) | (d << 24);
+}
+__host__ __device__ inline uint32_t quad_mask(uint32_t cells, uint32_t kx, uint32_t ky)
+{
+    const uint32_t xlo = cells & 0xffu, xh8 = (cells >> 8) & 0xffu, ylo = (cells >> 16) & 0xffu, yh8 = cells >> 24;
+    const uint32_t xhi = xh8 == 255u ? 0x7fffffffu : xh8, yhi = yh8 == 255u ? 0x7fffffffu : yh8;
+    const uint32_t cx = 4u * kx, cy = 4u * ky;
+    const uint32_t hx0 = (xlo <= cx + 1u && xhi >= cx) ? 1u : 0u, hx1 = (xlo <= cx + 3u && xhi >= cx + 2u) ? 1u : 0u;
+    const uint32_t hy0 = (ylo <= cy + 1u && yhi >= cy) ? 1u : 0u, hy1 = (ylo <= cy + 3u && yhi >= cy + 2u) ? 1u : 0u;
+    return (hx0 & hy0) | ((hx1 & hy0) << 1) | ((hx0 & hy1) << 2) | ((hx1 & hy1) << 3);
+}
+constexpr int kKeyMaskBits = 4;
+__host__ __device__ inline int key_shift_for(int64_t P) { return P <= ((int64_t)1 << (32 - kKeyMaskBits)) ? kKeyMaskBits : 0; }
+__host__ __device__ inline uint32_t key_id(unsigned long long key, int shift) { return (uint32_t)key >> shift; }
+constexpr int kBucketCap = 5632;
+__host__ __device__ inline bool list_has_mask_words(uint32_t n) { return n >= 4u && n <= (uint32_t)kBucketCap; }
+__host__ __device__ inline uint32_t mask_word_index(uint32_t n, uint32_t chunk, uint32_t quad) { return quad * ((n + 63u) >> 6) + chunk; }
+extern std::atomic<int> g_quad_masks;
+
 hipError_t launch_scan_block_sums(int P, GeomPtrs gp, uint32_t* d_total, hipStream_t st);
 template <class CamT>
 hipError_t launch_preprocess_backward(const CamT& cam, int P, const GaussianBackward& g, const PoseRequest& pose, hipStream_t st);
@@ -707,7 +755,7 @@
 hipError_t launch_blend_forward(const Cam& cam, const uint2* ranges, const uint32_t* point_list, const float4* geom,
                                 float* out_color, float* out_depth, float* out_opacity, float* final_T,
                                 uint32_t* n_contrib, float* out_depth_sq, uint32_t cap, int segments, float* seg_T, float* split_state, uint32_t P, float* zero_fill,
-                                hipStream_t st);
+                                const unsigned long long* mask_words, hipStream_t st);
 hipError_t launch_blend_topdown(const Cam& cam, const uint2* ranges, const uint32_t* point_list, const float4* geom, float* free_opacity,
                                 uint8_t* free_binary, uint8_t* visible_rgb, uint8_t* visible_binary, uint32_t cap, uint32_t P, hipStream_t st);
 hipError_t launch_blend_backward(const Cam& cam, const uint2* ranges, const uint32_t* point_list, const float4* geom, const float* split_state,
diff --git a/activesplat_amd/csrc/preprocess.hip b/activesplat_amd/csrc/preprocess.hip
--- a/activesplat_amd/csrc/preprocess.hip
+++ b/activesplat_amd/csrc/preprocess.hip
@@ -45,6 +45,8 @@
 {
     uint32_t ntiles = 0;
     if (radius_out) *radius_out = 0;
+    uint32_t* cells_out = gp.offsets;
+    GS_OPAQUE_UNIFORM_PTR(cells_out);
     if (i < P) {
         const float* m = cam.view + 16 * view;
         const float* q = cam.proj + 16 * view;
@@ -148,6 +150,7 @@
             gp.geom[(size_t)io * 3] = g0; gp.geom[(size_t)io * 3 + 1] = g1; gp.geom[(size_t)io * 3 + 2] = g2;
             gp.rect[io] = rc;
             gp.depth_bits[io] = __float_as_uint(g2.y);
+            cells_out[io] = quad_cells(g0.x, g0.y, g2.z, g2.w, rc.x, rc.y);
         }
         gp.tiles[io] = ntiles;
         if (HAS_SH && !gp.sh_jac) gp.clamped[io] = clampbits;
diff --git a/activesplat_amd/csrc/tilebin.hip b/activesplat_amd/csrc/tilebin.hip
--- a/activesplat_amd/csrc/tilebin.hip
+++ b/activesplat_amd/csrc/tilebin.hip
@@ -20,8 +20,9 @@
             const uint32_t k = t - (lo ? incl_w[lo - 1] : 0u);
             const uint32_t xw = s_x0w[j];
             const uint32_t w = xw >> 16, x0 = xw & 0xffffu;
-            const uint32_t tile = (s_y0[j] + k / w) * (uint32_t)gx + x0 + k % w;
-            f(tile, j);
+            const uint32_t ky = k / w, kx = k - ky * w;
+            const uint32_t tile = (s_y0[j] + ky) * (uint32_t)gx + x0 + kx;
+            f(tile, j, kx, ky);
         }
     }
 }
@@ -31,13 +32,14 @@
                                                           uint32_t* __restrict__ tile_total,
                                                           uint32_t* __restrict__ tile_base,
                                                           const uint2* __restrict__ ranges,
-                                                          unsigned long long* __restrict__ pairs, uint32_t cap, int nchunks)
+                                                          unsigned long long* __restrict__ pairs, uint32_t cap, int nchunks, int key_shift)
 {
     __shared__ uint32_t s_hist[kMaxLdsTiles];
     __shared__ uint32_t s_incl[THREADS];
     __shared__ uint32_t s_x0w[THREADS];
     __shared__ uint32_t s_y0[THREADS];
     __shared__ uint32_t s_depth[THREADS];
+    __shared__ uint32_t s_cells[SCATTER ? THREADS : 1];
 
     const int tid = threadIdx.x, lane = tid & 63, wave = tid >> 6;
   const int cper = (nchunks + 7) >> 3;
@@ -52,18 +54,19 @@
     for (int r = 0; r < chunk / THREADS; r++) {
         const int i = cbase + r * THREADS + tid;
         if (cbase + r * THREADS >= P) break;
-        uint32_t n = 0, x0 = 0, w = 1, y0 = 0, dbits = 0;
+        uint32_t n = 0, x0 = 0, w = 1, y0 = 0, dbits = 0, cells = kQuadCellsNone;
         if (i < P) {
             n = gp.tiles[i];
             if (n) {
                 const uint2 rc = gp.rect[i];
                 x0 = rc.x & 0xffffu; w = (rc.x >> 16) - x0; y0 = rc.y & 0xffffu;
-                if (SCATTER) dbits = gp.depth_bits[i];
+                if (SCATTER) { dbits = gp.depth_bits[i]; if (key_shift) cells = gp.offsets[i]; }
             }
         }
         const int gbase = cbase + r * THREADS;
-        auto place = [&](uint32_t tile, uint32_t depth_bits, uint32_t id) {
+        auto place = [&](uint32_t tile, uint32_t depth_bits, uint32_t id, uint32_t cl, uint32_t kx, uint32_t ky) {
             if (SCATTER) {
+                if (key_shift) id = (id << key_shift) | quad_mask(cl, kx, ky);
                 const uint32_t slot = atomicAdd(&s_hist[tile], 1u);
                 if (slot < cap) pairs[slot] = ((unsigned long long)depth_bits << 32) | id;
             } else {
@@ -74,7 +77,7 @@
             uint32_t kx = 0, ky = 0;
             for (uint32_t k = 0; __any(k < n); k++) {
                 if (k < n) {
-                    place((y0 + ky) * (uint32_t)cam.gx + x0 + kx, dbits, (uint32_t)i);
+                    place((y0 + ky) * (uint32_t)cam.gx + x0 + kx, dbits, (uint32_t)i, cells, kx, ky);
                     if (++kx == w) { kx = 0; ++ky; }
                 }
             }
@@ -83,14 +86,14 @@
         if (n) {
             s_x0w[tid] = x0 | (w << 16);
             s_y0[tid] = y0;
-            if (SCATTER) s_depth[tid] = dbits;
+            if (SCATTER) { s_depth[tid] = dbits; s_cells[tid] = cells; }
         }
         const uint32_t incl = wave_inclusive_scan(n, lane);
         s_incl[tid] = incl;
         const uint32_t total = __shfl(incl, 63);
         __builtin_amdgcn_wave_barrier();
-        expand_wave(s_incl + wave * kWave, s_x0w, s_y0, wave, lane, total, cam.gx, [&](uint32_t tile, int j) {
-            place(tile, SCATTER ? s_depth[j] : 0u, (uint32_t)(gbase + j));
+        expand_wave(s_incl + wave * kWave, s_x0w, s_y0, wave, lane, total, cam.gx, [&](uint32_t tile, int j, uint32_t kx, uint32_t ky) {
+            place(tile, SCATTER ? s_depth[j] : 0u, (uint32_t)(gbase + j), SCATTER ? s_cells[j] : 0u, kx, ky);
         });
         __builtin_amdgcn_wave_barrier();
     }
@@ -283,7 +286,7 @@
 template <int E, int THREADS>
 __device__ __forceinline__ void tile_sort_impl(const uint2 range, uint32_t n, const unsigned long long* pairs,
                                                unsigned long long* pairs_out, uint32_t* __restrict__ point_list,
-                                               unsigned long long* buf, int tid)
+                                               unsigned long long* buf, int tid, int key_shift)
 {
     double k[E];
     const uint32_t base = (uint32_t)tid * E;
@@ -303,7 +306,7 @@
         if (e < n) {
             const unsigned long long v = buf[e];
             pairs_out[range.x + e] = v;
-            point_list[range.x + e] = (uint32_t)v;
+            point_list[range.x + e] = key_id(v, key_shift);
         }
     }
 }
@@ -311,7 +314,7 @@
 template <int CAP, int THREADS>
 __global__ __launch_bounds__(THREADS) void tile_sort_kernel(const uint2* __restrict__ ranges,
                                                              const unsigned long long* pairs, unsigned long long* pairs_out,
-                                                             uint32_t* __restrict__ point_list, uint32_t cap, uint32_t skip_le)
+                                                             uint32_t* __restrict__ point_list, uint32_t cap, uint32_t skip_le, int key_shift)
 {
     __shared__ unsigned long long s_a[CAP];
     const int tid = threadIdx.x;
@@ -322,12 +325,11 @@
     range.x += start;
     const uint32_t n = min(range.y - range.x, (uint32_t)CAP);
     constexpr int EMAX = CAP / THREADS;
-    if (n <= (uint32_t)THREADS * (EMAX / 4)) tile_sort_impl<EMAX / 4, THREADS>(range, n, pairs, pairs_out, point_list, s_a, tid);
-    else if (n <= (uint32_t)THREADS * (EMAX / 2)) tile_sort_impl<EMAX / 2, THREADS>(range, n, pairs, pairs_out, point_list, s_a, tid);
-    else tile_sort_impl<EMAX, THREADS>(range, n, pairs, pairs_out, point_list, s_a, tid);
-}
-
-constexpr int kBucketCap = 5632;
+    if (n <= (uint32_t)THREADS * (EMAX / 4)) tile_sort_impl<EMAX / 4, THREADS>(range, n, pairs, pairs_out, point_list, s_a, tid, key_shift);
+    else if (n <= (uint32_t)THREADS * (EMAX / 2)) tile_sort_impl<EMAX / 2, THREADS>(range, n, pairs, pairs_out, point_list, s_a, tid, key_shift);
+    else tile_sort_impl<EMAX, THREADS>(range, n, pairs, pairs_out, point_list, s_a, tid, key_shift);
+}
+
 constexpr int kBuckets = 2048;
 constexpr int kBucketThreads = 512;
 constexpr int kBucketRankMax = 64;
@@ -335,10 +337,10 @@
 constexpr int kBucketCapBig = 11 * kBucketThreadsBig;
 constexpr int kBucketsBig = 4096;
 
-template <int E, int T, int NB, int CAP>
-__device__ __forceinline__ void bucket_sort_impl(const uint2 range, uint32_t n, const unsigned long long* __restrict__ pairs,
+template <int E, int T, int NB, int CAP, bool MASKS>
+__device__ __forceinline__ void bucket_sort_impl(const uint2 range, uint32_t n, unsigned long long* pairs,
                                                  uint32_t* __restrict__ point_list, unsigned long long* s_keys, uint32_t* s_cnt, uint16_t* s_off,
-                                                 float* s_redf, uint32_t* s_redu, int tid)
+                                                 float* s_redf, uint32_t* s_redu, int tid, int key_shift)
 {
     const int lane = tid & 63, wave = tid >> 6;
     unsigned long long k[E];
@@ -396,6 +398,25 @@
         for (int j = 0; j < PB; j++) { s_off[tid * PB + j] = (uint16_t)run; run += c[j]; }
         if (tid * PB + PB == nbins) s_off[nbins] = (uint16_t)run;
     }
+    const bool words = MASKS && key_shift != 0 && list_has_mask_words(n);
+    const uint32_t nchunks = (n + 63u) >> 6;
+    static_assert(!MASKS || (CAP + 7) / 8 <= NB / 2, "the nibbles fit the counter array");
+    if (words && fullest > (uint32_t)kBucketRankMax) for (uint32_t w = tid; w < nchunks * 8u; w += T) s_cnt[w] = 0u;
+#define GS_NOTE(rank, key)                                                                                              \
+    if (words) {                                                                                                        \
+        const uint32_t r_ = (rank), m_ = (uint32_t)(key) & 15u;                                                         \
+        if (m_) atomicOr(&s_cnt[r_ >> 3], m_ << ((r_ & 7u) * 4u));                                                      \
+    }
+#define GS_WORDS_OUT()                                                                                                  \
+    if (words) {                                                                                                        \
+        __syncthreads();                                                                                                \
+        for (uint32_t c_ = (uint32_t)wave; c_ < nchunks; c_ += T / kWave) {                                             \
+            const uint32_t m_ = (s_cnt[c_ * 8u + ((uint32_t)lane >> 3)] >> (((uint32_t)lane & 7u) * 4u)) & 15u;         \
+            const unsigned long long w0_ = __ballot((m_ & 1u) != 0u), w1_ = __ballot((m_ & 2u) != 0u);                  \
+            const unsigned long long w2_ = __ballot((m_ & 4u) != 0u), w3_ = __ballot((m_ & 8u) != 0u);                  \
+            if (lane < 4) pairs[range.x + mask_word_index(n, c_, (uint32_t)lane)] = lane == 0 ? w0_ : lane == 1 ? w1_ : lane == 2 ? w2_ : w3_; \
+        }                                                                                                               \
+    }
     __syncthreads();
     if (fullest <= (uint32_t)kBucketRankMax) {
 #pragma unroll
@@ -404,16 +425,34 @@
             if (e < n) s_keys[s_off[GS_BIN(k[i])] + ((arr[i >> 1] >> (16 * (i & 1))) & 0xffffu)] = k[i];
         }
         __syncthreads();
+        uint32_t note[E];
 #pragma unroll
         for (int i = 0; i < E; i++) {
             const uint32_t p = (uint32_t)i * T + tid;
+            note[i] = 0xffffffffu;
             if (p < n) {
                 const unsigned long long key = s_keys[p];
                 const uint32_t b = GS_BIN(key);
                 const uint32_t lo = s_off[b], hi = s_off[b + 1];
                 uint32_t rank = lo;
                 for (uint32_t j = lo; j < hi; j++) rank += s_keys[j] < key ? 1u : 0u;
-                point_list[range.x + rank] = (uint32_t)key;
+                point_list[range.x + rank] = key_id(key, key_shift);
+                note[i] = (rank << 4) | ((uint32_t)key & 15u);
+            }
+        }
+        if (words) {
+            uint8_t* s_m8 = reinterpret_cast<uint8_t*>(s_keys);
+            __syncthreads();
+#pragma unroll
+            for (int i = 0; i < E; i++)
+                if (note[i] != 0xffffffffu) s_m8[note[i] >> 4] = (uint8_t)(note[i] & 15u);
+            __syncthreads();
+            for (uint32_t c_ = (uint32_t)wave; c_ < nchunks; c_ += T / kWave) {
+                const uint32_t at = c_ * 64u + (uint32_t)lane;
+                const uint32_t m_ = at < n ? (uint32_t)s_m8[at] : 0u;
+                const unsigned long long w0_ = __ballot((m_ & 1u) != 0u), w1_ = __ballot((m_ & 2u) != 0u);
+                const unsigned long long w2_ = __ballot((m_ & 4u) != 0u), w3_ = __ballot((m_ & 8u) != 0u);
+                if (lane < 4) pairs[range.x + mask_word_index(n, c_, (uint32_t)lane)] = lane == 0 ? w0_ : lane == 1 ? w1_ : lane == 2 ? w2_ : w3_;
             }
         }
         return;
@@ -432,8 +471,10 @@
         __syncthreads();
         for (uint32_t e = tid; e < n; e += T) {
             const unsigned long long v = s_keys[e];
-            point_list[range.x + e] = (uint32_t)v;
-        }
+            point_list[range.x + e] = key_id(v, key_shift);
+            GS_NOTE(e, v)
+        }
+        GS_WORDS_OUT()
         return;
     }
     constexpr int EB = 4;
@@ -460,13 +501,17 @@
             if (s_keys[base + mid] < key) lo = mid + 1; else hi = mid;
         }
         const uint32_t rank = (in_a ? e : e - nA) + lo;
-        point_list[range.x + rank] = (uint32_t)key;
-    }
+        point_list[range.x + rank] = key_id(key, key_shift);
+        GS_NOTE(rank, key)
+    }
+    GS_WORDS_OUT()
+#undef GS_NOTE
+#undef GS_WORDS_OUT
 }
 
 template <bool BIG>
 __global__ __launch_bounds__(BIG ? kBucketThreadsBig : kBucketThreads, BIG ? 4 : 6) void tile_bucket_sort_kernel(
-    const uint2* __restrict__ ranges, const unsigned long long* __restrict__ pairs, uint32_t* __restrict__ point_list, uint32_t cap)
+    const uint2* __restrict__ ranges, unsigned long long* pairs, uint32_t* __restrict__ point_list, uint32_t cap, int key_shift)
 {
     constexpr int T = BIG ? kBucketThreadsBig : kBucketThreads, NB = BIG ? kBucketsBig : kBuckets, CAP = BIG ? kBucketCapBig : kBucketCap;
     __shared__ unsigned long long s_keys[CAP];
@@ -479,17 +524,17 @@
     range.x = min(range.x, cap); range.y = min(range.y, cap);
     const uint32_t n = range.y - range.x;
     if (n == 0 || n > (uint32_t)CAP || (BIG && n <= (uint32_t)kBucketCap)) return;
-    if (BIG) { bucket_sort_impl<11, T, NB, CAP>(range, n, pairs, point_list, s_keys, s_cnt, s_off, s_redf, s_redu, tid); return; }
-    if (n <= 2u * T) bucket_sort_impl<2, T, NB, CAP>(range, n, pairs, point_list, s_keys, s_cnt, s_off, s_redf, s_redu, tid);
-    else if (n <= 4u * T) bucket_sort_impl<4, T, NB, CAP>(range, n, pairs, point_list, s_keys, s_cnt, s_off, s_redf, s_redu, tid);
-    else if (n <= 8u * T) bucket_sort_impl<8, T, NB, CAP>(range, n, pairs, point_list, s_keys, s_cnt, s_off, s_redf, s_redu, tid);
-    else bucket_sort_impl<11, T, NB, CAP>(range, n, pairs, point_list, s_keys, s_cnt, s_off, s_redf, s_redu, tid);
+    if (BIG) { bucket_sort_impl<11, T, NB, CAP, !BIG>(range, n, pairs, point_list, s_keys, s_cnt, s_off, s_redf, s_redu, tid, key_shift); return; }
+    if (n <= 2u * T) bucket_sort_impl<2, T, NB, CAP, !BIG>(range, n, pairs, point_list, s_keys, s_cnt, s_off, s_redf, s_redu, tid, key_shift);
+    else if (n <= 4u * T) bucket_sort_impl<4, T, NB, CAP, !BIG>(range, n, pairs, point_list, s_keys, s_cnt, s_off, s_redf, s_redu, tid, key_shift);
+    else if (n <= 8u * T) bucket_sort_impl<8, T, NB, CAP, !BIG>(range, n, pairs, point_list, s_keys, s_cnt, s_off, s_redf, s_redu, tid, key_shift);
+    else bucket_sort_impl<11, T, NB, CAP, !BIG>(range, n, pairs, point_list, s_keys, s_cnt, s_off, s_redf, s_redu, tid, key_shift);
 }
 
 template <int CAP, int CHUNK, int THREADS>
 __global__ __launch_bounds__(THREADS) void tile_merge_kernel(const uint2* __restrict__ ranges,
                                                               unsigned long long* __restrict__ pairs,
-                                                              uint32_t* __restrict__ point_list, uint32_t cap, uint32_t skip_le)
+                                                              uint32_t* __restrict__ point_list, uint32_t cap, uint32_t skip_le, int key_shift)
 {
     __shared__ unsigned long long s_k[CAP];
     const int tid = threadIdx.x;
@@ -515,14 +560,14 @@
             rank += lo;
         }
         pairs[range.x + rank] = key;
-        point_list[range.x + rank] = (uint32_t)key;
+        point_list[range.x + rank] = key_id(key, key_shift);
     }
 }
 
 template <int OUT, int THREADS>
 __global__ __launch_bounds__(THREADS) void tile_merge_pass_kernel(const uint2* __restrict__ ranges, const unsigned long long* __restrict__ src,
                                                                    unsigned long long* __restrict__ dst, uint32_t* __restrict__ point_list,
-                                                                   uint32_t run, uint32_t cap)
+                                                                   uint32_t run, uint32_t cap, int key_shift)
 {
     __shared__ unsigned long long s_in[OUT];
     __shared__ unsigned long long s_out[OUT];
@@ -575,7 +620,7 @@
     for (uint32_t i = tid; i < m; i += THREADS) {
         const unsigned long long key = s_out[i];
         dst[range.x + o0 + i] = key;
-        if (point_list) point_list[range.x + o0 + i] = (uint32_t)key;
+        if (point_list) point_list[range.x + o0 + i] = key_id(key, key_shift);
     }
 }
 
@@ -587,11 +632,11 @@
 
 template <bool SCATTER>
 static void launch_bin(int threads, int nb, hipStream_t st, Cam cam, int P, GeomPtrs gp, int tiles, int chunk,
-                       uint32_t* tile_total, uint32_t* tile_base, const uint2* ranges, unsigned long long* pairs, uint32_t cap)
+                       uint32_t* tile_total, uint32_t* tile_base, const uint2* ranges, unsigned long long* pairs, uint32_t cap, int key_shift = 0)
 {
     const int nchunks = nb;
     nb = 8 * ((nb + 7) / 8);
-    hipLaunchKernelGGL((tile_bin_kernel<SCATTER, 1024>), dim3(nb), dim3(1024), 0, st, cam, P, gp, tiles, chunk, tile_total, tile_base, ranges, pairs, cap, nchunks);
+    hipLaunchKernelGGL((tile_bin_kernel<SCATTER, 1024>), dim3(nb), dim3(1024), 0, st, cam, P, gp, tiles, chunk, tile_total, tile_base, ranges, pairs, cap, nchunks, key_shift);
 }
 
 hipError_t launch_tile_count(const Cam& cam, int P, GeomPtrs gp, uint32_t* tile_total, uint32_t* tile_base,
@@ -611,44 +656,45 @@
                                     uint32_t* point_list, uint32_t cap, hipStream_t st)
 {
     const int tiles = cam.gx * cam.gy;
+    const int key_shift = key_shift_for(P);
     int threads, chunk; bin_config(P, threads, chunk);
     const int nb = (P + chunk - 1) / chunk;
-    if (nb > 0) launch_bin<true>(threads, nb, st, cam, P, gp, tiles, chunk, nullptr, tile_base, ranges, pairs, cap);
+    if (nb > 0) launch_bin<true>(threads, nb, st, cam, P, gp, tiles, chunk, nullptr, tile_base, ranges, pairs, cap, key_shift);
     constexpr int kBigChunk = 2 * kSortChunk;
     const bool big = max_tile_instances > (uint32_t)kBucketCap && max_tile_instances <= (uint32_t)kSortCapMax && tiles <= 512;
     const uint32_t skip_le = max_tile_instances <= (uint32_t)kSortCapMax ? (uint32_t)(big ? kBucketCapBig : kBucketCap) : 0u;
     if (skip_le) {
-        hipLaunchKernelGGL(tile_bucket_sort_kernel<false>, dim3(tiles), dim3(kBucketThreads), 0, st, ranges, pairs, point_list, cap);
+        hipLaunchKernelGGL(tile_bucket_sort_kernel<false>, dim3(tiles), dim3(kBucketThreads), 0, st, ranges, pairs, point_list, cap, key_shift);
         if (max_tile_instances <= (uint32_t)kBucketCap) return hipGetLastError();
         if (big) {
-            hipLaunchKernelGGL(tile_bucket_sort_kernel<true>, dim3(tiles), dim3(kBucketThreadsBig), 0, st, ranges, pairs, point_list, cap);
+            hipLaunchKernelGGL(tile_bucket_sort_kernel<true>, dim3(tiles), dim3(kBucketThreadsBig), 0, st, ranges, pairs, point_list, cap, key_shift);
             if (max_tile_instances <= (uint32_t)kBucketCapBig) return hipGetLastError();
         }
     }
     if (max_tile_instances <= (uint32_t)kSortChunk) {
-        hipLaunchKernelGGL((tile_sort_kernel<kSortChunk, 256>), dim3(tiles, 1), dim3(256), 0, st, ranges, pairs, pairs, point_list, cap, 0u);
+        hipLaunchKernelGGL((tile_sort_kernel<kSortChunk, 256>), dim3(tiles, 1), dim3(256), 0, st, ranges, pairs, pairs, point_list, cap, 0u, key_shift);
         return hipGetLastError();
     }
     const unsigned chunks = (max_tile_instances + kBigChunk - 1) / kBigChunk;
     if (max_tile_instances <= (uint32_t)kSortCapMax) {
-        hipLaunchKernelGGL((tile_sort_kernel<kBigChunk, 256>), dim3(tiles, chunks), dim3(256), 0, st, ranges, pairs, pairs, point_list, cap, skip_le);
+        hipLaunchKernelGGL((tile_sort_kernel<kBigChunk, 256>), dim3(tiles, chunks), dim3(256), 0, st, ranges, pairs, pairs, point_list, cap, skip_le, key_shift);
         if (max_tile_instances > 8192)
-            hipLaunchKernelGGL((tile_merge_kernel<kSortCapMax, kBigChunk, 1024>), dim3(tiles), dim3(1024), 0, st, ranges, pairs, point_list, cap, skip_le);
+            hipLaunchKernelGGL((tile_merge_kernel<kSortCapMax, kBigChunk, 1024>), dim3(tiles), dim3(1024), 0, st, ranges, pairs, point_list, cap, skip_le, key_shift);
         else if (max_tile_instances > (uint32_t)kBigChunk)
-            hipLaunchKernelGGL((tile_merge_kernel<8192, kBigChunk, 1024>), dim3(tiles), dim3(1024), 0, st, ranges, pairs, point_list, cap, skip_le);
+            hipLaunchKernelGGL((tile_merge_kernel<8192, kBigChunk, 1024>), dim3(tiles), dim3(1024), 0, st, ranges, pairs, point_list, cap, skip_le, key_shift);
         return hipGetLastError();
     }
     constexpr int kOut = kSortChunk;
     int passes = 0;
     for (uint64_t r = kBigChunk; r < max_tile_instances; r <<= 1) passes++;
     unsigned long long* cur = (passes & 1) ? pairs_alt : pairs;
-    hipLaunchKernelGGL((tile_sort_kernel<kBigChunk, 256>), dim3(tiles, chunks), dim3(256), 0, st, ranges, pairs, cur, point_list, cap, 0u);
+    hipLaunchKernelGGL((tile_sort_kernel<kBigChunk, 256>), dim3(tiles, chunks), dim3(256), 0, st, ranges, pairs, cur, point_list, cap, 0u, key_shift);
     const unsigned blocks = (max_tile_instances + kOut - 1) / kOut;
     uint64_t r = kBigChunk;
     for (int p = 0; p < passes; p++, r <<= 1) {
         unsigned long long* nxt = cur == pairs ? pairs_alt : pairs;
         hipLaunchKernelGGL((tile_merge_pass_kernel<kOut, 256>), dim3(tiles, blocks), dim3(256), 0, st, ranges, cur, nxt,
-                           p == passes - 1 ? point_list : nullptr, (uint32_t)r, cap);
+                           p == passes - 1 ? point_list : nullptr, (uint32_t)r, cap, key_shift);
         cur = nxt;
     }
     return hipGetLastError();
diff --git a/include/gsplat_hip.h b/include/gsplat_hip.h
--- a/include/gsplat_hip.h
+++ b/include/gsplat_hip.h
@@ -83,6 +83,7 @@
 int gs_set_backward_chain_tickets(int32_t on);
 int gs_set_backward_chain_polls(int32_t polls);
 int gs_set_forward_priority(int32_t mode, float param);
+int gs_set_quadrant_masks(int32_t on);
 int gs_async_status_word(uint32_t** host_word);
 int gs_async_status_clear(void);
 int gs_recorded_cut(uint32_t target, uint32_t* nearest, int32_t* level);
@@ -91,7 +92,7 @@
 
 const char* gs_last_error(void);
 const char* gs_version(void);
-#define GS_ABI_VERSION 22
+#define GS_ABI_VERSION 23
 int32_t gs_abi_version(void);
 
 int gs_profile_enable(int32_t on);
```

After: 1508 frames/s (median of 3 runs). About the same (+0.2%).
